# actionml/universal-recommender

Hardware: AMD Instinct MI355X
Metric: cooccurrence pairs/sec (A'A+A'B) + LLR top-k items/sec (higher is better)
Workload: dtype int32 counts / f64 LLR; 1 GPU; config4: synthetic 10M users x 2M items, Zipf-1.0, 5 event types (purchase/view/add-to-cart/search/category-pref); generator=torch Philox on the GPU (universal_recommender_amd.synth.generate_device), maxEventsPerEventType=500, maxCorrelatorsPerEventType=50, seed=20260925, entry_point=urcco_context_build_device (C ABI, include/urcco.h), launch=one process per GPU, parallelism=items range-partitioned over 1 GPU(s), one HIP stream per event type

## Files before the change

### include/urcco.h

```cpp
#ifndef URCCO_H
#define URCCO_H

#include <stdint.h>

#ifdef __cplusplus
extern "C" {
#endif

#define URCCO_VERSION 305

typedef enum urcco_status {
  URCCO_OK = 0,
  URCCO_BAD_ARG = 1,
  URCCO_OOM_HOST = 2,
  URCCO_OOM_DEVICE = 3,
  URCCO_HIP_ERROR = 4,
  URCCO_INTERNAL = 5,
  URCCO_NO_DEVICE = 6,
  URCCO_RCCL_ERROR = 7,
  URCCO_BUSY = 8
} urcco_status;

#define URCCO_ROW_RATE_MAHOUT_INT_DIV 0
#define URCCO_ROW_RATE_FRACTIONAL 1
// ... 117 lines not shown
  int32_t reserved;
  const urcco_dev_shard* shards;
} urcco_dev_dataset;
typedef struct urcco_dev_result {
  int32_t item_lo, item_hi;
  const int64_t* row_ptr;
  const int32_t* col_idx;
  const double* llr;
  const int64_t* stats;
  const int64_t* sampled_row_ptr;
  const int32_t* sampled_col_idx;
  int64_t sampled_rows;
  int64_t sampled_nnz_total;
  int32_t sampled_col_mask;
} urcco_dev_result;
int urcco_context_build_device(urcco_context* ctx, const urcco_dev_dataset* datasets, int32_t n_datasets, int64_t n_users_total,
                               int32_t random_seed, void* input_stream, urcco_dev_result* out);
int urcco_context_wait_stream(urcco_context* ctx, void* stream);
int urcco_context_synchronize(urcco_context* ctx);
int urcco_context_set_timing(urcco_context* ctx, int32_t enable);
int urcco_context_get_timings(urcco_context* ctx, double* ms, int64_t* launches);
int urcco_context_get_timings_gpu(urcco_context* ctx, int32_t local_gpu, double* ms, int64_t* launches);
int urcco_context_set_debug(urcco_context* ctx, int32_t flags);
int urcco_context_set_flags(urcco_context* ctx, int32_t flags);


typedef struct urcco_session urcco_session;

int urcco_session_create(int32_t device, void* stream, urcco_session** out);
void urcco_session_destroy(urcco_session* s);
int urcco_session_synchronize(urcco_session* s);
#define URCCO_N_STAGES 17
enum {
  URCCO_STAGE_COLUMN_COUNTS = 0,
  URCCO_STAGE_DOWNSAMPLE_FLAGS = 1,
  URCCO_STAGE_DOWNSAMPLE_SCAN = 2,
  URCCO_STAGE_DOWNSAMPLE_COMPACT = 3,
  URCCO_STAGE_TRANSPOSE = 4,
  URCCO_STAGE_ROW_WORK = 5,
  URCCO_STAGE_BINNING = 6,
  URCCO_STAGE_ENTROPY = 7,
  URCCO_STAGE_CCO_BIN0 = 8,
  URCCO_STAGE_CCO_BIN1 = 9,
  URCCO_STAGE_CCO_BIN2 = 10,
  URCCO_STAGE_CCO_BIN3 = 11,
  URCCO_STAGE_CCO_BIN4 = 12,
  URCCO_STAGE_CCO_BIN5 = 13,
  URCCO_STAGE_CCO_BIN6 = 14,
  URCCO_STAGE_COMPACT_INDICATORS = 15,
  URCCO_STAGE_EXCHANGE = 16
};
int urcco_session_set_timing(urcco_session* s, int32_t enable);
int urcco_session_set_debug(urcco_session* s, int32_t flags);
int urcco_session_get_timings(urcco_session* s, double* ms , int64_t* launches );
int64_t urcco_session_scratch_bytes(const urcco_session* s);
void urcco_debug_dump_marks(void);

int urcco_dev_column_counts(urcco_session* s, int64_t nnz, const int32_t* col_idx, int32_t n_cols, int32_t* counts);

int urcco_dev_downsample(urcco_session* s, int64_t n_rows, const int64_t* row_ptr, const int32_t* col_idx,
                         int64_t nnz, int32_t n_cols, const int32_t* raw_counts, int32_t seed,
                         int32_t max_elements_per_row, int32_t row_rate_mode, int64_t row_base,
                         int64_t* out_row_ptr, int32_t* out_col_idx, int32_t* post_counts);

int urcco_dev_transpose(urcco_session* s, int64_t n_rows, const int64_t* row_ptr, const int32_t* col_idx,
                        int64_t nnz, int32_t n_cols, const int32_t* counts, int32_t col_lo, int32_t col_hi,
                        int64_t* out_col_ptr, int32_t* out_row_idx);

int urcco_dev_row_work(urcco_session* s, int32_t item_lo, int32_t item_hi, int32_t n_items_a, const int64_t* a_col_ptr,
                       const int32_t* a_row_idx, int64_t nnz_a_bound, const int64_t* b_row_ptr, int64_t* work);

int urcco_dev_row_work_csr(urcco_session* s, int64_t n_rows, const int64_t* a_row_ptr, const int32_t* a_col_idx,
                           int64_t nnz_a, const int64_t* b_row_ptr, int32_t n_items_a, int64_t* work);

int urcco_dev_partition(urcco_session* s, int32_t n_items, const int64_t* work, int32_t n_parts,
                        int32_t* bounds_host);

int urcco_dev_merge_fragments(urcco_session* s, int32_t world, int32_t item_lo, int32_t item_hi, int32_t n_items,
                              const void* lens, int32_t wire16, const int32_t* entries, int64_t n_entries,
                              const int64_t* sizes, const int32_t* counts, int64_t* out_col_ptr, int32_t* out_row_idx);

#define URCCO_STATS_LEN 32
#define URCCO_EXCH_SIZES 4
int urcco_dev_cco_rows(urcco_session* s, int32_t item_lo, int32_t item_hi, int32_t n_items_a,
                       const int64_t* a_col_ptr, const int32_t* a_row_idx, int64_t nnz_a_bound,
                       const int64_t* b_row_ptr, const int32_t* b_col_idx, int32_t n_cols_b, const int32_t* counts_a,
                       const int32_t* counts_b, int64_t n_users, int32_t exclude_self, int32_t k,
                       int32_t has_min_llr, double min_llr, int32_t* out_count, int32_t* out_idx,
                       double* out_llr, int64_t* stats_dev);

int urcco_dev_pack_counts(urcco_session* s, int64_t n_rows_b, const int64_t* b_row_ptr, const int32_t* b_col_idx, int64_t nnz_b_bound, const int32_t* counts_b,
                          int32_t n_cols_b, int32_t* out_packed, int32_t* out_bad);
int urcco_dev_cco_rows_packed(urcco_session* s, int32_t item_lo, int32_t item_hi, int32_t n_items_a,
                              const int64_t* a_col_ptr, const int32_t* a_row_idx, int64_t nnz_a_bound,
                              const int64_t* b_row_ptr, const int32_t* b_col_idx, int32_t n_cols_b, const int32_t* counts_a,
                              const int32_t* counts_b, int64_t n_users, int32_t exclude_self, int32_t k,
                              int32_t has_min_llr, double min_llr, int32_t* out_count, int32_t* out_idx,
                              double* out_llr, int64_t* stats_dev, const int32_t* b_packed, const int32_t* pack_bad);

int urcco_dev_compact_indicators(urcco_session* s, int32_t n_rows, int32_t k, const int32_t* count,
                                 const int32_t* idx, const double* llr, int64_t* out_row_ptr,
                                 int32_t* out_col_idx, double* out_llr);

int urcco_dev_pop_counts(urcco_session* s, int64_t n_events, const int32_t* item_ids, const int64_t* times_ms, int32_t n_items,
                         int32_t n_intervals, const int64_t* bounds_host, int32_t* counts);

// ... 65 lines not shown
```

### universal-recommender_amd/_lib.py

```python
from __future__ import annotations

import ctypes as C
import os
from typing import Optional

_HERE = os.path.dirname(os.path.abspath(__file__))
DEFAULT_PATH = os.path.join(_HERE, "lib", "liburcco.so")

OK, BAD_ARG, OOM_HOST, OOM_DEVICE, HIP_ERROR, INTERNAL, NO_DEVICE, RCCL_ERROR, BUSY = range(9)
FLAG_SINGLE_STREAM = 1
FLAG_FORCE_EXCHANGE = 2
FLAG_UNORDERED_ROWS = 4
FLAG_EMULATE_RANKS = 8
UNIQUE_ID_BYTES = 128
ROW_RATE_MAHOUT_INT_DIV = 0
ROW_RATE_FRACTIONAL = 1
RNG_SPLITMIX53 = 0
RNG_MIX32 = 0x100
N_STAGES = 17
N_BINS = 7
STATS_LEN = 32
REC_MAX_CLAUSES = 16
REC_MAX_NUM = 256
REC_NO_BACKFILL = 1
# ... 68 lines not shown

class DatasetStats(C.Structure):
    _fields_ = [("nnz_raw", C.c_int64), ("nnz_sampled", C.c_int64), ("pairs", C.c_int64), ("nnz_out", C.c_int64),
                ("rows_by_bin", C.c_int64 * 7), ("ms_total", C.c_double)]


class RecClause(C.Structure):
    _fields_ = [("n_cols", C.c_int32), ("reserved", C.c_int32), ("boost", C.c_double), ("ind_col_ptr", C.c_void_p), ("ind_row_idx", C.c_void_p),
                ("q_row_ptr", C.c_void_p), ("q_col_idx", C.c_void_p)]


class RecRule(C.Structure):
    _fields_ = [("kind", C.c_int32), ("n_cols", C.c_int32), ("m_row_ptr", C.c_void_p), ("m_col_idx", C.c_void_p), ("q_row_ptr", C.c_void_p),
                ("q_col_idx", C.c_void_p), ("item_value", C.c_void_p), ("q_lo", C.c_void_p), ("q_hi", C.c_void_p)]


_p = C.c_void_p
SYMBOLS = {
    "urcco_version": (C.c_int, []),
    "urcco_device_count": (C.c_int, []),
    "urcco_last_error": (C.c_char_p, []),
    "urcco_status_string": (C.c_char_p, [C.c_int]),
    "urcco_cooccurrences_idss": (C.c_int, [C.POINTER(Csr), C.c_int32, C.c_int32, C.c_int32, C.c_int32, C.POINTER(Options),
                                           C.POINTER(Indicators), C.POINTER(DatasetStats)]),
    "urcco_cross_occurrence_downsampled": (C.c_int, [C.POINTER(Dataset), C.c_int32, C.c_int32, C.POINTER(Options),
                                                     C.POINTER(Indicators), C.POINTER(DatasetStats)]),
    "urcco_free_indicators": (None, [C.POINTER(Indicators), C.c_int32]),
    "urcco_cross_occurrence_stage": (C.c_int, [C.POINTER(Dataset), C.c_int32, C.c_int32, C.POINTER(Options)]),
    "urcco_cross_occurrence_finish": (C.c_int, [C.POINTER(Indicators), C.c_int32, C.POINTER(DatasetStats)]),
    "urcco_cross_occurrence_cancel": (C.c_int, []),
    "urcco_cross_occurrence_cancel_any": (C.c_int, []),
    "urcco_context_stage": (C.c_int, [_p, C.POINTER(Dataset), C.c_int32, C.c_int32]),
    "urcco_context_finish": (C.c_int, [_p, C.POINTER(Indicators), C.POINTER(DatasetStats)]),
    "urcco_shutdown": (C.c_int, []),
    "urcco_comm_unique_id": (C.c_int, [_p]),
    "urcco_context_create": (C.c_int, [C.POINTER(Options), C.POINTER(CommConfig), C.POINTER(_p)]),
    "urcco_context_destroy": (None, [_p]),
    "urcco_context_local_gpus": (C.c_int32, [_p]),
    "urcco_context_cross_occurrence": (C.c_int, [_p, C.POINTER(Dataset), C.c_int32, C.c_int32, C.POINTER(Indicators), C.POINTER(DatasetStats)]),
    "urcco_context_build_device": (C.c_int, [_p, C.POINTER(DevDataset), C.c_int32, C.c_int64, C.c_int32, _p, C.POINTER(DevResult)]),
    "urcco_context_wait_stream": (C.c_int, [_p, _p]),
    "urcco_context_synchronize": (C.c_int, [_p]),
    "urcco_context_set_timing": (C.c_int, [_p, C.c_int32]),
    "urcco_context_get_timings": (C.c_int, [_p, C.POINTER(C.c_double), C.POINTER(C.c_int64)]),
    "urcco_context_get_timings_gpu": (C.c_int, [_p, C.c_int32, C.POINTER(C.c_double), C.POINTER(C.c_int64)]),
    "urcco_context_set_debug": (C.c_int, [_p, C.c_int32]),
    "urcco_context_set_flags": (C.c_int, [_p, C.c_int32]),
    "urcco_session_create": (C.c_int, [C.c_int32, _p, C.POINTER(_p)]),
    "urcco_session_destroy": (None, [_p]),
    "urcco_session_synchronize": (C.c_int, [_p]),
    "urcco_session_scratch_bytes": (C.c_int64, [_p]),
    "urcco_session_set_timing": (C.c_int, [_p, C.c_int32]),
    "urcco_session_set_debug": (C.c_int, [_p, C.c_int32]),
    "urcco_debug_dump_marks": (None, []),
    "urcco_session_get_timings": (C.c_int, [_p, C.POINTER(C.c_double), C.POINTER(C.c_int64)]),
    "urcco_dev_column_counts": (C.c_int, [_p, C.c_int64, _p, C.c_int32, _p]),
    "urcco_dev_downsample": (C.c_int, [_p, C.c_int64, _p, _p, C.c_int64, C.c_int32, _p, C.c_int32, C.c_int32, C.c_int32, C.c_int64,
                                       _p, _p, _p]),
    "urcco_dev_transpose": (C.c_int, [_p, C.c_int64, _p, _p, C.c_int64, C.c_int32, _p, C.c_int32, C.c_int32, _p, _p]),
    "urcco_dev_row_work_csr": (C.c_int, [_p, C.c_int64, _p, _p, C.c_int64, _p, C.c_int32, _p]),
    "urcco_dev_row_work": (C.c_int, [_p, C.c_int32, C.c_int32, C.c_int32, _p, _p, C.c_int64, _p, _p]),
    "urcco_dev_partition": (C.c_int, [_p, C.c_int32, _p, C.c_int32, C.POINTER(C.c_int32)]),
    "urcco_dev_merge_fragments": (C.c_int, [_p, C.c_int32, C.c_int32, C.c_int32, C.c_int32, _p, C.c_int32, _p, C.c_int64, _p, _p, _p, _p]),
    "urcco_dev_cco_rows": (C.c_int, [_p, C.c_int32, C.c_int32, C.c_int32, _p, _p, C.c_int64, _p, _p, C.c_int32, _p, _p, C.c_int64, C.c_int32,
                                     C.c_int32, C.c_int32, C.c_double, _p, _p, _p, _p]),
    "urcco_dev_pack_counts": (C.c_int, [_p, C.c_int64, _p, _p, C.c_int64, _p, C.c_int32, _p, _p]),
    "urcco_dev_cco_rows_packed": (C.c_int, [_p, C.c_int32, C.c_int32, C.c_int32, _p, _p, C.c_int64, _p, _p, C.c_int32, _p, _p, C.c_int64, C.c_int32,
                                            C.c_int32, C.c_int32, C.c_double, _p, _p, _p, _p, _p, _p]),
    "urcco_dev_compact_indicators": (C.c_int, [_p, C.c_int32, C.c_int32, _p, _p, _p, _p, _p, _p]),
    "urcco_dev_pop_counts": (C.c_int, [_p, C.c_int64, _p, _p, C.c_int32, C.c_int32, C.POINTER(C.c_int64), _p]),
    "urcco_dev_recommend": (C.c_int, [_p, C.c_int64, C.c_int32, C.POINTER(RecClause), C.c_int32, _p, _p, _p, _p, C.c_int32, C.c_int32, _p, _p, _p, _p]),
    "urcco_dev_recommend_rules": (C.c_int, [_p, C.c_int64, C.c_int32, C.POINTER(RecClause), C.c_int32, _p, _p, _p, _p, C.c_int32, C.c_int32, _p, _p, _p, _p,
                                            C.POINTER(RecRule), C.c_int32]),
    "urcco_dev_llr": (C.c_int, [_p, C.c_int64, _p, _p, _p, _p, _p]),
    "urcco_dev_u01": (C.c_int, [_p, C.c_int64, C.c_int32, _p, _p, _p]),
    "urcco_dev_u01_rng": (C.c_int, [_p, C.c_int64, C.c_int32, _p, _p, C.c_int32, _p]),
    "urcco_dev_dictionary_build": (C.c_int, [_p, C.c_int64, _p, _p, C.c_int32, _p, C.POINTER(_p), C.POINTER(C.c_int64)]),
    "urcco_dev_dictionary_lookup": (C.c_int, [_p, _p, C.c_int64, _p, _p, _p]),
    "urcco_dev_dictionary_verify": (C.c_int, [_p, _p, C.c_int64, _p, _p, _p, _p, C.POINTER(C.c_int64)]),
    "urcco_dev_dictionary_verify_against": (C.c_int, [_p, _p, C.c_int64, _p, _p, _p, _p, _p, C.POINTER(C.c_int64)]),
    "urcco_hash_strings": (C.c_int, [_p, _p, C.c_int64, C.c_uint64, _p]),
    "urcco_key_table_destroy": (None, [_p]),
    "urcco_dev_csr_from_pairs": (C.c_int, [_p, C.c_int64, _p, _p, C.c_int64, _p, _p, C.POINTER(C.c_int64)]),
}

_cache = {}
_lib_path: Optional[str] = None


def _bind(path: str) -> C.CDLL:
    try:
        import torch
    except ImportError:
        pass
    lib = C.CDLL(path)
    for name, (res, args) in SYMBOLS.items():
        fn = getattr(lib, name)
        fn.restype = res
        fn.argtypes = args
    return lib


def use_library(path: Optional[str]) -> None:
    global _lib_path
    _lib_path = path

# ... 26 lines not shown
```

### universal-recommender_amd/csrc/cco_common.h

```cpp
#pragma once
#include "cco_kernels.h"

namespace urcco {


constexpr int WAVE = 64;

__device__ __forceinline__ unsigned long long shfl_xor_u64(unsigned long long v, int m) {
  unsigned lo = (unsigned)v, hi = (unsigned)(v >> 32);
  lo = __shfl_xor(lo, m);
  hi = __shfl_xor(hi, m);
  return ((unsigned long long)hi << 32) | lo;
}
__device__ __forceinline__ long long shfl_i64(long long v, int src) {
  unsigned lo = (unsigned)v, hi = (unsigned)((unsigned long long)v >> 32);
  lo = __shfl(lo, src);
  hi = __shfl(hi, src);
  return (long long)(((unsigned long long)hi << 32) | lo);
}
__device__ __forceinline__ long long shfl_up_i64(long long v, unsigned d) {
  unsigned lo = (unsigned)v, hi = (unsigned)((unsigned long long)v >> 32);
  lo = __shfl_up(lo, d);
  hi = __shfl_up(hi, d);
  return (long long)(((unsigned long long)hi << 32) | lo);
// ... 35 lines not shown
        x[2 * q + 1] = (long long)(((unsigned long long)(unsigned)a.w << 32) | (unsigned)a.z);
      }
    } else {
#pragma unroll
      for (int q = 0; q < 8; ++q) x[q] = p[i + q];
    }
  }
};
template <int NT = SCAN_THREADS>
__device__ __forceinline__ long long block_exclusive_scan(long long v, long long* s_wave , long long* total) {
  const int lane = threadIdx.x & (WAVE - 1), wave = threadIdx.x / WAVE;
  long long inc = v;
#pragma unroll
  for (int d = 1; d < WAVE; d <<= 1) {
    const long long o = shfl_up_i64(inc, d);
    if (lane >= d) inc += o;
  }
  if (lane == WAVE - 1) s_wave[wave] = inc;
  __syncthreads();
  long long base = 0, tot = 0;
#pragma unroll
  for (int w = 0; w < NT / WAVE; ++w) {
    const long long sw = s_wave[w];
    if (w < wave) base += sw;
    tot += sw;
  }
  __syncthreads();
  *total = tot;
  return base + inc - v;
}

template <typename Load>
__global__ __launch_bounds__(SCAN_THREADS) void scan_reduce_kernel(Load ld, int64_t n, int64_t* __restrict__ tile_sums,
                                                                   const int64_t* __restrict__ n_live) {
  __shared__ long long s_wave[SCAN_THREADS / WAVE];
  const int64_t base = (int64_t)blockIdx.x * SCAN_TILE;
  if (n_live && base >= *n_live) {
    if (threadIdx.x == 0) tile_sums[blockIdx.x] = 0;
    return;
  }
  long long v = 0;
#pragma unroll
  for (int q = 0; q < SCAN_ITEMS; ++q) {
    const int64_t i = base + (int64_t)q * SCAN_THREADS + threadIdx.x;
    if (i < n) v += ld(i);
  }
  long long tot;
  block_exclusive_scan(v, s_wave, &tot);
  if (threadIdx.x == 0) tile_sums[blockIdx.x] = tot;
}

constexpr int ST_THREADS = 1024;
constexpr int ST_ITEMS = 8;
static __global__ __launch_bounds__(ST_THREADS) void scan_tiles_kernel(int64_t* __restrict__ tile_sums, int64_t n_tiles, const int64_t* __restrict__ n_live) {
  __shared__ long long s_wave[ST_THREADS / WAVE];
  const int lane = threadIdx.x & (WAVE - 1), wave = threadIdx.x / WAVE;
  int64_t live_tiles = n_tiles;
  if (n_live) {
    const int64_t lt = *n_live / SCAN_TILE + 1;
    if (lt < live_tiles) live_tiles = lt;
  }
  long long carry = 0;
  for (int64_t base = 0; base < live_tiles; base += ST_THREADS * ST_ITEMS) {
    const int64_t first = base + (int64_t)threadIdx.x * ST_ITEMS;
    long long x[ST_ITEMS];
    long long sum = 0;
#pragma unroll
    for (int q = 0; q < ST_ITEMS; ++q) {
      x[q] = first + q < live_tiles ? tile_sums[first + q] : 0;
      sum += x[q];
    }
    long long inc = sum;
#pragma unroll
    for (int d = 1; d < WAVE; d <<= 1) {
      const long long o = shfl_up_i64(inc, d);
      if (lane >= d) inc += o;
    }
    if (lane == WAVE - 1) s_wave[wave] = inc;
    __syncthreads();
    long long before = 0, tot = 0;
#pragma unroll
    for (int w = 0; w < ST_THREADS / WAVE; ++w) {
      const long long sw = s_wave[w];
      if (w < wave) before += sw;
      tot += sw;
    }
    __syncthreads();
    long long run = carry + before + inc - sum;
#pragma unroll
    for (int q = 0; q < ST_ITEMS; ++q) {
      if (first + q < live_tiles) tile_sums[first + q] = run;
      run += x[q];
    }
    carry += tot;
  }
  for (int64_t t = live_tiles + threadIdx.x; t < n_tiles; t += ST_THREADS) tile_sums[t] = carry;
  if (threadIdx.x == 0) tile_sums[n_tiles] = carry;
}

template <typename Load>
__global__ __launch_bounds__(SCAN_THREADS) void scan_downsweep_kernel(Load ld, int64_t n, const int64_t* __restrict__ tile_sums,
                                                                      int64_t n_tiles, int64_t* __restrict__ out,
                                                                      const int64_t* __restrict__ n_live) {
  __shared__ long long s_wave[SCAN_THREADS / WAVE];
  if (n_live && (int64_t)blockIdx.x * SCAN_TILE > *n_live) return;
  const int64_t first = (int64_t)blockIdx.x * SCAN_TILE + (int64_t)threadIdx.x * SCAN_ITEMS;
  static_assert(SCAN_ITEMS == 8, "load8");
  long long x[SCAN_ITEMS];
  long long v = 0;
  const bool interior = first + SCAN_ITEMS <= n;
  if (interior) {
    ld.load8(first, x);
  } else {
#pragma unroll
    for (int q = 0; q < SCAN_ITEMS; ++q) x[q] = first + q < n ? ld(first + q) : 0;
  }
#pragma unroll
  for (int q = 0; q < SCAN_ITEMS; ++q) v += x[q];
  long long tot;
  long long run = block_exclusive_scan(v, s_wave, &tot) + tile_sums[blockIdx.x];
  if (interior && (reinterpret_cast<uintptr_t>(out) & 15) == 0) {
#pragma unroll
    for (int q = 0; q < SCAN_ITEMS; q += 2) {
      const long long e0 = run, e1 = run + x[q];
      run = e1 + x[q + 1];
      int4 w;
      w.x = (int)(unsigned)e0; w.y = (int)(unsigned)((unsigned long long)e0 >> 32);
      w.z = (int)(unsigned)e1; w.w = (int)(unsigned)((unsigned long long)e1 >> 32);
      *reinterpret_cast<int4*>(out + first + q) = w;
    }
  } else {
#pragma unroll
    for (int q = 0; q < SCAN_ITEMS; ++q) {
      const int64_t i = first + q;
      if (i < n) out[i] = run;
      run += x[q];
    }
  }
  if (blockIdx.x == 0 && threadIdx.x == 0) out[n] = tile_sums[n_tiles];
}

constexpr int SB_THREADS = 1024;
constexpr int SB_ITEMS = 8;
constexpr int64_t SB_MAX = 32768;
template <typename Load>
__global__ __launch_bounds__(SB_THREADS) void scan_block_kernel(Load ld, int64_t n, int64_t* __restrict__ out) {
  __shared__ long long s_wave[SB_THREADS / WAVE];
  const int lane = threadIdx.x & (WAVE - 1), wave = threadIdx.x / WAVE;
  long long carry = 0;
  for (int64_t base = 0; base < n; base += SB_THREADS * SB_ITEMS) {
    const int64_t first = base + (int64_t)threadIdx.x * SB_ITEMS;
    long long x[SB_ITEMS];
    long long sum = 0;
    if (first + SB_ITEMS <= n) {
      ld.load8(first, x);
    } else {
#pragma unroll
      for (int q = 0; q < SB_ITEMS; ++q) x[q] = first + q < n ? ld(first + q) : 0;
    }
#pragma unroll
    for (int q = 0; q < SB_ITEMS; ++q) sum += x[q];
    long long inc = sum;
#pragma unroll
    for (int d = 1; d < WAVE; d <<= 1) {
      const long long o = shfl_up_i64(inc, d);
      if (lane >= d) inc += o;
    }
    if (lane == WAVE - 1) s_wave[wave] = inc;
    __syncthreads();
    long long before = 0, tot = 0;
#pragma unroll
    for (int w = 0; w < SB_THREADS / WAVE; ++w) {
      const long long sw = s_wave[w];
      if (w < wave) before += sw;
      tot += sw;
    }
    __syncthreads();
    long long run = carry + before + inc - sum;
#pragma unroll
    for (int q = 0; q < SB_ITEMS; ++q) {
      if (first + q < n) out[first + q] = run;
      run += x[q];
    }
    carry += tot;
  }
  if (threadIdx.x == 0) out[n] = carry;
}

template <typename Load>
static hipError_t launch_scan(hipStream_t st, Load ld, int64_t n, int64_t* out, int64_t* tile_sums, const int64_t* n_live = nullptr, bool tile_sums_ready = false) {
  if (n <= 0) return hipMemsetAsync(out, 0, sizeof(int64_t), st);
  if (n <= SB_MAX) {
    hipLaunchKernelGGL((scan_block_kernel<Load>), dim3(1), dim3(SB_THREADS), 0, st, ld, n, out);
    return hipGetLastError();
  }
  const int64_t n_tiles = (n + SCAN_TILE - 1) / SCAN_TILE;
  if (!tile_sums_ready) hipLaunchKernelGGL((scan_reduce_kernel<Load>), dim3((unsigned)n_tiles), dim3(SCAN_THREADS), 0, st, ld, n, tile_sums, n_live);
  hipLaunchKernelGGL(scan_tiles_kernel, dim3(1), dim3(ST_THREADS), 0, st, tile_sums, n_tiles, n_live);
  hipLaunchKernelGGL((scan_downsweep_kernel<Load>), dim3((unsigned)n_tiles), dim3(SCAN_THREADS), 0, st, ld, n, tile_sums, n_tiles, out, n_live);
  return hipGetLastError();
}
}
```

### universal-recommender_amd/csrc/cco_expand.hip

```cpp
#include "cco_kernels.h"

#include <atomic>
#include <cstdio>
#include <cstdlib>

#include "cco_common.h"
#include "cco_device.h"


namespace urcco {

__global__ __launch_bounds__(256) void item_entropy_kernel(const int32_t* __restrict__ counts, int32_t n, long long n_users,
                                                           double* __restrict__ ent, double* __restrict__ xlx_n) {
  const int64_t i = (int64_t)blockIdx.x * 256 + threadIdx.x;
  if (i < n) {
    const long long c = counts[i];
    ent[i] = entropy2(c, n_users - c);
  }
  if (i == 0 && xlx_n) *xlx_n = x_log_x(n_users);
}

hipError_t launch_item_entropy(hipStream_t st, const int32_t* counts, int32_t n, long long n_users, double* ent, double* xlx_n) {
  const int blocks = n > 0 ? (n + 255) / 256 : 1;
  hipLaunchKernelGGL(item_entropy_kernel, dim3(blocks), dim3(256), 0, st, counts, n, n_users, ent, xlx_n);
// ... 58 lines not shown
    const unsigned d0 = two ? (unsigned)cnt[z.x] : 0u, d1 = two ? (unsigned)cnt[z.y] : 0u, d2 = two ? (unsigned)cnt[z.z] : 0u, d3 = two ? (unsigned)cnt[z.w] : 0u;
    n_bad += (c0 >= limit) + (c1 >= limit) + (c2 >= limit) + (c3 >= limit) + (d0 >= limit) + (d1 >= limit) + (d2 >= limit) + (d3 >= limit);
    int4 y;
    y.x = (int)((unsigned)x.x | (c0 << shift)); y.y = (int)((unsigned)x.y | (c1 << shift));
    y.z = (int)((unsigned)x.z | (c2 << shift)); y.w = (int)((unsigned)x.w | (c3 << shift));
    nt_store4(out + 4 * v, y);
    if (two) {
      y.x = (int)((unsigned)z.x | (d0 << shift)); y.y = (int)((unsigned)z.y | (d1 << shift));
      y.z = (int)((unsigned)z.z | (d2 << shift)); y.w = (int)((unsigned)z.w | (d3 << shift));
      nt_store4(out + 4 * (v + stride), y);
    }
  }
  for (int64_t e = (nvec << 2) + (int64_t)blockIdx.x * 256 + threadIdx.x; e < nnz; e += stride) {
    const unsigned j = (unsigned)ci[e], c = (unsigned)cnt[j];
    n_bad += c >= limit;
    out[e] = (int)(j | (c << shift));
  }
  if (n_bad) atomicAdd(bad, n_bad);
}
hipError_t launch_pack_counts(hipStream_t st, int n_cu, const int32_t* col_idx, const int64_t* nnz_dev, int64_t nnz_bound, const unsigned short* counts16,
                              const int32_t* bad16, int32_t count_bits, int32_t* out, int32_t* bad) {
  hipError_t e = hipMemsetAsync(bad, 0, sizeof(int32_t), st);
  if (e != hipSuccess || nnz_bound <= 0) return e;
  const int shift = 32 - count_bits;
  int64_t blocks = (nnz_bound / 4 + 255) / 256;
  const int64_t cap = (int64_t)n_cu * 16;
  if (blocks > cap) blocks = cap;
  if (blocks < 1) blocks = 1;
  const int vec_ok = ((reinterpret_cast<uintptr_t>(col_idx) | reinterpret_cast<uintptr_t>(out)) & 15) == 0;
  hipLaunchKernelGGL(pack_counts_kernel, dim3((unsigned)blocks), dim3(256), 0, st, col_idx, nnz_dev, nnz_bound, counts16, bad16, shift, out, bad, vec_ok);
  return hipGetLastError();
}

__global__ __launch_bounds__(256) void xlx_table_kernel(double* __restrict__ tab) {
  const int x = blockIdx.x * 256 + threadIdx.x;
  if (x < XLX_TABLE) tab[x] = x_log_x((long long)x);
}
hipError_t launch_xlx_table(hipStream_t st, double* tab) {
  hipLaunchKernelGGL(xlx_table_kernel, dim3(XLX_TABLE / 256), dim3(256), 0, st, tab);
  return hipGetLastError();
}
__global__ __launch_bounds__(256) void xlx_hi_table_kernel(double* __restrict__ tab, const double* __restrict__ xlx_tab, long long n_users) {
  const int d = blockIdx.x * 256 + threadIdx.x;
  if (d >= XLX_TABLE) return;
  tab[d] = n_users - d >= 0 ? x_log_x(n_users - (long long)d) : 0.0;
  const double hi = n_users - d >= 0 ? x_log_x(n_users - (long long)d) : 0.0;
  tab[XLX_TABLE + d] = d <= n_users ? (x_log_x(n_users) - x_log_x_tab((long long)d, xlx_tab)) - hi : 0.0;
}
hipError_t launch_xlx_hi_table(hipStream_t st, double* tab, const double* xlx_tab, long long n_users) {
  hipLaunchKernelGGL(xlx_hi_table_kernel, dim3(XLX_TABLE / 256), dim3(256), 0, st, tab, xlx_tab, n_users);
  return hipGetLastError();
}

__global__ __launch_bounds__(256) void narrow_row_ptr_kernel(const int64_t* __restrict__ rp, int64_t n, unsigned* __restrict__ out) {
  for (int64_t i = (int64_t)blockIdx.x * 256 + threadIdx.x; i < n; i += (int64_t)gridDim.x * 256) out[i] = (unsigned)rp[i];
}

__global__ __launch_bounds__(256) void expand_prepare_kernel(const int64_t* __restrict__ a_cp, int32_t n_items_a, const int32_t* __restrict__ a_ri,
                                                             const int64_t* __restrict__ b_rp, const unsigned* __restrict__ b_rp32, int64_t n_rows_b,
                                                             int64_t cap, int64_t* __restrict__ pstart, int32_t* __restrict__ plen) {
  const int64_t nnz = a_cp[n_items_a];
  int64_t lim = (nnz / SCAN_TILE + 1) * SCAN_TILE;
  if (lim > cap) lim = cap;
  const bool narrow = b_rp32 != nullptr && b_rp[n_rows_b] < ((int64_t)1 << 32);
  const int64_t stride = (int64_t)gridDim.x * 256;
  for (int64_t p0 = (int64_t)blockIdx.x * 256 + threadIdx.x; p0 < lim; p0 += stride * 4) {
    int u[4];
#pragma unroll
    for (int q = 0; q < 4; ++q) {
      const int64_t p = p0 + q * stride;
      u[q] = p < nnz ? a_ri[p] : -1;
    }
    int64_t s[4], e[4];
    if (narrow) {
#pragma unroll
      for (int q = 0; q < 4; ++q) {
        s[q] = u[q] >= 0 ? (int64_t)b_rp32[u[q]] : 0;
        e[q] = u[q] >= 0 ? (int64_t)b_rp32[u[q] + 1] : 0;
      }
    } else {
#pragma unroll
      for (int q = 0; q < 4; ++q) {
        s[q] = u[q] >= 0 ? b_rp[u[q]] : 0;
        e[q] = u[q] >= 0 ? b_rp[u[q] + 1] : 0;
      }
    }
#pragma unroll
    for (int q = 0; q < 4; ++q) {
      const int64_t p = p0 + q * stride;
      if (p < lim) {
        pstart[p] = s[q];
        plen[p] = (int32_t)(e[q] - s[q]);
      }
    }
  }
}

hipError_t launch_expand_prepare(hipStream_t st, int n_cu, const int64_t* a_col_ptr, int32_t n_items_a, const int32_t* a_row_idx,
                                 const int64_t* b_row_ptr, unsigned* b_rp32_scratch, int64_t n_rows_b, int64_t cap, int64_t* pstart, int32_t* plen,
                                 int64_t* wp, int64_t* tile_sums) {
  if (cap > 0) {
    if (b_rp32_scratch) {
      int64_t nb = (n_rows_b + 1 + 255) / 256;
      if (nb > (int64_t)n_cu * 8) nb = (int64_t)n_cu * 8;
      hipLaunchKernelGGL(narrow_row_ptr_kernel, dim3((unsigned)nb), dim3(256), 0, st, b_row_ptr, n_rows_b + 1, b_rp32_scratch);
    }
    int64_t blocks = (cap + 1023) / 1024;
    const int64_t lim = (int64_t)n_cu * 16;
    if (blocks > lim) blocks = lim;
    hipLaunchKernelGGL(expand_prepare_kernel, dim3((unsigned)blocks), dim3(256), 0, st, a_col_ptr, n_items_a, a_row_idx, b_row_ptr,
                       (const unsigned*)b_rp32_scratch, n_rows_b, cap, pstart, plen);
  }
  return launch_scan(st, LoadI32{plen}, cap, wp, tile_sums, a_col_ptr + n_items_a);
}

struct __attribute__((packed, aligned(4))) Words4 { unsigned a, b, c, d; };
struct __attribute__((packed, aligned(4))) Words2 { unsigned a, b; };
struct ExpandMultiArgs {
  const int64_t* b_rp[EXPAND_MULTI_MAX];
  int64_t* pstart[EXPAND_MULTI_MAX];
  int32_t* plen[EXPAND_MULTI_MAX];
  int64_t* tsum[EXPAND_MULTI_MAX];
  int n;
};
__global__ __launch_bounds__(256) void expand_pack_kernel(ExpandMultiArgs a, int64_t n_rows_b, unsigned* __restrict__ T) {
  for (int64_t u = (int64_t)blockIdx.x * 256 + threadIdx.x; u <= n_rows_b; u += (int64_t)gridDim.x * 256)
    for (int d = 0; d < a.n; ++d) T[u * a.n + d] = (unsigned)a.b_rp[d][u];
}
template <int N>
__global__ __launch_bounds__(256) void expand_prepare_multi_kernel(const int64_t* __restrict__ a_cp, int32_t n_items_a, const int32_t* __restrict__ a_ri,
                                                                   const unsigned* __restrict__ T, int64_t cap, ExpandMultiArgs a) {
  __shared__ long long s_part[256 / WAVE][N];
  const int64_t nnz = a_cp[n_items_a];
  int64_t lim = (nnz / SCAN_TILE + 1) * SCAN_TILE;
  if (lim > cap) lim = cap;
  const int64_t n_tiles = (lim + SCAN_TILE - 1) / SCAN_TILE;
  for (int64_t tile = blockIdx.x; tile < n_tiles; tile += gridDim.x) {
    const int64_t base = tile * SCAN_TILE;
    long long sum[N];
#pragma unroll
    for (int d = 0; d < N; ++d) sum[d] = 0;
    for (int r = 0; r < SCAN_ITEMS; r += 2) {
      int u[2];
      unsigned v[2][2 * N];
#pragma unroll
      for (int q = 0; q < 2; ++q) {
        const int64_t p = base + (int64_t)(r + q) * 256 + threadIdx.x;
        u[q] = p < nnz ? a_ri[p] : -1;
      }
#pragma unroll
      for (int q = 0; q < 2; ++q) {
        if (u[q] >= 0) {
          const unsigned* t = T + (int64_t)u[q] * N;
          if (N == 4) {
            const uint4 x = *reinterpret_cast<const uint4*>(t), y = *reinterpret_cast<const uint4*>(t + 4);
            v[q][0] = x.x; v[q][1] = x.y; v[q][2] = x.z; v[q][3] = x.w;
            v[q][4 % (2 * N)] = y.x; v[q][5 % (2 * N)] = y.y; v[q][6 % (2 * N)] = y.z; v[q][7 % (2 * N)] = y.w;
          } else {
            constexpr int W = 2 * N;
#pragma unroll
            for (int d = 0; d + 4 <= W; d += 4) {
              const Words4 x = *reinterpret_cast<const Words4*>(t + d);
              v[q][d] = x.a; v[q][(d + 1) % W] = x.b; v[q][(d + 2) % W] = x.c; v[q][(d + 3) % W] = x.d;
            }
            if (W % 4 >= 2) {
              const Words2 x = *reinterpret_cast<const Words2*>(t + (W / 4) * 4);
              v[q][(W / 4) * 4 % W] = x.a; v[q][((W / 4) * 4 + 1) % W] = x.b;
            }
            if (W % 2 == 1) v[q][W - 1] = t[W - 1];
          }
        } else {
#pragma unroll
          for (int d = 0; d < 2 * N; ++d) v[q][d] = 0u;
        }
      }
#pragma unroll
      for (int q = 0; q < 2; ++q) {
        const int64_t p = base + (int64_t)(r + q) * 256 + threadIdx.x;
        if (p < lim) {
#pragma unroll
          for (int d = 0; d < N; ++d) {
            const int32_t len = (int32_t)(v[q][N + d] - v[q][d]);
            a.pstart[d][p] = (int64_t)v[q][d];
            a.plen[d][p] = len;
            sum[d] += (long long)len;
          }
        }
      }
    }
#pragma unroll
    for (int d = 0; d < N; ++d) {
      unsigned long long x = (unsigned long long)sum[d];
#pragma unroll
      for (int m = 1; m < WAVE; m <<= 1) x += shfl_xor_u64(x, m);
      if ((threadIdx.x & (WAVE - 1)) == 0) s_part[threadIdx.x / WAVE][d] = (long long)x;
    }
    __syncthreads();
    if (threadIdx.x < N && a.tsum[threadIdx.x]) {
      long long tot = 0;
#pragma unroll
      for (int w = 0; w < 256 / WAVE; ++w) tot += s_part[w][threadIdx.x];
      a.tsum[threadIdx.x][tile] = tot;
    }
    __syncthreads();
  }
}
hipError_t launch_expand_prepare_multi(hipStream_t st, int n_cu, const int64_t* a_col_ptr, int32_t n_items_a, const int32_t* a_row_idx, int n,
                                       const int64_t* const* b_row_ptr, int64_t n_rows_b, int64_t cap, int64_t* const* pstart, int32_t* const* plen, void* T,
                                       int64_t* const* tsum) {
  if (n < 1 || n > EXPAND_MULTI_MAX) return hipErrorInvalidValue;
  if (cap <= 0) return hipSuccess;
  ExpandMultiArgs a;
  a.n = n;
  for (int d = 0; d < EXPAND_MULTI_MAX; ++d) {
    a.b_rp[d] = d < n ? b_row_ptr[d] : nullptr;
    a.pstart[d] = d < n ? pstart[d] : nullptr;
    a.plen[d] = d < n ? plen[d] : nullptr;
    a.tsum[d] = (d < n && tsum) ? tsum[d] : nullptr;
  }
  int64_t nb = (n_rows_b + 255) / 256;
  if (nb > (int64_t)n_cu * 8) nb = (int64_t)n_cu * 8;
  if (nb < 1) nb = 1;
  hipLaunchKernelGGL(expand_pack_kernel, dim3((unsigned)nb), dim3(256), 0, st, a, n_rows_b, static_cast<unsigned*>(T));
  int64_t blocks = (cap + SCAN_TILE - 1) / SCAN_TILE;
  const int64_t lim = (int64_t)n_cu * 16;
  if (blocks > lim) blocks = lim;
  const unsigned* Tc = static_cast<const unsigned*>(T);
  switch (n) {
    case 1: hipLaunchKernelGGL(expand_prepare_multi_kernel<1>, dim3((unsigned)blocks), dim3(256), 0, st, a_col_ptr, n_items_a, a_row_idx, Tc, cap, a); break;
    case 2: hipLaunchKernelGGL(expand_prepare_multi_kernel<2>, dim3((unsigned)blocks), dim3(256), 0, st, a_col_ptr, n_items_a, a_row_idx, Tc, cap, a); break;
    case 3: hipLaunchKernelGGL(expand_prepare_multi_kernel<3>, dim3((unsigned)blocks), dim3(256), 0, st, a_col_ptr, n_items_a, a_row_idx, Tc, cap, a); break;
    case 4: hipLaunchKernelGGL(expand_prepare_multi_kernel<4>, dim3((unsigned)blocks), dim3(256), 0, st, a_col_ptr, n_items_a, a_row_idx, Tc, cap, a); break;
    case 5: hipLaunchKernelGGL(expand_prepare_multi_kernel<5>, dim3((unsigned)blocks), dim3(256), 0, st, a_col_ptr, n_items_a, a_row_idx, Tc, cap, a); break;
    case 6: hipLaunchKernelGGL(expand_prepare_multi_kernel<6>, dim3((unsigned)blocks), dim3(256), 0, st, a_col_ptr, n_items_a, a_row_idx, Tc, cap, a); break;
    case 7: hipLaunchKernelGGL(expand_prepare_multi_kernel<7>, dim3((unsigned)blocks), dim3(256), 0, st, a_col_ptr, n_items_a, a_row_idx, Tc, cap, a); break;
    default: hipLaunchKernelGGL(expand_prepare_multi_kernel<8>, dim3((unsigned)blocks), dim3(256), 0, st, a_col_ptr, n_items_a, a_row_idx, Tc, cap, a); break;
  }
  return hipGetLastError();
}
hipError_t launch_expand_scan(hipStream_t st, const int64_t* a_col_ptr, int32_t n_items_a, const int32_t* plen, int64_t cap, int64_t* wp, int64_t* tile_sums,
                              bool tile_sums_ready) {
  return launch_scan(st, LoadI32{plen}, cap, wp, tile_sums, a_col_ptr + n_items_a, tile_sums_ready);
}

__global__ __launch_bounds__(256) void row_work_kernel(int32_t item_lo, int32_t item_hi, const int64_t* __restrict__ a_cp,
                                                       const int64_t* __restrict__ wp, int64_t* __restrict__ work) {
  const int64_t n = (int64_t)item_hi - item_lo;
  for (int64_t t = (int64_t)blockIdx.x * 256 + threadIdx.x; t < n; t += (int64_t)gridDim.x * 256) {
    const int64_t i = item_lo + t;
    work[t] = wp[a_cp[i + 1]] - wp[a_cp[i]];
  }
}

hipError_t launch_row_work(hipStream_t st, int n_cu, int32_t item_lo, int32_t item_hi, const int64_t* a_col_ptr, const int64_t* wp, int64_t* work) {
  const int64_t n = (int64_t)item_hi - item_lo;
  if (n <= 0) return hipSuccess;
  int64_t blocks = (n + 255) / 256;
  const int64_t cap = (int64_t)n_cu * 8;
  if (blocks > cap) blocks = cap;
  hipLaunchKernelGGL(row_work_kernel, dim3((unsigned)blocks), dim3(256), 0, st, item_lo, item_hi, a_col_ptr, wp, work);
  return hipGetLastError();
}


}
```

### universal-recommender_amd/csrc/cco_kernels.h

```cpp
#pragma once
#include <hip/hip_runtime.h>
#include <stdint.h>

namespace urcco {

constexpr int NBINS = 7;
constexpr int MP_KMAX_HOST = 256;

constexpr int SCAN_TILE = 2048;
constexpr int DS_TILE = 4096;
constexpr int GLOBAL_BIN_BLOCKS = 128;
constexpr int BIN_TILE = 1024;
constexpr int XLX_TABLE_HOST = 4096;
constexpr int BIN_COLS_HOST = 3 * NBINS + 3;
constexpr int BIN_OFF_LEN = NBINS + 3;
constexpr int CAND_SLOTS = 64;
constexpr int STATS_LEN = 32;

constexpr int32_t DBG_GATHER_ONLY = 1;
constexpr int32_t DBG_NO_LLR = 2;
constexpr int32_t DBG_NO_TOPK = 4;
constexpr int32_t DBG_NO_SELECT = 8;
constexpr int32_t DBG_NO_RANK = 16;
constexpr int32_t DBG_NO_COUNT_GATHER = 512;
constexpr int32_t DBG_UNFUSED_EXPAND = 4096;
constexpr int32_t DBG_GATHERED_PRIMARY = 8192;
constexpr int32_t DBG_UNFILTERED_EXCHANGE = 16384;
constexpr int32_t DBG_SELECT_DELAY = 131072;
constexpr int32_t DBG_UNPACKED_COUNTS = 1048576;
constexpr int32_t DBG_ROW_KERNELS = DBG_GATHER_ONLY | DBG_NO_LLR | DBG_NO_TOPK | DBG_NO_SELECT | DBG_NO_RANK | DBG_NO_COUNT_GATHER | DBG_SELECT_DELAY;

struct CcoArgs {
  const int32_t* bin_rows;
  const int32_t* bin_off;
  const int64_t* a_col_ptr;
  const int64_t* pstart;
  const int64_t* wp;
  const int32_t* b_col_idx;
  const int32_t* b_packed;
  const int32_t* pack_bad;
  int32_t pk_known;
  uint32_t b_col_mask;
  const int32_t* cnt_a;
  const int32_t* cnt_b;
  const double* ent_a;
  const unsigned short* cnt_b16;
  const int32_t* cnt16_bad;
  const double* xlx_n;
  const double* xlx_tab;
  const double* xlx_hi;
  const double* col_ent;
  int32_t debug;
  long long n_users;
  int32_t n_cols_b;
  int32_t item_lo;
  int32_t exclude_self;
  int32_t k;
  int32_t has_min_llr;
  double min_llr;
  int32_t count_bits;
  int32_t col_bytes;
  int32_t g_log2;
  int32_t unordered;
  int32_t* out_count;
  int32_t* out_idx;
  double* out_llr;
  unsigned long long* err;
  unsigned long long* cand;
  int32_t* g_counts;
  unsigned long long* g_cand_key;
  int32_t* g_cand_col;
  int32_t g_blocks;
};

hipError_t launch_column_counts(hipStream_t st, int n_cu, const int32_t* col_idx, int64_t nnz, int32_t n_cols, int32_t* counts);
constexpr int64_t PH_MIN_NNZ = 1 << 20;
int64_t column_counts_scratch_bytes(int64_t nnz, int32_t n_cols);
hipError_t launch_column_counts_partitioned(hipStream_t st, const int32_t* col_idx, int64_t nnz, const int64_t* nnz_dev, int32_t n_cols,
                                            int32_t* counts, char* scratch);

hipError_t launch_scan_i32(hipStream_t st, const int32_t* in, int64_t n, int64_t* out, int64_t* tile_sums);
hipError_t launch_slice_weights(hipStream_t st, const unsigned short* loc_t, int n_buckets, int64_t n_parts, long long* weight);

hipError_t launch_downsample_flags(hipStream_t st, int n_cu, int64_t n_rows, const int64_t* row_ptr, const int32_t* col_idx, int64_t nnz,
                                   int32_t n_cols, const int32_t* raw_counts, unsigned long long* thresholds, uint32_t seed, int32_t max_n,
                                   int row_rate_mode, int64_t row_base, int64_t* tile_rows, unsigned long long* flags, int64_t* tile_count,
                                   int32_t* post_counts);
hipError_t launch_downsample_scan(hipStream_t st, int64_t nnz, int64_t* tile_count);
hipError_t launch_downsample_compact(hipStream_t st, int64_t n_rows, const int64_t* row_ptr, const int32_t* col_idx, int64_t nnz,
                                     const int64_t* tile_rows, const unsigned long long* flags, const int64_t* tile_off, int64_t* out_row_ptr,
                                     int32_t* out_col_idx);

hipError_t launch_scan_i32_range(hipStream_t st, const int32_t* in, int64_t n, int32_t lo, int32_t hi, int64_t* out, int64_t* tile_sums);
hipError_t launch_transpose(hipStream_t st, int n_cu, int64_t n_rows, const int64_t* row_ptr, const int32_t* col_idx, int g_log2,
                            const int64_t* col_ptr, int32_t* cursor, int32_t* out_row_idx, int32_t col_lo, int32_t col_hi);
int64_t transpose_scratch_bytes(int64_t n_rows, int64_t nnz, int32_t n_cols);
hipError_t launch_transpose_partitioned(hipStream_t st, int64_t n_rows, const int64_t* row_ptr, const int32_t* col_idx, int64_t nnz, int32_t n_cols,
                                        const int64_t* col_ptr, int32_t* cursor , int32_t* out_row_idx, int32_t col_lo, int32_t col_hi, char* scratch);
hipError_t launch_row_work_csr(hipStream_t st, int n_cu, int64_t n_rows, const int64_t* a_row_ptr, const int32_t* a_col_idx,
                               const int64_t* b_row_ptr, int g_log2, int32_t n_items_a, int64_t* work);

struct KeyTable {
  unsigned long long* keys;
  unsigned* minpos;
  unsigned* count;
  int32_t* id;
  unsigned long long mask;
};
hipError_t launch_dictionary_build(hipStream_t st, int n_cu, KeyTable t, int64_t n, const unsigned long long* keys, const int32_t* select,
                                   int32_t min_count, int32_t* flag, int64_t* prefix, int64_t* tile_sums, int64_t* first_pos);
hipError_t launch_dictionary_lookup(hipStream_t st, int n_cu, KeyTable t, int64_t n, const unsigned long long* keys, const int32_t* select,
                                    int32_t* ids);
hipError_t launch_dictionary_verify(hipStream_t st, int n_cu, KeyTable t, int64_t n, const unsigned long long* keys, const int32_t* select,
                                    const unsigned long long* check, const unsigned long long* ref_check, const int64_t* first_pos, unsigned long long* err);
hipError_t launch_csr_from_pairs(hipStream_t st, int n_cu, int64_t n, const int32_t* rows, const int32_t* cols, int64_t n_rows, int32_t* cnt,
                                 int64_t* raw_ptr, int32_t* tmp, int64_t* tile_sums, int64_t* out_row_ptr, int32_t* out_col_idx);

constexpr int EXCH_SIZES = 4;
hipError_t launch_row_lengths(hipStream_t st, int n_cu, int64_t n_rows, const int64_t* row_ptr, int32_t* len, unsigned short* len16, int64_t* sizes);
hipError_t launch_counts_over_limit(hipStream_t st, int n_cu, const int32_t* counts, int64_t n, int32_t count_bits, int64_t* out);
hipError_t launch_need_mask(hipStream_t st, int n_cu, int64_t n_rows, const int64_t* a_row_ptr, const int32_t* a_col_idx, const int32_t* bounds, int world,
                            unsigned long long* mask);
hipError_t launch_masked_lengths(hipStream_t st, int n_cu, int64_t n_rows, const int64_t* row_ptr, const unsigned long long* mask, int world, int32_t* mlen, int64_t* off,
                                 int64_t* tile_sums, int64_t* to_nnz);
hipError_t launch_pack_rows(hipStream_t st, int n_cu, int64_t n_rows, const int64_t* row_ptr, const int32_t* col_idx, const unsigned long long* mask, int world,
                            const int64_t* off, int32_t* pack);
hipError_t launch_scan_u16(hipStream_t st, const unsigned short* in, int64_t n, int64_t* out, int64_t* tile_sums);
hipError_t launch_frag_record(hipStream_t st, int32_t world, const int32_t* bounds, const int64_t* l_cp, const int32_t* bad, int64_t* rec);
hipError_t launch_frag_place(hipStream_t st, int n_cu, int32_t world, int32_t lo, int32_t n_range, const void* lens, int wire16, const int64_t* src_off,
                             const int32_t* ents, const int64_t* a_cp, const int64_t* sizes, int32_t* a_ri);

hipError_t launch_validate_csr(hipStream_t st, int n_cu, int64_t n_rows, const int64_t* row_ptr, const int32_t* col_idx, int64_t nnz, int32_t n_cols,
                               int g_log2, int64_t rp0, unsigned long long* err);
hipError_t launch_rebase_i64(hipStream_t st, int n_cu, int64_t* p, int64_t n, int64_t delta);
hipError_t launch_publish_word(hipStream_t st, const unsigned long long* src, unsigned long long* dst_mapped);

hipError_t launch_pop_counts(hipStream_t st, int n_cu, int64_t n, const int32_t* item, const int64_t* t_ms, int32_t n_items, int n_buckets,
                             const int64_t* bounds, int32_t* counts);

hipError_t launch_pack_counts(hipStream_t st, int n_cu, const int32_t* col_idx, const int64_t* nnz_dev, int64_t nnz_bound, const unsigned short* counts16,
                              const int32_t* bad16, int32_t count_bits, int32_t* out, int32_t* bad);
hipError_t launch_xlx_table(hipStream_t st, double* tab);
hipError_t launch_xlx_hi_table(hipStream_t st, double* tab , const double* xlx_tab, long long n_users);
hipError_t launch_item_entropy(hipStream_t st, const int32_t* counts, int32_t n, long long n_users, double* ent, double* xlx_n);
hipError_t launch_narrow_counts(hipStream_t st, int n_cu, const int32_t* counts, int64_t n, unsigned short* out16, int32_t* bad);

hipError_t launch_expand_prepare(hipStream_t st, int n_cu, const int64_t* a_col_ptr, int32_t n_items_a, const int32_t* a_row_idx,
                                 const int64_t* b_row_ptr, unsigned* b_rp32_scratch , int64_t n_rows_b, int64_t cap,
                                 int64_t* pstart, int32_t* plen, int64_t* wp, int64_t* tile_sums);
constexpr int EXPAND_MULTI_MAX = 8;
hipError_t launch_expand_prepare_multi(hipStream_t st, int n_cu, const int64_t* a_col_ptr, int32_t n_items_a, const int32_t* a_row_idx, int n,
                                       const int64_t* const* b_row_ptr, int64_t n_rows_b, int64_t cap, int64_t* const* pstart, int32_t* const* plen, void* T,
                                       int64_t* const* tsum );
hipError_t launch_expand_scan(hipStream_t st, const int64_t* a_col_ptr, int32_t n_items_a, const int32_t* plen, int64_t cap, int64_t* wp, int64_t* tile_sums,
                              bool tile_sums_ready = false);
hipError_t launch_row_work(hipStream_t st, int n_cu, int32_t item_lo, int32_t item_hi, const int64_t* a_col_ptr, const int64_t* wp, int64_t* work);

hipError_t launch_binning(hipStream_t st, int32_t item_lo, int32_t n, const int64_t* work, const int32_t* cnt_a, int32_t n_cols_b,
                          int32_t count_bits, int32_t k, int64_t* tile_counts, int32_t* bin_off, int32_t* bin_rows, int64_t* stats);

hipError_t launch_cco_rows_bin(hipStream_t st, int n_cu, const CcoArgs& args, int bin, int32_t n_rows );
hipError_t launch_bin_out_stats(hipStream_t st, const int32_t* bin_rows, const int32_t* bin_off, int32_t item_lo, const int32_t* out_count,
                                const unsigned long long* cand, int64_t* stats);

hipError_t launch_compact_indicators(hipStream_t st, int32_t n_rows, int32_t k, const int32_t* count, const int32_t* idx,
                                     const double* llr, const int64_t* row_ptr, int32_t* out_idx, double* out_llr);

hipError_t launch_partition(hipStream_t st, int32_t n_items, const int64_t* work_prefix, int32_t n_parts, int32_t* bounds);
hipError_t launch_scan_i64(hipStream_t st, const int64_t* in, int64_t n, int64_t* out, int64_t* tile_sums);

constexpr int REC_MAX_CLAUSES = 16;
constexpr int REC_MAX_NUM = 256;
constexpr int REC_NO_BACKFILL = 1;
constexpr int REC_STATS_LEN = 8;
constexpr int REC_LDS_LIMIT = 3072;
struct RecClause {
  const int64_t* ind_col_ptr;
  const int32_t* ind_row_idx;
  const int64_t* q_row_ptr;
  const int32_t* q_col_idx;
  double boost;
  int32_t n_cols;
  int32_t reserved;
};
constexpr int REC_MAX_RULES = 16;
constexpr int REC_RULE_ANY = 0;
constexpr int REC_RULE_NONE = 1;
constexpr int REC_RULE_RANGE = 2;
struct RecRule {
  const int64_t* m_row_ptr;
  const int32_t* m_col_idx;
  const int64_t* q_row_ptr;
  const int32_t* q_col_idx;
  const int64_t* item_value;
  const int64_t* q_lo;
  const int64_t* q_hi;
  int32_t kind, n_cols;
};
struct RecArgs;
int32_t recommend_global_blocks(int64_t n_queries, int32_t n_items, int n_cu);
hipError_t launch_recommend(hipStream_t st, int n_cu, int64_t n_queries, int32_t n_items, const RecClause* clauses, int32_t n_clauses, const int64_t* excl_row_ptr,
                            const int32_t* excl_col_idx, const uint8_t* item_mask, const int32_t* fill_order, int32_t num, int32_t flags, int32_t* out_count,
                            int32_t* out_idx, double* out_score, int64_t* stats_dev, unsigned long long* ctr, int32_t* list, int32_t* pos, int32_t g_blocks,
                            unsigned* g_state, unsigned* g_m, int32_t* g_list, double* g_score, int32_t lds_limit = REC_LDS_LIMIT, const RecRule* rules = nullptr,
                            int32_t n_rules = 0);

hipError_t launch_llr_test(hipStream_t st, int64_t n, const int64_t* a, const int64_t* b, const int64_t* ab, const int64_t* nu, double* out);
hipError_t launch_u01_test(hipStream_t st, int64_t n, uint32_t seed, const int32_t* row, const int32_t* col, double* out, int rng32 = 0);

// ... 2 lines not shown
```

### universal-recommender_amd/csrc/cco_rows.hip

```cpp
#include "cco_kernels.h"

#include <atomic>
#include <cstdlib>

#include "cco_common.h"
#include "cco_device.h"


namespace urcco {

constexpr int E0 = 1024, E1S = 4096, E1 = 8192, E2S = 16384, E2 = 32768;
constexpr int MP_KMAX = 256;

__host__ __device__ constexpr int table_slots(int E, int T) { return (2 * E / 3) / (2 * T) * (2 * T); }
constexpr int URCCO_WB1 = 512;
constexpr int URCCO_WB2 = 8192;
__device__ __forceinline__ int choose_bin(long long w, long long ca, int32_t n_cols_b, int32_t count_bits, int32_t k) {
  if (ca <= 0 || w <= 0) return -1;
  if (count_bits < 31 && ca > ((1ll << count_bits) - 1)) return NBINS - 1;
  if (w <= 64 && ca <= 64) return 0;
  int cap_bin = NBINS - 1;
  const long long dmax = (w < (long long)n_cols_b ? w : (long long)n_cols_b) * 3 + (long long)k * 3 + 2;
  if (dmax <= E0) cap_bin = 1;
  else if (dmax <= E1S) cap_bin = 2;
// ... 389 lines not shown
}

template <int T>
__device__ __forceinline__ unsigned claim_positions(bool want, unsigned* counter, unsigned& wave_count) {
  const unsigned long long m = __ballot(want);
  const unsigned c = (unsigned)__popcll(m);
  unsigned base;
  if (T == WAVE) {
    base = wave_count;
    wave_count += c;
  } else {
    unsigned b = 0u;
    if ((threadIdx.x & (WAVE - 1)) == 0 && c != 0u) b = atomicAdd(counter, c);
    base = wave_read_lane(b, 0);
  }
  return base + lanes_below(m);
}
template <int T>
__device__ __forceinline__ unsigned team_exclusive_scan(unsigned v, unsigned* s_wsum , unsigned* total) {
  const int lane = threadIdx.x & (WAVE - 1);
  const unsigned inc = wave_inclusive_sum(v);
  if (T == WAVE) {
    *total = wave_read_lane(inc, WAVE - 1);
    return inc - v;
  }
  const int wave = (threadIdx.x % T) / WAVE;
  if (lane == WAVE - 1) s_wsum[wave] = inc;
  __syncthreads();
  unsigned base = 0, tot = 0;
#pragma unroll
  for (int w = 0; w < T / WAVE; ++w) {
    const unsigned sw = s_wsum[w];
    if (w < wave) base += sw;
    tot += sw;
  }
  __syncthreads();
  *total = tot;
  return base + inc - v;
}

constexpr int URCCO_U_WAVE = 2;
constexpr int URCCO_U_BS = 2;
constexpr int URCCO_U_B = 2;
constexpr int URCCO_U_H = 1;
constexpr int URCCO_U_C = 1;
constexpr int URCCO_OCC_WAVE = 8;
constexpr int URCCO_OCC_BS = 7;
constexpr int URCCO_G_WAVE = 2;
constexpr int URCCO_SEL_AMB_WAVE = 64;
constexpr int URCCO_SEL_AMB_BLOCK = 128;
constexpr int URCCO_G_BLOCK = 2;
constexpr int URCCO_SEL_M_BLOCK = 128;
constexpr int URCCO_G_CU = 2;
template <int T, int E, int U, bool MP = false, bool DBG = false, bool PK = false>
__global__ __launch_bounds__((T < 256 ? 256 : T), (T == 64 ? URCCO_OCC_WAVE : (T == 256 && E == 4096 ? URCCO_OCC_BS : (T == 512 ? 4 : 1)))) void cco_rows_kernel(CcoArgs a, int bin) {
  if ((a.b_packed != nullptr && (a.pk_known != 0 || *a.pack_bad == 0)) != PK) return;
  const int dbg = DBG ? a.debug : 0;
  constexpr bool packed = PK;
  URCCO_OWN_GLOBAL_PTR(const int32_t, b_col_idx, PK ? a.b_packed : a.b_col_idx);
  const int cshift = 32 - a.count_bits;
  const unsigned colmask = PK ? (1u << cshift) - 1u : a.b_col_mask;
  URCCO_OWN_GLOBAL_PTR(const unsigned short, cnt_b16, a.cnt_b16);
  URCCO_OWN_GLOBAL_PTR(const int32_t, cnt_b, a.cnt_b);
  URCCO_OWN_GLOBAL_PTR(const double, xlx_tab, a.xlx_tab);
  URCCO_OWN_GLOBAL_PTR(const double, xlx_hi, a.xlx_hi);
  URCCO_OWN_GLOBAL_PTR(const double, col_ent, a.col_ent);
  URCCO_OWN_GLOBAL_PTR(int32_t, out_idx, a.out_idx);
  URCCO_OWN_GLOBAL_PTR(double, out_llr, a.out_llr);
  long long n_users = a.n_users;
  URCCO_OWN_SGPRS(n_users);
  constexpr int BLOCK = T < 256 ? 256 : T;
  constexpr int TEAMS = BLOCK / T;
  constexpr int SH = table_slots(E, T);
  constexpr int SPT = SH / T;
  static_assert(SH % (2 * T) == 0 && SH + SH / 2 <= E && SH <= 65536, "slots and the candidate list share the table; a slot index takes 16 bits of a list word");
  constexpr unsigned CAND_CAP = (unsigned)(E - SH);
  constexpr int CPT = ((E - 5) / 3 + T - 1) / T;
  constexpr int NW = T / WAVE;
  constexpr int G = T == WAVE ? URCCO_G_WAVE : (T == 256 ? URCCO_G_BLOCK : URCCO_G_CU);
  constexpr int LOG2E = E == 1024 ? 10 : (E == 4096 ? 12 : (E == 8192 ? 13 : (E == 16384 ? 14 : 15)));
  static_assert((1 << LOG2E) == E, "table size");
  constexpr int LOG2T = T == 64 ? 6 : (T == 256 ? 8 : (T == 512 ? 9 : 10));
  static_assert((1 << LOG2T) == T, "team size");
  __shared__ __attribute__((aligned(16))) unsigned s_tab[TEAMS * E];
  constexpr int NH = T == WAVE ? 1 : 3;
  constexpr int SEL_CAP = T == WAVE ? 0 : (T == 256 ? 512 : 2048);
  constexpr int SEL_M = T == WAVE ? 64 : URCCO_SEL_M_BLOCK;
  constexpr int SEL_AMB = T == WAVE ? URCCO_SEL_AMB_WAVE : URCCO_SEL_AMB_BLOCK;
  static_assert(SEL_AMB <= SEL_M, "ambiguous set capacity");
  constexpr bool SHARE = T == WAVE || (T == 256 && E == 4096);
  constexpr int SH_INS = T * 8 + (T + 1) * 4;
  constexpr int SH_LST = ((NH * 128 * 4 > SEL_M * 12 ? NH * 128 * 4 : SEL_M * 12) + 7) / 8 * 8;
  constexpr int SH_SEL = SH_LST + SEL_CAP * 2;
  constexpr int SHARE_WORDS = ((SH_INS > SH_SEL ? SH_INS : SH_SEL) + 7) / 8;
  __shared__ unsigned long long s_share[SHARE ? TEAMS * SHARE_WORDS : 1];
  __shared__ long long s_ustart[SHARE ? 1 : TEAMS * T];
  __shared__ unsigned s_uoff[SHARE ? 1 : TEAMS * (T + 1)];
  __shared__ unsigned s_wsum[NW];
  __shared__ unsigned s_hist[SHARE ? 1 : TEAMS * NH * 128];
  __shared__ unsigned s_selres[TEAMS * 4];
  __shared__ unsigned short s_lst[SHARE ? 1 : TEAMS * (SEL_CAP > 0 ? SEL_CAP : 1)];
  __shared__ unsigned long long s_ambkey[SHARE ? 1 : TEAMS * SEL_M];
  __shared__ unsigned s_ambcol[SHARE ? 1 : TEAMS * SEL_M];
  __shared__ unsigned long long s_selthr[TEAMS * 2];
  constexpr bool SKIP_SHARED = T >= 256;
  __shared__ unsigned long long s_kbits[2 * NW];
  __shared__ unsigned s_mpflag;
  __shared__ unsigned s_ncand;
  __shared__ unsigned long long s_runk[MP ? 2 * MP_KMAX : 1];
  __shared__ unsigned s_runc[MP ? 2 * MP_KMAX : 1];

  const int team = TEAMS == 1 ? 0 : uni((int)threadIdx.x / T);
  const int tl = threadIdx.x % T;
  const int lane = threadIdx.x & (WAVE - 1);
  unsigned* tab = s_tab + team * E;
  unsigned* cand = tab + SH;
  unsigned long long* share = s_share + (SHARE ? team * SHARE_WORDS : 0);
  long long* ustart = SHARE ? reinterpret_cast<long long*>(share) : s_ustart + team * T;
  unsigned* uoff = SHARE ? reinterpret_cast<unsigned*>(share + T) : s_uoff + team * (T + 1);
  unsigned* hist = SHARE ? reinterpret_cast<unsigned*>(share) : s_hist + team * NH * 128;
  unsigned* sel_res = s_selres + team * 4;
  unsigned* nsel = sel_res + 3;
  unsigned short* lst = SHARE ? reinterpret_cast<unsigned short*>(share) + SH_LST / 2 : s_lst + team * (SEL_CAP > 0 ? SEL_CAP : 1);
  unsigned long long* amb_key = SHARE ? share : s_ambkey + team * SEL_M;
  unsigned* amb_col = SHARE ? reinterpret_cast<unsigned*>(share + SEL_M) : s_ambcol + team * SEL_M;
  unsigned long long* sel_thr = s_selthr + team * 2;
  const int list_start = a.bin_off[bin];
  const int list_n = a.bin_off[bin + 1] - list_start;
  const int total_teams = gridDim.x * TEAMS;
  bool ident = (long long)a.n_cols_b * 3 + (long long)a.k * 3 + 2 <= E && a.n_cols_b <= SH;
  int cb = a.count_bits;
  unsigned cmask = (1u << cb) - 1u;
  unsigned long long cand_acc = 0ull;
  const double xlx_n = *a.xlx_n;
  const bool use16 = *a.cnt16_bad == 0;

  int li = blockIdx.x * TEAMS + team;
  if (li >= list_n) return;
  const int S = total_teams;
  auto pos_of = [&](int l) { return list_start + (l < list_n ? l : list_n - 1); };
  const unsigned* wp32 = reinterpret_cast<const unsigned*>(a.wp);
  const int lane3 = lane < 3 ? lane : 2;
  int idv = a.bin_rows[pos_of(li + lane3 * S)];
  int64_t cs_c, ce_c;
  int64_t bnd_b;
  {
    const int id0 = (int)wave_read_lane((unsigned)idv, 0);
    const int id1 = (int)wave_read_lane((unsigned)idv, 1);
    cs_c = uni(a.a_col_ptr[id0]);
    ce_c = uni(a.a_col_ptr[id0 + 1]);
    bnd_b = a.a_col_ptr[id1 + (lane & 1)];
  }
  unsigned pf_w0, pf_w1, pf_wp;
  int64_t pf_start;
  {
    const int64_t c1 = cs_c + T < ce_c ? cs_c + T : ce_c;
    const int64_t pl = cs_c + tl < c1 ? cs_c + tl : c1 - 1;
    pf_w0 = wp32[2 * cs_c];
    pf_w1 = wp32[2 * c1];
    pf_wp = wp32[2 * pl];
    pf_start = a.pstart[pl];
  }
  URCCO_SETTLE(idv); URCCO_SETTLE(bnd_b); URCCO_SETTLE(pf_w0); URCCO_SETTLE(pf_w1); URCCO_SETTLE(pf_wp); URCCO_SETTLE(pf_start);
  int64_t cs_n = 0, ce_n = 0, bnd_c = 0;
  for (; li < list_n; li += S, cs_c = cs_n, ce_c = ce_n, bnd_b = bnd_c) {
    const int i = (int)wave_read_lane((unsigned)idv, 0);
    const int id2 = (int)wave_read_lane((unsigned)idv, 2);
    const int64_t cs = cs_c, ce = ce_c;
    cs_n = wave_read_lane64(bnd_b, 0);
    ce_n = wave_read_lane64(bnd_b, 1);
    const unsigned row_w0 = uni(pf_w0), row_w1 = uni(pf_w1);
    const unsigned my_wp = pf_wp;
    const int64_t my_start = pf_start;
    int lz = lane;
    URCCO_OPAQUE(lz);
    idv = a.bin_rows[pos_of(li + (1 + (lz < 3 ? lz : 2)) * S)];
    bnd_c = a.a_col_ptr[id2 + (lz & 1)];
    if (!MP) {
      const int64_t c1 = cs_n + T < ce_n ? cs_n + T : ce_n;
      const int64_t pl = cs_n + tl < c1 ? cs_n + tl : c1 - 1;
      pf_w0 = wp32[2 * cs_n];
      pf_w1 = wp32[2 * c1];
      pf_wp = wp32[2 * pl];
      pf_start = a.pstart[pl];
    }
    int mp_s = 0;
    unsigned mp_q = 0u, n_run = 0u, run_cur = 0u;
    if (MP) {
      const long long w_row = (long long)(uni(a.wp[ce]) - uni(a.wp[cs]));
      const long long ca_row = a.cnt_a[i];
      const long long dd = w_row < (long long)a.n_cols_b ? w_row : (long long)a.n_cols_b;
      const long long cap = ((long long)E - 3ll * a.k - 2ll) / 3ll;
      for (;; ++mp_s) {
        const long long cols_pp = ((long long)a.n_cols_b + (1ll << mp_s) - 1) >> mp_s;
        int kb = 1;
        while ((1ll << kb) <= cols_pp) ++kb;
        const bool count_ok = kb <= 1 || ca_row <= (1ll << (32 - kb)) - 1;
        const long long exp_d = ((dd >> mp_s) + (dd >> (mp_s + 2)) + 1) < cols_pp ? ((dd >> mp_s) + (dd >> (mp_s + 2)) + 1) : cols_pp;
        if (count_ok && exp_d <= cap) break;
      }
    }
  mp_again:
    if (MP) {
      const long long cols_pp = ((long long)a.n_cols_b + (1ll << mp_s) - 1) >> mp_s;
      int kb = 1;
      while ((1ll << kb) <= cols_pp) ++kb;
      cb = 32 - kb;
      cmask = cb >= 32 ? 0xffffffffu : (1u << cb) - 1u;
      ident = cols_pp * 3 + 3ll * a.k + 2ll <= (long long)E && cols_pp <= (long long)SH;
      if (tl == 0) s_mpflag = 0u;
    }
    const unsigned mp_mask = MP ? (1u << mp_s) - 1u : 0u;
#pragma unroll
    for (int q = 0; q < SPT / 2; ++q) *reinterpret_cast<uint2*>(&tab[2 * (tl + q * T)]) = make_uint2(0u, 0u);
    unsigned n_cand = 0u;
    if (T != WAVE && tl == 0) s_ncand = 0u;
    team_sync<T>();
    for (int64_t c0 = cs; c0 < ce; c0 += T) {
      const int64_t c1 = c0 + T < ce ? c0 + T : ce;
      const bool pre = !MP && c0 == cs;
      const unsigned w0 = pre ? row_w0 : uni(wp32[2 * c0]);
      const unsigned total = (pre ? row_w1 : uni(wp32[2 * c1])) - w0;
      const int64_t p = c0 + tl;
      if (p < c1) {
        ustart[tl] = pre ? my_start : a.pstart[p];
        uoff[tl] = (pre ? my_wp : wp32[2 * p]) - w0;
      } else {
        uoff[tl] = total;
      }
      if (tl == 0) uoff[T] = total;
      team_sync<T>();
      if (total > 0u) {
        const unsigned per = (total + T - 1) / T;
        const unsigned first = (unsigned)tl * per;
        const bool act = first < total;
        const unsigned last = act ? (first + per < total ? first + per : total) : first;
        int o = 0;
        int64_t pos = 0;
        unsigned uend = 0u;
        if (act) {
          int lo = 1, hi = T;
#pragma unroll
          for (int step = 0; step < LOG2T; ++step) {
            const int mid = (lo + hi) >> 1;
            const bool gt = uoff[mid] > first;
            hi = gt ? mid : hi;
            lo = gt ? lo : mid + 1;
          }
          o = lo - 1;
          pos = ustart[o] + (first - uoff[o]);
          uend = uoff[o + 1];
        }
        for (unsigned x = 0; x < per; x += G) {
          unsigned jj[G];
          bool on[G];
#pragma unroll
          for (int q = 0; q < G; ++q) {
            const unsigned t = first + x + (unsigned)q;
            on[q] = t < last;
            jj[q] = 0u;
            if (on[q]) {
              if (t >= uend) {
                do { ++o; } while (uoff[o + 1] <= t);
                pos = ustart[o];
                uend = uoff[o + 1];
              }
              jj[q] = (unsigned)b_col_idx[pos++];
            }
          }
          unsigned at[G];
#pragma unroll
          for (int q = 0; q < G; ++q) {
            at[q] = ~0u;
            if (on[q]) {
              const unsigned col = jj[q] & colmask;
              if (dbg & DBG_GATHER_ONLY) {
                if (jj[q] == 0xffffffffu) tab[0] = 1u;
              } else if (MP) {
                if ((col & mp_mask) == mp_q && !tab_insert<SH>(tab, (col >> mp_s) + 1u, cb, ident, at[q])) s_mpflag = 1u;
              } else if (!tab_insert<SH>(tab, col + 1u, cb, ident, at[q])) {
                atomicAdd(a.err, 1ull);
              }
            }
          }
          unsigned long long cm[G];
          unsigned n_new = 0u;
#pragma unroll
          for (int q = 0; q < G; ++q) {
            cm[q] = __ballot(at[q] != ~0u);
            n_new += (unsigned)__popcll(cm[q]);
          }
          if (n_new != 0u) {
            unsigned base;
            if (T == WAVE) {
              base = n_cand;
              n_cand += n_new;
            } else {
              unsigned b = 0u;
              if (lane == 0) b = atomicAdd(&s_ncand, n_new);
              base = wave_read_lane(b, 0);
            }
#pragma unroll
            for (int q = 0; q < G; ++q) {
              const unsigned idx = base + lanes_below(cm[q]);
              if (at[q] != ~0u) {
                if (idx < CAND_CAP) cand[idx] = at[q] | ((packed ? jj[q] >> cshift : 0u) << 16);
                else if (MP) s_mpflag = 1u;
                else atomicAdd(a.err, 1ull);
              }
              base += (unsigned)__popcll(cm[q]);
            }
          }
        }
      }
      team_sync<T>();
    }
    unsigned D = T == WAVE ? n_cand : uni(s_ncand);
// ... 402 lines not shown
      const unsigned* rc = s_runc + run_cur * MP_KMAX;
      for (unsigned t = (unsigned)tl; t < n_run; t += T) {
        out_idx[obase + t] = (int)rc[t];
        out_llr[obase + t] = __longlong_as_double((long long)rk[t]);
      }
      if (tl == 0) a.out_count[i - a.item_lo] = (int)n_run;
    }
    team_sync<T>();
  }
  if (a.cand && tl == 0 && cand_acc != 0ull) atomicAdd(&a.cand[(blockIdx.x * TEAMS + team) & (CAND_SLOTS - 1)], cand_acc);
}

constexpr int URCCO_OCC_MICRO = 8;
template <int L> struct MicroGeom {
  static constexpr int S = WAVE / L;
  static constexpr int TW = 256 / S;
  static constexpr int LOG2TW = S == 1 ? 8 : (S == 2 ? 7 : 6);
  static constexpr int LIST = L + 4;
  static constexpr int MARKS = L + 2;
  static constexpr int ROW_WORDS = LIST + 2 * LIST + MARKS;
  static constexpr int WORDS = (256 + S * ROW_WORDS + 3) / 4 * 4;
};
template <int L>
__device__ __forceinline__ unsigned seg_inclusive_max(unsigned v) {
  if (L == WAVE) return wave_inclusive_max(v);
  int x = (int)v;
  int y;
  y = __builtin_amdgcn_update_dpp(0, x, 0x111, 0xf, 0xf, true);
  x = (unsigned)y > (unsigned)x ? y : x;
  y = __builtin_amdgcn_update_dpp(0, x, 0x112, 0xf, 0xf, true);
  x = (unsigned)y > (unsigned)x ? y : x;
  y = __builtin_amdgcn_update_dpp(0, x, 0x114, 0xf, 0xf, true);
  x = (unsigned)y > (unsigned)x ? y : x;
  y = __builtin_amdgcn_update_dpp(0, x, 0x118, 0xf, 0xf, true);
  x = (unsigned)y > (unsigned)x ? y : x;
  if (L == 32) {
    y = __builtin_amdgcn_update_dpp(0, x, 0x142, 0xa, 0xf, false);
    x = (unsigned)y > (unsigned)x ? y : x;
  }
  return (unsigned)x;
}
template <int L>
__device__ __forceinline__ unsigned seg_max_popc(unsigned long long m) {
  if (L == WAVE) return (unsigned)__popcll(m);
  unsigned best = 0;
#pragma unroll
  for (int q = 0; q < WAVE / L; ++q) {
    const unsigned c = (unsigned)__popcll((m >> (q * L)) & ((1ull << L) - 1ull));
    best = c > best ? c : best;
  }
  return best;
}

template <int L, bool DBG, bool PK = false>
__global__ __launch_bounds__(256, (L == WAVE ? URCCO_OCC_MICRO : URCCO_OCC_MICRO - 2)) void cco_rows_micro_kernel(CcoArgs a) {
  if ((a.b_packed != nullptr && (a.pk_known != 0 || *a.pack_bad == 0)) != PK) return;
  using G = MicroGeom<L>;
  constexpr int S = G::S;
  const int dbg = DBG ? a.debug : 0;
  const int32_t* bin_rows = a.bin_rows;
  const int64_t* a_col_ptr = a.a_col_ptr;
  const int64_t* pstart = a.pstart;
  constexpr bool packed = PK;
  const int32_t* b_col_idx = PK ? a.b_packed : a.b_col_idx;
  const int cshift = 32 - a.count_bits;
  const unsigned colmask = PK ? (1u << cshift) - 1u : a.b_col_mask;
  const int32_t* cnt_a = a.cnt_a;
  const double* ent_a = a.ent_a;
  const double* xlx_tab = a.xlx_tab;
  const double* xlx_hi = a.xlx_hi;
  const double* col_ent = a.col_ent;
  int32_t* out_idx = a.out_idx;
  double* out_llr = a.out_llr;
  int32_t* out_count = a.out_count;
  long long n_users = a.n_users;
  constexpr int TEAMS = 256 / WAVE;
  __shared__ __attribute__((aligned(16))) unsigned s_tab[TEAMS * G::WORDS];
  const int team = threadIdx.x / WAVE;
  const int lane = threadIdx.x & (WAVE - 1);
  const int seg = lane / L, sl = lane % L;
  const unsigned long long seg_mask = L == WAVE ? ~0ull : (((1ull << (L % WAVE)) - 1ull) << (seg * L));
  unsigned* tab_w = s_tab + team * G::WORDS;
  unsigned* tab = tab_w + seg * G::TW;
  unsigned* cand = tab_w + 256 + seg * G::ROW_WORDS;
  unsigned long long* kkm = reinterpret_cast<unsigned long long*>(cand + G::LIST);
  unsigned* marks = cand + 3 * G::LIST;
  const int list_start = L == 16 ? a.bin_off[0] : a.bin_off[NBINS + (L == 32 ? 1 : 2)];
  const int list_n = (L == 16 ? a.bin_off[NBINS + 1] : (L == 32 ? a.bin_off[NBINS + 2] : a.bin_off[1])) - list_start;
  const int n_groups = (list_n + S - 1) / S;
  const int total_teams = gridDim.x * TEAMS;
  const bool ident = a.n_cols_b <= G::TW;
  const int cb = a.count_bits;
  const unsigned cmask = (1u << cb) - 1u;
  const double xlx_n = *a.xlx_n;
  const bool use16 = *a.cnt16_bad == 0;
  unsigned long long cand_acc = 0ull;

  int li = blockIdx.x * TEAMS + team;
  if (li >= n_groups) return;
  const int stride = total_teams;
  auto row_at = [&](int g) { const int l = g * S + seg; return bin_rows[list_start + (l < list_n ? l : list_n - 1)]; };
  const unsigned* wp32 = reinterpret_cast<const unsigned*>(a.wp);
  const unsigned* cnt_words = use16 ? reinterpret_cast<const unsigned*>(a.cnt_b16) : reinterpret_cast<const unsigned*>(a.cnt_b);
  int i_cur = row_at(li);
  int i_n1 = row_at(li + stride);
  int i_n2 = row_at(li + 2 * stride);
  int64_t cs1 = a_col_ptr[i_n1], ce1 = a_col_ptr[i_n1 + 1];
  unsigned pf_w1, pf_wp;
  int64_t pf_start;
  int pf_ca;
  double pf_ent;
  int n_cur;
  {
    const int64_t cs0 = a_col_ptr[i_cur], ce0 = a_col_ptr[i_cur + 1];
    n_cur = (int)(ce0 - cs0);
    const int64_t pl = sl < n_cur ? cs0 + sl : ce0 - 1;
    pf_w1 = wp32[2 * ce0];
    pf_wp = wp32[2 * pl];
    pf_start = pstart[pl];
    pf_ca = cnt_a[i_cur];
    pf_ent = ent_a[i_cur];
  }
  URCCO_SETTLE(pf_w1); URCCO_SETTLE(pf_wp); URCCO_SETTLE(pf_start); URCCO_SETTLE(pf_ca); URCCO_SETTLE(pf_ent);
  URCCO_SETTLE(cs1); URCCO_SETTLE(ce1); URCCO_SETTLE(i_n2);
#pragma unroll
  for (int q = 0; q < 4; ++q) tab_w[lane + q * WAVE] = 0u;
  for (; li < n_groups; li += stride) {
    const int i = i_cur;
    const bool live = S == 1 || li * S + seg < list_n;
    const unsigned w0 = S == 1 ? wave_read_lane(pf_wp, 0) : wave_gather(pf_wp, (unsigned)(lane & ~(L - 1)));
    const unsigned total = live ? pf_w1 - w0 : 0u;
    const bool owns_user = live && sl < n_cur;
    const long long ca = (long long)pf_ca;
    const double row_entropy = pf_ent;
    const int64_t my_start = owns_user ? pf_start : 0;
    const unsigned my_off = owns_user ? pf_wp - w0 : total;
    int i_n3 = row_at(li + 3 * stride);
    int64_t cs2 = a_col_ptr[i_n2], ce2 = a_col_ptr[i_n2 + 1];
    n_cur = (int)(ce1 - cs1);
    {
      const int64_t pl = sl < n_cur ? cs1 + sl : ce1 - 1;
      pf_w1 = wp32[2 * ce1];
      pf_wp = wp32[2 * pl];
      pf_start = pstart[pl];
      pf_ca = cnt_a[i_n1];
      pf_ent = ent_a[i_n1];
    }
    marks[sl] = 0u;
    wave_sync();
    if (owns_user) atomicMax(&marks[my_off], (unsigned)sl);
    wave_sync();
    const unsigned o = seg_inclusive_max<L>(marks[sl]);
    const int64_t base_o = wave_gather64(my_start - (int64_t)my_off, (unsigned)(seg * L) + o);
    unsigned slot = 0xffffffffu;
    unsigned jj = 0u;
    if ((unsigned)sl < total) {
      jj = (unsigned)b_col_idx[base_o + sl];
      if (!(dbg & DBG_GATHER_ONLY)) {
        bool ok;
        slot = tab_insert_claim(tab, (jj & colmask) + 1u, cb, (unsigned)(G::TW - 1), 32 - G::LOG2TW, ident, &ok);
        if (!ok) atomicAdd(a.err, 1ull);
      }
    }
    wave_sync();
    const bool is_cand = slot != 0xffffffffu;
    const unsigned long long cand_mask = __ballot(is_cand);
    const unsigned D = (unsigned)__popcll(cand_mask & seg_mask);
    const unsigned D_max = seg_max_popc<L>(cand_mask);
    cand_acc += (unsigned)__popcll(cand_mask);
    unsigned long long mk = 0ull;
    unsigned vv = 0u, cb_raw = 0u;
    if (is_cand) {
      vv = tab[slot];
      tab[slot] = 0u;
      const int j = (int)(vv >> cb) - 1;
      if (!packed) cb_raw = cnt_words[use16 ? j >> 1 : j];
    }
    if (D + (unsigned)sl < (unsigned)G::LIST) {
      kkm[D + (unsigned)sl] = 0ull;
      cand[D + (unsigned)sl] = 0xffffffffu;
    }
    bool in_tables = true;
    if (is_cand) {
      const int j = (int)(vv >> cb) - 1;
      const long long k11 = (long long)(vv & cmask);
      const unsigned cbj = packed ? jj >> cshift : ((dbg & DBG_NO_COUNT_GATHER) ? (unsigned)k11 + 100u : (use16 ? ((j & 1) ? cb_raw >> 16 : cb_raw & 0xffffu) : cb_raw));
      in_tables = llr_operands_in_tables((unsigned)k11, ca, cbj, n_users, col_ent);
    }
    const bool all_in_tables = !(dbg & DBG_NO_LLR) && __ballot(is_cand && !in_tables) == 0ull;
    if (is_cand) {
      const int j = (int)(vv >> cb) - 1;
      const long long k11 = (long long)(vv & cmask);
      if (!(a.exclude_self && j == i)) {
        const unsigned cbj = packed ? jj >> cshift : ((dbg & DBG_NO_COUNT_GATHER) ? (unsigned)k11 + 100u : (use16 ? ((j & 1) ? cb_raw >> 16 : cb_raw & 0xffffu) : cb_raw));
        const double llr = all_in_tables ? llr_from_tables(row_entropy, xlx_n, (unsigned)k11, (unsigned)ca, cbj, xlx_tab, xlx_hi, col_ent)
                                         : ((dbg & DBG_NO_LLR) ? (double)k11
                                                      : llr_of(row_entropy, xlx_n, k11, ca, (long long)cbj, n_users, xlx_tab, xlx_hi, col_ent));
        if (llr > 0.0 && (!a.has_min_llr || llr >= a.min_llr)) mk = (unsigned long long)__double_as_longlong(llr);
      }
      const unsigned pos = lanes_below(cand_mask & seg_mask);
      kkm[pos] = mk;
      cand[pos] = (unsigned)j;
    }
    wave_sync();
    const unsigned long long valid_mask = __ballot(mk != 0ull);
    const int n_valid = __popcll(valid_mask & seg_mask);
    const bool all_fit_k = (int)seg_max_popc<L>(valid_mask) <= a.k;
    auto settle_prefetch = [&]() {
      URCCO_SETTLE(pf_w1); URCCO_SETTLE(pf_wp); URCCO_SETTLE(pf_start); URCCO_SETTLE(pf_ca); URCCO_SETTLE(pf_ent);
      URCCO_SETTLE(cs2); URCCO_SETTLE(ce2); URCCO_SETTLE(i_n3);
// ... 11 lines not shown
      const int64_t obase = ((int64_t)(i - a.item_lo)) * a.k;
      unsigned rank;
      unsigned long long rk;
      unsigned rc;
      unsigned ln = (unsigned)sl;
      URCCO_OPAQUE(ln);
      if (D_max <= (unsigned)(L / 4)) {
        const unsigned c = ln & (unsigned)(L / 4 - 1);
        rk = kkm[c];
        rc = cand[c];
        rank = rank_by_counting_strided<4>(kkm, cand, ln / (unsigned)(L / 4), (D_max + 3u) & ~3u, rk, rc);
        rank += (unsigned)__shfl_xor((int)rank, L / 4);
        rank += (unsigned)__shfl_xor((int)rank, L / 2);
      } else if (D_max <= (unsigned)(L / 2)) {
        const unsigned c = ln & (unsigned)(L / 2 - 1);
        rk = kkm[c];
        rc = cand[c];
        rank = rank_by_counting_strided<2>(kkm, cand, ln / (unsigned)(L / 2), (D_max + 1u) & ~1u, rk, rc);
        rank += (unsigned)__shfl_xor((int)rank, L / 2);
      } else {
        rk = kkm[ln];
        rc = cand[ln];
        rank = rank_by_counting_strided<1>(kkm, cand, 0u, D_max, rk, rc);
      }
      wave_sync();
      const unsigned n_out = (unsigned)(n_valid < a.k ? n_valid : a.k);
      if ((unsigned)sl < D && rk != 0ull && rank < n_out) {
        cand[rank] = rc;
        kkm[rank] = rk;
      }
      wave_sync();
      settle_prefetch();
      if ((unsigned)sl < n_out) {
        out_idx[obase + sl] = (int)cand[sl];
        out_llr[obase + sl] = __longlong_as_double((long long)kkm[sl]);
      }
      if (sl == 0 && live) out_count[i - a.item_lo] = (int)n_out;
    } else {
      settle_prefetch();
    }
    i_cur = i_n1;
    i_n1 = i_n2;
    i_n2 = i_n3;
    cs1 = cs2;
    ce1 = ce2;
    wave_sync();
  }
  if (a.cand && lane == 0 && cand_acc != 0ull) atomicAdd(&a.cand[(blockIdx.x * TEAMS + team) & (CAND_SLOTS - 1)], cand_acc);
}

constexpr int GB_THREADS = 1024;
constexpr int GSEL_K = 1024;

__global__ __launch_bounds__(GB_THREADS) void cco_rows_global_kernel(CcoArgs a) {
  constexpr int NW = GB_THREADS / WAVE;
  __shared__ unsigned long long s_pkey[2][NW];
  __shared__ int s_pcol[2][NW];
  __shared__ int s_ncand;
  __shared__ unsigned s_hist[256];
  __shared__ unsigned s_sel[4];
  __shared__ int s_nsel;
  __shared__ unsigned long long s_selk[GSEL_K];
  __shared__ unsigned s_selc[GSEL_K];
  const int bin = NBINS - 1;
  const int list_start = a.bin_off[bin];
  const int list_n = a.bin_off[bin + 1] - list_start;
  int32_t* cnt = a.g_counts + (int64_t)blockIdx.x * a.n_cols_b;
  unsigned long long* ckey = a.g_cand_key + (int64_t)blockIdx.x * a.n_cols_b;
  int32_t* ccol = a.g_cand_col + (int64_t)blockIdx.x * a.n_cols_b;
  const int lane = threadIdx.x & (WAVE - 1), wv = threadIdx.x / WAVE;
  const int G = 1 << a.g_log2;
  const int grp = threadIdx.x >> a.g_log2, gl = threadIdx.x & (G - 1), ngrp = GB_THREADS >> a.g_log2;
  const double xlx_n = *a.xlx_n;
  for (int li = blockIdx.x; li < list_n; li += gridDim.x) {
    const int i = a.bin_rows[list_start + li];
    const int64_t cs = a.a_col_ptr[i], ce = a.a_col_ptr[i + 1];
    if (threadIdx.x == 0) s_ncand = 0;
    for (int64_t p = cs + grp; p < ce; p += ngrp) {
      const int64_t s = a.pstart[p], e = s + (a.wp[p + 1] - a.wp[p]);
      for (int64_t q = s + gl; q < e; q += G) atomicAdd(&cnt[(unsigned)a.b_col_idx[q] & a.b_col_mask], 1);
    }
    __syncthreads();
    const long long ca = a.cnt_a[i];
    const double row_entropy = a.ent_a[i];
    for (int64_t p = cs + grp; p < ce; p += ngrp) {
      const int64_t s = a.pstart[p], e = s + (a.wp[p + 1] - a.wp[p]);
      for (int64_t q = s + gl; q < e; q += G) {
        const int j = (int)((unsigned)a.b_col_idx[q] & a.b_col_mask);
        const long long k11 = atomicExch(&cnt[j], 0);
        if (k11 > 0 && !(a.exclude_self && j == i)) {
          const long long cbj = a.cnt_b[j];
          const double llr = llr_from_entropies_tab(row_entropy, column_entropy_of(cbj, xlx_n, a.n_users, a.xlx_tab, a.xlx_hi, a.col_ent), xlx_n, k11, ca - k11, cbj - k11,
                                                    a.n_users - ca - cbj + k11, a.xlx_tab, a.n_users, a.xlx_hi);
          if (llr > 0.0 && (!a.has_min_llr || llr >= a.min_llr)) {
            const int pos = atomicAdd(&s_ncand, 1);
            ckey[pos] = (unsigned long long)__double_as_longlong(llr);
            ccol[pos] = j;
          }
        }
      }
    }
    __syncthreads();
    const int ncand = s_ncand;
    const int64_t obase = ((int64_t)(i - a.item_lo)) * a.k;
    if (a.k <= GSEL_K) {
      unsigned long long thr_key = 0ull;
      unsigned thr_ncol = 0u;
      if (ncand > a.k) {
        unsigned need = (unsigned)a.k;
        if (a.col_bytes < 4) thr_ncol = 0xffffffffu << (8 * a.col_bytes);
        const int first_col_pass = 8 + (3 - (a.col_bytes - 1));
        for (int p = 0; p < 12; ++p) {
          if (p >= 8 && p < first_col_pass) continue;
          if (threadIdx.x < 256) s_hist[threadIdx.x] = 0u;
          __syncthreads();
          const int shk = p < 8 ? 56 - 8 * p : 0, shc = p < 8 ? 0 : 24 - 8 * (p - 8);
          for (int t = threadIdx.x; t < ncand; t += GB_THREADS) {
            const unsigned long long key = ckey[t];
            bool match;
            unsigned dig;
            if (p < 8) {
              match = p == 0 || (key >> (shk + 8)) == (thr_key >> (shk + 8));
              dig = (unsigned)(key >> shk) & 255u;
            } else {
              const unsigned ncol = ~(unsigned)ccol[t];
              match = key == thr_key && (p == first_col_pass || (ncol >> (shc + 8)) == (thr_ncol >> (shc + 8)));
              dig = (ncol >> shc) & 255u;
            }
            if (match) atomicAdd(&s_hist[dig], 1u);
          }
          __syncthreads();
          if (threadIdx.x == 0) {
            unsigned above = 0u, d = 255u;
            for (;; --d) {
              if (above + s_hist[d] >= need || d == 0u) break;
              above += s_hist[d];
            }
            s_sel[0] = d;
            s_sel[1] = s_hist[d];
// ... 188 lines not shown
```

### universal-recommender_amd/csrc/urcco_api.hip

```cpp
#include <memory>

#include "urcco_internal.h"

using namespace urcco_detail;

#include <signal.h>
#include <unistd.h>

#include <mutex>

namespace urcco_detail {
char* err_buf() {
  static thread_local char buf[512] = "";
  return buf;
}

const DebugCfg& debug_cfg() {
  static const DebugCfg cfg = [] {
    DebugCfg c;
    const char* m = getenv("URCCO_DEBUG_MARKS");
    const char* p = getenv("URCCO_DEBUG_POISON");
    c.marks = m && *m && *m != '0';
    c.poison = p && *p && *p != '0';
    return c;
// ... 100 lines not shown

const char* urcco_last_error(void) { return err_buf(); }

const char* urcco_status_string(int status) {
  switch (status) {
    case URCCO_OK: return "OK";
    case URCCO_BAD_ARG: return "BAD_ARG";
    case URCCO_OOM_HOST: return "OOM_HOST";
    case URCCO_OOM_DEVICE: return "OOM_DEVICE";
    case URCCO_HIP_ERROR: return "HIP_ERROR";
    case URCCO_INTERNAL: return "INTERNAL";
    case URCCO_NO_DEVICE: return "NO_DEVICE";
    case URCCO_RCCL_ERROR: return "RCCL_ERROR";
    default: return "UNKNOWN";
  }
}

void urcco_debug_dump_marks(void) {
  if (debug_cfg().marks) dump_marks("dump");
}

int urcco_session_create(int32_t device, void* stream, urcco_session** out) {
  if (!out) return fail(URCCO_BAD_ARG, "urcco_session_create: out is NULL");
  *out = nullptr;
  const int n = urcco_device_count();
  if (n <= 0) return fail(URCCO_NO_DEVICE, "no HIP device visible (liburcco has no CPU fallback)");
  if (device < 0 || device >= n) return fail(URCCO_BAD_ARG, "device %d out of range [0,%d)", device, n);
  HIPC(hipSetDevice(device));
  urcco_session* s = new (std::nothrow) urcco_session();
  if (!s) return fail(URCCO_OOM_HOST, "session alloc");
  s->device = device;
  if (stream) {
    s->stream = (hipStream_t)stream;
  } else {
    hipError_t e = hipStreamCreate(&s->stream);
    if (e != hipSuccess) { delete s; return hip_fail(e, "hipStreamCreate"); }
    s->own_stream = true;
  }
  hipDeviceProp_t prop;
  if (hipGetDeviceProperties(&prop, device) == hipSuccess && prop.multiProcessorCount > 0) s->n_cu = prop.multiProcessorCount;
  debug_register(s);
  *out = s;
  return URCCO_OK;
}

void urcco_session_destroy(urcco_session* s) {
  if (!s) return;
  (void)hipSetDevice(s->device);
  (void)hipStreamSynchronize(s->stream);
  debug_unregister(s);
  if (s->arena) (void)hipFree(s->arena);
  if (s->xlx_tab) (void)hipFree(s->xlx_tab);
  if (s->xlx_hi) (void)hipFree(s->xlx_hi);
  if (s->g_counts) { (void)hipFree(s->g_counts); (void)hipFree(s->g_cand_key); (void)hipFree(s->g_cand_col); }
  s->collect();
  for (hipEvent_t e : s->free_events) (void)hipEventDestroy(e);
  if (s->own_stream) (void)hipStreamDestroy(s->stream);
  delete s;
}

int urcco_session_synchronize(urcco_session* s) {
  if (!s) return fail(URCCO_BAD_ARG, "session is NULL");
  HIPC(hipStreamSynchronize(s->stream));
  return URCCO_OK;
}

int urcco_session_set_debug(urcco_session* s, int32_t flags) {
  if (!s) return fail(URCCO_BAD_ARG, "session is NULL");
  s->debug = flags;
  return URCCO_OK;
}

int urcco_session_set_timing(urcco_session* s, int32_t enable) {
  if (!s) return fail(URCCO_BAD_ARG, "session is NULL");
  s->collect();
  s->timing = enable != 0;
  for (int i = 0; i < URCCO_N_STAGES; ++i) { s->acc_ms[i] = 0; s->acc_n[i] = 0; }
  return URCCO_OK;
}

int urcco_session_get_timings(urcco_session* s, double* ms, int64_t* launches) {
  if (!s || !ms || !launches) return fail(URCCO_BAD_ARG, "urcco_session_get_timings: bad argument");
  s->collect();
  for (int i = 0; i < URCCO_N_STAGES; ++i) { ms[i] = s->acc_ms[i]; launches[i] = s->acc_n[i]; }
  return URCCO_OK;
}

int64_t urcco_session_scratch_bytes(const urcco_session* s) {
  if (!s) return 0;
  return (int64_t)s->arena_cap + (int64_t)s->g_cap * 16;
}

int urcco_dev_column_counts(urcco_session* s, int64_t nnz, const int32_t* col_idx, int32_t n_cols, int32_t* counts) {
  if (!s || nnz < 0 || n_cols < 0 || (nnz > 0 && !col_idx) || (n_cols > 0 && !counts)) return fail(URCCO_BAD_ARG, "urcco_dev_column_counts: bad argument");
  if (n_cols == 0) return URCCO_OK;
  const int64_t ph_bytes = urcco::column_counts_scratch_bytes(nnz, n_cols);
  if (ph_bytes > 0) URC(s->reserve((size_t)ph_bytes));
  s->begin(URCCO_STAGE_COLUMN_COUNTS);
  if (ph_bytes > 0)
    HIPC(urcco::launch_column_counts_partitioned(s->stream, col_idx, nnz, nullptr, n_cols, counts, s->take<char>((size_t)ph_bytes)));
  else
    HIPC(urcco::launch_column_counts(s->stream, s->n_cu, col_idx, nnz, n_cols, counts));
  s->end();
  return URCCO_OK;
}

int urcco_dev_downsample(urcco_session* s, int64_t n_rows, const int64_t* row_ptr, const int32_t* col_idx, int64_t nnz, int32_t n_cols,
                         const int32_t* raw_counts, int32_t seed, int32_t max_elements_per_row, int32_t row_rate_mode, int64_t row_base,
                         int64_t* out_row_ptr, int32_t* out_col_idx, int32_t* post_counts) {
  if (!s || n_rows < 0 || nnz < 0 || n_cols < 0 || !row_ptr || !out_row_ptr || (nnz > 0 && (!col_idx || !raw_counts || !out_col_idx)))
    return fail(URCCO_BAD_ARG, "urcco_dev_downsample: bad argument");
  if (max_elements_per_row <= 0) return fail(URCCO_BAD_ARG, "maxElementsPerRow must be positive, got %d", max_elements_per_row);
  if ((row_rate_mode & ~URCCO_RNG_MIX32) != URCCO_ROW_RATE_MAHOUT_INT_DIV && (row_rate_mode & ~URCCO_RNG_MIX32) != URCCO_ROW_RATE_FRACTIONAL)
    return fail(URCCO_BAD_ARG, "unknown row_rate_mode %d", row_rate_mode);
  if (post_counts && n_cols > 0) HIPC(hipMemsetAsync(post_counts, 0, sizeof(int32_t) * (size_t)n_cols, s->stream));
  if (nnz == 0) {
    HIPC(hipMemsetAsync(out_row_ptr, 0, sizeof(int64_t) * (size_t)(n_rows + 1), s->stream));
    return URCCO_OK;
  }
  const int64_t ph_bytes = post_counts ? urcco::column_counts_scratch_bytes(nnz, n_cols) : 0;
  const int64_t ds_tiles = (nnz + urcco::DS_TILE - 1) / urcco::DS_TILE;
  const size_t n_words = (size_t)ds_tiles * (urcco::DS_TILE / 64);
// ... 20 lines not shown
    HIPC(urcco::launch_column_counts_partitioned(s->stream, out_col_idx, nnz, out_row_ptr + n_rows, n_cols, post_counts, s->take<char>((size_t)ph_bytes)));
    s->end();
  }
  return URCCO_OK;
}

int urcco_dev_transpose(urcco_session* s, int64_t n_rows, const int64_t* row_ptr, const int32_t* col_idx, int64_t nnz, int32_t n_cols,
                        const int32_t* counts, int32_t col_lo, int32_t col_hi, int64_t* out_col_ptr, int32_t* out_row_idx) {
  if (!s || n_rows < 0 || nnz < 0 || n_cols < 0 || !row_ptr || !out_col_ptr || (n_cols > 0 && !counts) || (nnz > 0 && (!col_idx || !out_row_idx)) ||
      col_lo < 0 || col_hi < col_lo || col_hi > n_cols)
    return fail(URCCO_BAD_ARG, "urcco_dev_transpose: bad argument");
  const int64_t n_tiles = ((int64_t)n_cols + urcco::SCAN_TILE - 1) / urcco::SCAN_TILE;
  const int64_t tr_bytes = urcco::transpose_scratch_bytes(n_rows, nnz, n_cols);
  URC(s->reserve(urcco_session::need((size_t)n_cols, 4) + urcco_session::need((size_t)n_tiles + 2, 8) + (size_t)tr_bytes + 256));
  int32_t* cursor = s->take<int32_t>((size_t)n_cols);
  int64_t* tile_sums = s->take<int64_t>((size_t)n_tiles + 2);
  s->begin(URCCO_STAGE_TRANSPOSE);
  HIPC(urcco::launch_scan_i32_range(s->stream, counts, n_cols, col_lo, col_hi, out_col_ptr, tile_sums));
  if (nnz > 0 && n_rows > 0) {
    int g = ceil_log2_i64((nnz + n_rows - 1) / n_rows);
    if (g < 1) g = 1;
    if (g > 6) g = 6;
    HIPC(hipMemsetAsync(cursor, 0, sizeof(int32_t) * (size_t)n_cols, s->stream));
    if (tr_bytes > 0) {
      HIPC(urcco::launch_transpose_partitioned(s->stream, n_rows, row_ptr, col_idx, nnz, n_cols, out_col_ptr, cursor, out_row_idx, col_lo, col_hi,
                                               s->take<char>((size_t)tr_bytes)));
    } else {
      HIPC(urcco::launch_transpose(s->stream, s->n_cu, n_rows, row_ptr, col_idx, g, out_col_ptr, cursor, out_row_idx, col_lo, col_hi));
    }
  }
  s->end();
  return URCCO_OK;
}

int urcco_dev_row_work_csr(urcco_session* s, int64_t n_rows, const int64_t* a_row_ptr, const int32_t* a_col_idx, int64_t nnz_a, const int64_t* b_row_ptr,
                           int32_t n_items_a, int64_t* work) {
  if (!s || n_rows < 0 || nnz_a < 0 || n_items_a < 0 || !a_row_ptr || !b_row_ptr || (nnz_a > 0 && !a_col_idx) || (n_items_a > 0 && !work))
    return fail(URCCO_BAD_ARG, "urcco_dev_row_work_csr: bad argument");
  int g = n_rows > 0 ? ceil_log2_i64((nnz_a + n_rows - 1) / n_rows) : 1;
  if (g < 1) g = 1;
  if (g > 6) g = 6;
  s->begin(URCCO_STAGE_ROW_WORK);
  HIPC(urcco::launch_row_work_csr(s->stream, s->n_cu, n_rows, a_row_ptr, a_col_idx, b_row_ptr, g, n_items_a, work));
  s->end();
  return URCCO_OK;
}

int urcco_dev_row_work(urcco_session* s, int32_t item_lo, int32_t item_hi, int32_t n_items_a, const int64_t* a_col_ptr, const int32_t* a_row_idx,
                       int64_t nnz_a_bound, const int64_t* b_row_ptr, int64_t* work) {
  if (!s || item_lo < 0 || item_hi < item_lo || item_hi > n_items_a || nnz_a_bound < 0 || !a_col_ptr || !b_row_ptr || (item_hi > item_lo && !work))
    return fail(URCCO_BAD_ARG, "urcco_dev_row_work: bad argument");
  const int64_t cap = nnz_a_bound;
  const int64_t n_tiles = (cap + urcco::SCAN_TILE - 1) / urcco::SCAN_TILE;
  URC(s->reserve(urcco_session::need((size_t)cap, 8) + urcco_session::need((size_t)cap, 4) + urcco_session::need((size_t)cap + 1, 8) +
                 urcco_session::need((size_t)n_tiles + 2, 8)));
  int64_t* pstart = s->take<int64_t>((size_t)cap);
  int32_t* plen = s->take<int32_t>((size_t)cap);
  int64_t* wp = s->take<int64_t>((size_t)cap + 1);
  int64_t* tile_sums = s->take<int64_t>((size_t)n_tiles + 2);
  s->begin(URCCO_STAGE_ROW_WORK);
  HIPC(urcco::launch_expand_prepare(s->stream, s->n_cu, a_col_ptr, n_items_a, a_row_idx, b_row_ptr, nullptr, 0, cap, pstart, plen, wp, tile_sums));
  HIPC(urcco::launch_row_work(s->stream, s->n_cu, item_lo, item_hi, a_col_ptr, wp, work));
  s->end();
  return URCCO_OK;
}

int urcco_dev_partition(urcco_session* s, int32_t n_items, const int64_t* work, int32_t n_parts, int32_t* bounds_host) {
  if (!s || n_items < 0 || n_parts <= 0 || n_parts > 4096 || !bounds_host || (n_items > 0 && !work)) return fail(URCCO_BAD_ARG, "urcco_dev_partition: bad argument");
  int32_t* bounds = nullptr;
  URC(urcco_detail::partition_dev(s, n_items, work, n_parts, nullptr, &bounds));
  HIPC(hipMemcpyAsync(bounds_host, bounds, sizeof(int32_t) * (size_t)(n_parts + 1), hipMemcpyDeviceToHost, s->stream));
  HIPC(hipStreamSynchronize(s->stream));
  return URCCO_OK;
}

int urcco_dev_merge_fragments(urcco_session* s, int32_t world, int32_t item_lo, int32_t item_hi, int32_t n_items, const void* lens, int32_t wire16,
                              const int32_t* entries, int64_t n_entries, const int64_t* sizes, const int32_t* counts, int64_t* out_col_ptr,
                              int32_t* out_row_idx) {
  if (!s || world <= 0 || item_lo < 0 || item_hi < item_lo || item_hi > n_items || n_entries < 0 || !sizes || !out_col_ptr || (n_items > 0 && !counts) ||
      (item_hi > item_lo && !lens) || (n_entries > 0 && (!entries || !out_row_idx)))
    return fail(URCCO_BAD_ARG, "urcco_dev_merge_fragments: bad argument");
  const int32_t n_range = item_hi - item_lo;
  const int64_t n_runs = (int64_t)world * n_range;
  const int64_t t_items = ((int64_t)n_items + urcco::SCAN_TILE - 1) / urcco::SCAN_TILE, t_runs = (n_runs + urcco::SCAN_TILE - 1) / urcco::SCAN_TILE;
  URC(s->reserve(urcco_session::need((size_t)n_runs + 1, 8) + urcco_session::need((size_t)(t_items > t_runs ? t_items : t_runs) + 2, 8)));
  int64_t* src_off = s->take<int64_t>((size_t)n_runs + 1);
  int64_t* tile_sums = s->take<int64_t>((size_t)(t_items > t_runs ? t_items : t_runs) + 2);
  s->begin(URCCO_STAGE_TRANSPOSE);
  HIPC(urcco::launch_scan_i32_range(s->stream, counts, n_items, item_lo, item_hi, out_col_ptr, tile_sums));
  if (wire16) {
    HIPC(urcco::launch_scan_u16(s->stream, static_cast<const unsigned short*>(lens), n_runs, src_off, tile_sums));
  } else {
    HIPC(urcco::launch_scan_i32(s->stream, static_cast<const int32_t*>(lens), n_runs, src_off, tile_sums));
  }
  HIPC(urcco::launch_frag_place(s->stream, s->n_cu, world, item_lo, n_range, lens, wire16, src_off, entries, out_col_ptr, sizes, out_row_idx));
  s->end();
  return URCCO_OK;
}

int urcco_dev_cco_rows(urcco_session* s, int32_t item_lo, int32_t item_hi, int32_t n_items_a, const int64_t* a_col_ptr,
                       const int32_t* a_row_idx, int64_t nnz_a_bound, const int64_t* b_row_ptr, const int32_t* b_col_idx, int32_t n_cols_b,
                       const int32_t* counts_a, const int32_t* counts_b, int64_t n_users, int32_t exclude_self, int32_t k,
                       int32_t has_min_llr, double min_llr, int32_t* out_count, int32_t* out_idx, double* out_llr, int64_t* stats_dev) {
  return urcco_detail::cco_rows_impl(s, item_lo, item_hi, n_items_a, a_col_ptr, a_row_idx, nnz_a_bound, b_row_ptr, b_col_idx, n_cols_b, counts_a, counts_b, n_users,
                                     exclude_self, k, has_min_llr, min_llr, out_count, out_idx, out_llr, stats_dev, nullptr, nullptr);
}

int urcco_dev_pack_counts(urcco_session* s, int64_t n_rows_b, const int64_t* b_row_ptr, const int32_t* b_col_idx, int64_t nnz_b_bound, const int32_t* counts_b,
                          int32_t n_cols_b, int32_t* out_packed, int32_t* out_bad) {
  return urcco_detail::pack_counts(s, b_row_ptr, n_rows_b, b_col_idx, nnz_b_bound, counts_b, n_cols_b, out_packed, out_bad);
}

int urcco_dev_cco_rows_packed(urcco_session* s, int32_t item_lo, int32_t item_hi, int32_t n_items_a, const int64_t* a_col_ptr,
                              const int32_t* a_row_idx, int64_t nnz_a_bound, const int64_t* b_row_ptr, const int32_t* b_col_idx, int32_t n_cols_b,
                              const int32_t* counts_a, const int32_t* counts_b, int64_t n_users, int32_t exclude_self, int32_t k,
                              int32_t has_min_llr, double min_llr, int32_t* out_count, int32_t* out_idx, double* out_llr, int64_t* stats_dev,
                              const int32_t* b_packed, const int32_t* pack_bad) {
  if ((b_packed == nullptr) != (pack_bad == nullptr)) return fail(URCCO_BAD_ARG, "urcco_dev_cco_rows_packed: b_packed and pack_bad come together");
  return urcco_detail::cco_rows_impl(s, item_lo, item_hi, n_items_a, a_col_ptr, a_row_idx, nnz_a_bound, b_row_ptr, b_col_idx, n_cols_b, counts_a, counts_b, n_users,
                                     exclude_self, k, has_min_llr, min_llr, out_count, out_idx, out_llr, stats_dev, nullptr, nullptr, nullptr, b_packed, pack_bad);
}

}

namespace urcco_detail {

int partition_dev(urcco_session* s, int32_t n_items, const int64_t* work, int32_t n_parts, int32_t* bounds_dev, int32_t** bounds_out) {
  const int64_t n_tiles = ((int64_t)n_items + urcco::SCAN_TILE - 1) / urcco::SCAN_TILE;
  URC(s->reserve(urcco_session::need((size_t)n_items + 1, 8) + urcco_session::need((size_t)n_tiles + 2, 8) + urcco_session::need((size_t)n_parts + 1, 4)));
  int64_t* prefix = s->take<int64_t>((size_t)n_items + 1);
  int64_t* tile_sums = s->take<int64_t>((size_t)n_tiles + 2);
  int32_t* bounds = bounds_dev ? bounds_dev : s->take<int32_t>((size_t)n_parts + 1);
  HIPC(urcco::launch_scan_i64(s->stream, work, n_items, prefix, tile_sums));
  HIPC(urcco::launch_partition(s->stream, n_items, prefix, n_parts, bounds));
  if (bounds_out) *bounds_out = bounds;
  return URCCO_OK;
}

int cco_rows_impl(urcco_session* s, int32_t item_lo, int32_t item_hi, int32_t n_items_a, const int64_t* a_col_ptr, const int32_t* a_row_idx, int64_t nnz_a_bound,
                  const int64_t* b_row_ptr, const int32_t* b_col_idx, int32_t n_cols_b, const int32_t* counts_a, const int32_t* counts_b, int64_t n_users,
                  int32_t exclude_self, int32_t k, int32_t has_min_llr, double min_llr, int32_t* out_count, int32_t* out_idx, double* out_llr, int64_t* stats_dev,
                  const int64_t* pre_pstart, const int32_t* pre_plen, int64_t* pre_tile_sums, const int32_t* b_packed, const int32_t* pack_bad, bool pk_known) {
  if (!s || item_lo < 0 || item_hi < item_lo || item_hi > n_items_a || n_cols_b < 0 || n_users < 0 || nnz_a_bound < 0 || !a_col_ptr || !b_row_ptr)
    return fail(URCCO_BAD_ARG, "urcco_dev_cco_rows: bad argument");
  if (k <= 0) return fail(URCCO_BAD_ARG, "maxInterestingElements must be positive, got %d", k);
  const int32_t n = item_hi - item_lo;
  if (n == 0) {
    if (stats_dev) HIPC(hipMemsetAsync(stats_dev, 0, sizeof(int64_t) * URCCO_STATS_LEN, s->stream));
    return URCCO_OK;
  }
  if (!out_count || !out_idx || !out_llr || !counts_a || (n_cols_b > 0 && !counts_b)) return fail(URCCO_BAD_ARG, "urcco_dev_cco_rows: NULL buffer");
  HIPC(hipMemsetAsync(out_count, 0, sizeof(int32_t) * (size_t)n, s->stream));
  if (n_cols_b == 0 || n_users == 0) {
    if (stats_dev) HIPC(hipMemsetAsync(stats_dev, 0, sizeof(int64_t) * URCCO_STATS_LEN, s->stream));
    return URCCO_OK;
  }
  int key_bits = 1;
  while (((int64_t)1 << key_bits) <= (int64_t)n_cols_b) ++key_bits;
  const int count_bits = 32 - key_bits;
  if (count_bits < 1) return fail(URCCO_BAD_ARG, "n_cols_b %d too large for the packed accumulator", n_cols_b);
  const bool dense_bin6 = k > urcco::MP_KMAX_HOST || 3ll * k + 5 > 32768ll;
  if (dense_bin6) URC(s->ensure_global_bin(n_cols_b));
  if (!s->xlx_tab) {
    HIPC(hipMalloc((void**)&s->xlx_tab, sizeof(double) * urcco::XLX_TABLE_HOST));
    HIPC(urcco::launch_xlx_table(s->stream, s->xlx_tab));
  }
  if (!s->xlx_hi) HIPC(hipMalloc((void**)&s->xlx_hi, sizeof(double) * 2 * urcco::XLX_TABLE_HOST));
  if (s->xlx_hi_n != n_users) {
    HIPC(urcco::launch_xlx_hi_table(s->stream, s->xlx_hi, s->xlx_tab, n_users));
    s->xlx_hi_n = n_users;
  }
  const int64_t n_tiles = ((int64_t)n + urcco::BIN_TILE - 1) / urcco::BIN_TILE;
  const int64_t cap = nnz_a_bound;
  const int64_t p_tiles = (cap + urcco::SCAN_TILE - 1) / urcco::SCAN_TILE;
  URC(s->reserve(urcco_session::need((size_t)cap, 8) + urcco_session::need((size_t)cap, 4) + urcco_session::need((size_t)cap + 1, 8) +
                 urcco_session::need((size_t)p_tiles + 2, 8) +
                 urcco_session::need((size_t)n, 8) + urcco_session::need((size_t)(n_tiles + 1) * urcco::BIN_COLS_HOST, 8) +
                 urcco_session::need(urcco::BIN_OFF_LEN, 4) + urcco_session::need((size_t)n, 4) + urcco_session::need((size_t)n_items_a, 8) +
                 urcco_session::need((size_t)n_cols_b, 2) + urcco_session::need(1, 4) + urcco_session::need(urcco::CAND_SLOTS, 8) + urcco_session::need(1, 8) + urcco_session::need(URCCO_STATS_LEN, 8) +
                 urcco_session::need((size_t)n_users + 1, 4)));
  int64_t* own_pstart = s->take<int64_t>((size_t)cap);
  int32_t* own_plen = s->take<int32_t>((size_t)cap);
  const int64_t* pstart = pre_pstart ? pre_pstart : own_pstart;
  int64_t* wp = s->take<int64_t>((size_t)cap + 1);
  int64_t* p_tile_sums = s->take<int64_t>((size_t)p_tiles + 2);
  int64_t* work = s->take<int64_t>((size_t)n);
  int64_t* tile_counts = s->take<int64_t>((size_t)(n_tiles + 1) * urcco::BIN_COLS_HOST);
  int32_t* bin_off = s->take<int32_t>(urcco::BIN_OFF_LEN);
  int32_t* bin_rows = s->take<int32_t>((size_t)n);
  double* ent_a = s->take<double>((size_t)n_items_a);
  unsigned short* cnt_b16 = s->take<unsigned short>((size_t)n_cols_b);
  int32_t* cnt16_bad = s->take<int32_t>(1);
  unsigned long long* cand = s->take<unsigned long long>(urcco::CAND_SLOTS);
  double* xlx_n = s->take<double>(1);
  int64_t* stats = stats_dev ? stats_dev : s->take<int64_t>(URCCO_STATS_LEN);
  unsigned* b_rp32 = s->take<unsigned>((size_t)n_users + 1);

  s->begin(URCCO_STAGE_ROW_WORK);
  if (pre_pstart && pre_plen)
    HIPC(urcco::launch_expand_scan(s->stream, a_col_ptr, n_items_a, pre_plen, cap, wp, pre_tile_sums ? pre_tile_sums : p_tile_sums, pre_tile_sums != nullptr));
  else
    HIPC(urcco::launch_expand_prepare(s->stream, s->n_cu, a_col_ptr, n_items_a, a_row_idx, b_row_ptr, b_rp32, n_users, cap, own_pstart, own_plen, wp, p_tile_sums));
  HIPC(urcco::launch_row_work(s->stream, s->n_cu, item_lo, item_hi, a_col_ptr, wp, work));
  s->end();
  s->begin(URCCO_STAGE_BINNING);
  HIPC(hipMemsetAsync(stats, 0, sizeof(int64_t) * URCCO_STATS_LEN, s->stream));
  HIPC(urcco::launch_binning(s->stream, item_lo, n, work, counts_a, n_cols_b, count_bits, k, tile_counts, bin_off, bin_rows, stats));
  s->end();
  s->begin(URCCO_STAGE_ENTROPY);
  HIPC(urcco::launch_item_entropy(s->stream, counts_a, n_items_a, n_users, ent_a, xlx_n));
  HIPC(urcco::launch_narrow_counts(s->stream, s->n_cu, counts_b, n_cols_b, cnt_b16, cnt16_bad));
  s->end();

  urcco::CcoArgs a;
  a.bin_rows = bin_rows; a.bin_off = bin_off;
  a.a_col_ptr = a_col_ptr; a.pstart = pstart; a.wp = wp; a.b_col_idx = b_col_idx;
  a.b_packed = pk_known ? b_col_idx : ((b_packed && pack_bad && !(s->debug & urcco::DBG_UNPACKED_COUNTS)) ? b_packed : nullptr);
  a.pack_bad = pack_bad;
  a.pk_known = pk_known ? 1 : 0;
  a.b_col_mask = pk_known ? (key_bits >= 32 ? 0xffffffffu : (1u << key_bits) - 1u) : 0xffffffffu;
  a.cnt_a = counts_a; a.cnt_b = counts_b; a.ent_a = ent_a; a.cnt_b16 = cnt_b16; a.cnt16_bad = cnt16_bad; a.xlx_n = xlx_n; a.xlx_tab = s->xlx_tab; a.xlx_hi = s->xlx_hi; a.col_ent = s->xlx_hi + urcco::XLX_TABLE_HOST; a.debug = s->debug;
  a.n_users = n_users; a.n_cols_b = n_cols_b; a.item_lo = item_lo; a.exclude_self = exclude_self ? 1 : 0; a.k = k;
  a.has_min_llr = has_min_llr ? 1 : 0; a.min_llr = min_llr; a.count_bits = count_bits;
  a.col_bytes = n_cols_b <= (1 << 8) ? 1 : (n_cols_b <= (1 << 16) ? 2 : (n_cols_b <= (1 << 24) ? 3 : 4));
  a.unordered = s->unordered_rows ? 1 : 0;
  a.g_log2 = 4;
  a.out_count = out_count; a.out_idx = out_idx; a.out_llr = out_llr;
  a.err = reinterpret_cast<unsigned long long*>(stats + 1 + 4 * urcco::NBINS);
  a.cand = s->timing ? cand : nullptr;
  if (s->timing) HIPC(hipMemsetAsync(cand, 0, sizeof(unsigned long long) * urcco::CAND_SLOTS, s->stream));
  a.g_counts = s->g_counts; a.g_cand_key = s->g_cand_key; a.g_cand_col = s->g_cand_col; a.g_blocks = dense_bin6 ? s->g_blocks : 0;
  for (int step = 0; step < urcco::NBINS; ++step) {
    const int bin = urcco::NBINS - 1 - step;
    s->begin(URCCO_STAGE_CCO_BIN0 + bin);
    HIPC(urcco::launch_cco_rows_bin(s->stream, s->n_cu, a, bin, n));
    s->end();
  }
  if (s->timing) HIPC(urcco::launch_bin_out_stats(s->stream, bin_rows, bin_off, item_lo, out_count, cand, stats));
  return URCCO_OK;
}

int pack_counts(urcco_session* s, const int64_t* b_row_ptr, int64_t n_rows_b, const int32_t* b_col_idx, int64_t nnz_bound, const int32_t* counts_b, int32_t n_cols_b,
                int32_t* out, int32_t* bad) {
  if (!s || !b_row_ptr || n_rows_b < 0 || nnz_bound < 0 || !out || !bad || (nnz_bound > 0 && (!b_col_idx || !counts_b))) return fail(URCCO_BAD_ARG, "pack_counts: bad argument");
  int key_bits = 1;
  while (((int64_t)1 << key_bits) <= (int64_t)n_cols_b) ++key_bits;
  const int count_bits = 32 - key_bits;
  if (count_bits < 1) return fail(URCCO_BAD_ARG, "n_cols_b %d too large for the packed accumulator", n_cols_b);
  URC(s->reserve(urcco_session::need((size_t)n_cols_b + 8, 2) + urcco_session::need(1, 4) + 256));
  unsigned short* c16 = s->take<unsigned short>((size_t)n_cols_b + 8);
  int32_t* bad16 = s->take<int32_t>(1);
  s->begin(URCCO_STAGE_ENTROPY);
  HIPC(urcco::launch_narrow_counts(s->stream, s->n_cu, counts_b, n_cols_b, c16, bad16));
  HIPC(urcco::launch_pack_counts(s->stream, s->n_cu, b_col_idx, b_row_ptr + n_rows_b, nnz_bound, c16, bad16, count_bits, out, bad));
  s->end();
  return URCCO_OK;
}

int expand_multi(urcco_session* s, int n, const int64_t* a_col_ptr, int32_t n_items_a, const int32_t* a_row_idx, int64_t cap, const int64_t* const* b_row_ptr,
                 int64_t n_users, int64_t* const* pstart, int32_t* const* plen, int64_t* const* tile_sums) {
  if (!s || n < 1 || n > urcco::EXPAND_MULTI_MAX || !a_col_ptr || cap < 0) return fail(URCCO_BAD_ARG, "expand_multi: bad argument");
  URC(s->reserve(urcco_session::need(((size_t)n_users + 2) * (size_t)n, 4) + 256));
  void* T = s->take<unsigned>(((size_t)n_users + 2) * (size_t)n);
  s->begin(URCCO_STAGE_ROW_WORK);
  HIPC(urcco::launch_expand_prepare_multi(s->stream, s->n_cu, a_col_ptr, n_items_a, a_row_idx, n, b_row_ptr, n_users, cap, pstart, plen, T, tile_sums));
  s->end();
  return URCCO_OK;
}

}

extern "C" {

int urcco_dev_compact_indicators(urcco_session* s, int32_t n_rows, int32_t k, const int32_t* count, const int32_t* idx, const double* llr,
                                 int64_t* out_row_ptr, int32_t* out_col_idx, double* out_llr) {
  if (!s || n_rows < 0 || k <= 0 || !out_row_ptr || (n_rows > 0 && (!count || !idx || !llr || !out_col_idx || !out_llr)))
    return fail(URCCO_BAD_ARG, "urcco_dev_compact_indicators: bad argument");
  const int64_t n_tiles = ((int64_t)n_rows + urcco::SCAN_TILE - 1) / urcco::SCAN_TILE;
  URC(s->reserve(urcco_session::need((size_t)n_tiles + 2, 8)));
  int64_t* tile_sums = s->take<int64_t>((size_t)n_tiles + 2);
  s->begin(URCCO_STAGE_COMPACT_INDICATORS);
  HIPC(urcco::launch_scan_i32(s->stream, count, n_rows, out_row_ptr, tile_sums));
  HIPC(urcco::launch_compact_indicators(s->stream, n_rows, k, count, idx, llr, out_row_ptr, out_col_idx, out_llr));
  s->end();
  return URCCO_OK;
}

struct urcco_key_table {
  urcco::KeyTable t{};
  int64_t capacity = 0;
  int device = 0;
};

void urcco_key_table_destroy(urcco_key_table* table) {
  if (!table) return;
  (void)hipSetDevice(table->device);
  if (table->t.keys) (void)hipFree(table->t.keys);
  if (table->t.minpos) (void)hipFree(table->t.minpos);
  if (table->t.count) (void)hipFree(table->t.count);
  if (table->t.id) (void)hipFree(table->t.id);
  delete table;
}

int urcco_dev_dictionary_build(urcco_session* s, int64_t n, const uint64_t* keys, const int32_t* select, int32_t min_count,
                               int64_t* first_pos, urcco_key_table** table, int64_t* n_ids) {
  if (!s || n < 0 || (n > 0 && (!keys || !first_pos)) || !table || !n_ids) return fail(URCCO_BAD_ARG, "urcco_dev_dictionary_build: bad argument");
  if (n >= ((int64_t)1 << 32) - 1) return fail(URCCO_BAD_ARG, "urcco_dev_dictionary_build: at most 2^32 - 2 events per stream, got %lld", (long long)n);
  *table = nullptr;
  std::unique_ptr<urcco_key_table, void (*)(urcco_key_table*)> tab(new (std::nothrow) urcco_key_table(), urcco_key_table_destroy);
  if (!tab) return fail(URCCO_OOM_HOST, "key table alloc");
  tab->device = s->device;
  int64_t cap = 1024;
  while (cap < 2 * n) cap <<= 1;
// ... 178 lines not shown
```

### universal-recommender_amd/csrc/urcco_context.hip

```cpp
#include <dlfcn.h>

#include <algorithm>
#include <atomic>
#include <chrono>
#include <condition_variable>
#include <functional>
#include <memory>
#include <future>
#include <mutex>
#include <string>
#include <thread>
#include <unordered_map>

#include "urcco_internal.h"

using namespace urcco_detail;

namespace {

struct Rccl {
  typedef struct { char internal[URCCO_UNIQUE_ID_BYTES]; } UniqueId;
  typedef void* Comm;
  void* handle = nullptr;
  int (*GetUniqueId)(UniqueId*) = nullptr;
// ... 98 lines not shown
      }
    return false;
  }
  void trim() {
    std::lock_guard<std::mutex> g(mu);
    std::vector<Block> keep;
    for (Block& b : blocks) {
      if (b.used) keep.push_back(b);
      else (void)hipHostFree(b.p);
    }
    blocks.swap(keep);
  }
};
PinnedPool& pinned_pool() {
  static PinnedPool* pool = new PinnedPool();
  return *pool;
}

constexpr int A_SETS = 2;

struct EvState {
  urcco_session* s = nullptr;
  DBuf<int64_t> in_rp;
  DBuf<int32_t> in_ci;
  DBuf<int32_t> raw, post;
  DBuf<int64_t> s_rp;
  DBuf<int32_t> s_ci;
  DBuf<int32_t> deg, f_deg;
  DBuf<unsigned short> deg16, f_deg16;
  DBuf<int64_t> f_rp;
  DBuf<int32_t> f_ci;
  DBuf<int64_t> sizes;
  DBuf<int64_t> scan_tmp;
  DBuf<int32_t> o_count, o_idx;
  DBuf<double> o_llr;
  DBuf<int64_t> c_rp;
  DBuf<int32_t> c_idx;
  DBuf<double> c_llr;
  DBuf<int64_t> stats;
  DBuf<unsigned long long> verr;
  DBuf<int32_t> b_pk;
  DBuf<int32_t> pk_bad;
  DBuf<int32_t> s_pk;
  bool b_pk_known = false;
  uint32_t b_col_mask = 0xffffffffu;
  unsigned long long* h_verr = nullptr;
  unsigned long long* h_verr_dev = nullptr;
  int ensure_h_verr() {
    if (h_verr) return URCCO_OK;
    HIPC(hipHostMalloc((void**)&h_verr, sizeof(unsigned long long), hipHostMallocMapped | hipHostMallocCoherent));
    HIPC(hipHostGetDevicePointer((void**)&h_verr_dev, h_verr, 0));
    return URCCO_OK;
  }
  DBuf<int64_t> pre_pstart;
  DBuf<int32_t> pre_plen;
  DBuf<int64_t> pre_tsum;
  DBuf<int32_t> mlen, pack;
  DBuf<unsigned short> mlen16;
  DBuf<int32_t> mlen_bad;
  DBuf<int64_t> moff, mtmp, to_nnz;
  hipEvent_t ev_sampled = nullptr, ev_done = nullptr, ev_rp = nullptr;
  hipEvent_t ev_cons[A_SETS] = {};
  bool cons_valid[A_SETS] = {};
  const int64_t* b_rp = nullptr;
  const int32_t* b_ci = nullptr;
  int64_t b_rows = 0, b_nnz_bound = 0;
  void release() {
    in_rp.release(); in_ci.release(); raw.release(); post.release(); s_rp.release(); s_ci.release(); deg.release(); f_deg.release();
    deg16.release(); f_deg16.release();
    f_rp.release(); f_ci.release(); sizes.release(); scan_tmp.release(); o_count.release(); o_idx.release(); o_llr.release(); c_rp.release();
    c_idx.release(); c_llr.release(); stats.release(); verr.release(); b_pk.release(); pk_bad.release(); s_pk.release(); pre_pstart.release(); pre_plen.release(); pre_tsum.release();
    mlen.release(); pack.release(); mlen16.release(); mlen_bad.release(); moff.release(); mtmp.release(); to_nnz.release();
    if (h_verr) (void)hipHostFree(h_verr);
    h_verr = nullptr;
    h_verr_dev = nullptr;
    if (ev_sampled) (void)hipEventDestroy(ev_sampled);
    if (ev_done) (void)hipEventDestroy(ev_done);
    if (ev_rp) (void)hipEventDestroy(ev_rp);
    for (int q = 0; q < A_SETS; ++q) {
      if (ev_cons[q]) (void)hipEventDestroy(ev_cons[q]);
      ev_cons[q] = nullptr;
      cons_valid[q] = false;
    }
    ev_sampled = ev_done = ev_rp = nullptr;
  }
};

struct DevState {
  int device = 0;
  int rank = 0;
  int n_cu = 256;
  std::vector<urcco_session*> sessions;
  std::vector<EvState> ev;
  DBuf<int64_t> a_cp[A_SETS];
  DBuf<int32_t> a_ri[A_SETS];
  DBuf<int32_t> a_post[A_SETS];
  int par = 0;
  DBuf<int64_t> work;
  DBuf<int32_t> bounds;
  DBuf<int32_t> l_cnt, l_ri, len_bad, f_ent;
  DBuf<int64_t> l_cp, rec;
  DBuf<unsigned short> len16;
  DBuf<char> f_len;
  DBuf<unsigned long long> need;
  hipEvent_t need_ready = nullptr;
  hipEvent_t a_ready = nullptr, in_ready = nullptr, b_expanded = nullptr;
  Rccl::Comm comm = nullptr;
// ... 232 lines not shown
    D.sessions.push_back(s);
  }
  if ((int)D.ev.size() < n_ds) D.ev.resize((size_t)n_ds);
  for (int d = 0; d < n_ds; ++d) {
    EvState& E = D.ev[(size_t)d];
    E.s = sess_of(c, D, d);
    E.s->unordered_rows = (c->flags & URCCO_FLAG_UNORDERED_ROWS) ? 1 : 0;
    if (!E.ev_sampled) HIPC(hipEventCreateWithFlags(&E.ev_sampled, hipEventDisableTiming));
    if (!E.ev_done) HIPC(hipEventCreateWithFlags(&E.ev_done, hipEventDisableTiming));
    for (int q = 0; q < A_SETS; ++q)
      if (!E.ev_cons[q]) HIPC(hipEventCreateWithFlags(&E.ev_cons[q], hipEventDisableTiming));
    if (!E.ev_rp) HIPC(hipEventCreateWithFlags(&E.ev_rp, hipEventDisableTiming));
  }
  if (!D.a_ready) HIPC(hipEventCreateWithFlags(&D.a_ready, hipEventDisableTiming));
  if (!D.in_ready) HIPC(hipEventCreateWithFlags(&D.in_ready, hipEventDisableTiming));
  if (!D.b_expanded) HIPC(hipEventCreateWithFlags(&D.b_expanded, hipEventDisableTiming));
  if (!D.need_ready) HIPC(hipEventCreateWithFlags(&D.need_ready, hipEventDisableTiming));
  return URCCO_OK;
}

int stage_raw_counts(DevState& D, EvState& E, const Shard& sh, const DsParams& p) {
  URC(E.raw.ensure((size_t)p.n_cols + 1));
  return urcco_dev_column_counts(E.s, sh.nnz, sh.ci, (int32_t)p.n_cols, E.raw.p);
}
DBuf<int32_t>& post_of(DevState& D, int d) { return d == 0 ? D.a_post[D.par] : D.ev[(size_t)d].post; }

int stage_downsample(urcco_context* c, DevState& D, int d, const Shard& sh, const DsParams& p, int32_t seed) {
  EvState& E = D.ev[(size_t)d];
  URC(E.s_rp.ensure((size_t)sh.n_rows + 1));
  URC(E.s_ci.ensure((size_t)sh.nnz + 4));
  URC(post_of(D, d).ensure((size_t)p.n_cols + 1));
  return urcco_dev_downsample(E.s, sh.n_rows, sh.rp, sh.ci, sh.nnz, (int32_t)p.n_cols, E.raw.p, seed, p.max_rows, c->row_rate_mode, sh.row_base, E.s_rp.p,
                              E.s_ci.p, post_of(D, d).p);
}

int stage_rows(DevState& D, EvState& E, EvState& A, int d, const DsParams& pa, const DsParams& p, int64_t n_users, int64_t a_nnz_bound, bool pre_expanded = false) {
  const int32_t n = D.item_hi - D.item_lo;
  const size_t strided = (size_t)(n > 0 ? n : 1) * (size_t)p.k;
  URC(E.o_count.ensure((size_t)n + 1));
  URC(E.o_idx.ensure(strided));
  URC(E.o_llr.ensure(strided));
  URC(E.c_rp.ensure((size_t)n + 2));
  URC(E.c_idx.ensure(strided));
  URC(E.c_llr.ensure(strided));
  URC(E.stats.ensure(URCCO_STATS_LEN));
  if (!E.b_pk_known) {
    URC(E.b_pk.ensure((size_t)E.b_nnz_bound + 4));
    URC(E.pk_bad.ensure(1));
    URC(pack_counts(E.s, E.b_rp, E.b_rows, E.b_ci, E.b_nnz_bound, post_of(D, d).p, (int32_t)p.n_cols, E.b_pk.p, E.pk_bad.p));
  }
  URC(cco_rows_impl(E.s, D.item_lo, D.item_hi, (int32_t)pa.n_cols, D.a_cp[D.par].p, D.a_ri[D.par].p, a_nnz_bound, E.b_rp, E.b_ci, (int32_t)p.n_cols,
                    post_of(D, 0).p, post_of(D, d).p, n_users, d == 0 ? 1 : 0, p.k, p.has_min_llr, p.min_llr, E.o_count.p, E.o_idx.p, E.o_llr.p, E.stats.p,
                    pre_expanded ? E.pre_pstart.p : nullptr, pre_expanded ? E.pre_plen.p : nullptr, pre_expanded ? E.pre_tsum.p : nullptr,
                    E.b_pk_known ? nullptr : E.b_pk.p, E.b_pk_known ? nullptr : E.pk_bad.p, E.b_pk_known));
  URC(urcco_dev_compact_indicators(E.s, n, p.k, E.o_count.p, E.o_idx.p, E.o_llr.p, E.c_rp.p, E.c_idx.p, E.c_llr.p));
  HIPC(hipEventRecord(E.ev_done, E.s->stream));
  HIPC(hipEventRecord(E.ev_cons[D.par], E.s->stream));
  E.cons_valid[D.par] = true;
  return URCCO_OK;
}

struct InputGate {
  const HostTrace* trace = nullptr;
  std::function<int(int)> after_chain;
  std::vector<int> order;
  std::vector<std::promise<int>> staged;
  std::vector<std::shared_future<int>> fut;
  std::vector<char> released;
  explicit InputGate(int n) : staged((size_t)n), fut((size_t)n), released((size_t)n, 0) {
    for (int d = 0; d < n; ++d) fut[(size_t)d] = staged[(size_t)d].get_future().share();
  }
  void release(int d, int status) {
    released[(size_t)d] = 1;
    staged[(size_t)d].set_value(status);
  }
  int wait(DevState& D, int d) {
    const int st = fut[(size_t)d].get();
    if (st != URCCO_OK) return fail(st, "dataset %d: staging failed", d);
    EvState& E = D.ev[(size_t)d];
    HIPC(hipStreamSynchronize(E.s->stream));
    const unsigned long long bad = E.h_verr ? *(volatile unsigned long long*)E.h_verr : 0ull;
    if (bad)
      return fail(URCCO_BAD_ARG, "dataset %d: %llu invalid entries (row_ptr not monotone, or col_idx out of [0, n_cols) / not strictly increasing inside a row)", d, bad);
    if (trace) trace->mark("matrices landed and checked", d);
    return URCCO_OK;
  }
};

int build_single(urcco_context* c, DevState& D, const std::vector<Shard>& sh, const std::vector<DsParams>& ps_, int64_t n_users, int32_t seed,
                 InputGate* gate) {
  const int n_ds = (int)sh.size();
  URC(set_dev(D));
  EvState& A = D.ev[0];
  D.item_lo = 0;
  D.item_hi = (int32_t)ps_[0].n_cols;
  URC(D.a_cp[D.par].ensure((size_t)ps_[0].n_cols + 2));
  URC(D.a_ri[D.par].ensure((size_t)sh[0].nnz + 4));
  std::atomic<bool> a_ok{false};
  const bool threaded = n_ds > 1 && !c->single_stream();
  std::promise<void> a_recorded;
  std::shared_future<void> a_recorded_f = a_recorded.get_future().share();
  bool fuse = n_ds >= 3 && n_ds - 1 <= urcco::EXPAND_MULTI_MAX && !(c->debug & urcco::DBG_UNFUSED_EXPAND) && gate == nullptr;
  for (int d = 1; d < n_ds; ++d) fuse = fuse && sh[(size_t)d].nnz < ((int64_t)1 << 32);
  const bool fold = fuse && n_ds <= urcco::EXPAND_MULTI_MAX && sh[0].nnz < ((int64_t)1 << 32);
  const int f0 = fold ? 0 : 1;
  std::vector<std::promise<int>> sampled((size_t)n_ds);
  std::vector<std::shared_future<int>> sampled_f((size_t)n_ds);
  for (int d = 0; d < n_ds; ++d) sampled_f[(size_t)d] = sampled[(size_t)d].get_future().share();
  std::promise<int> expanded;
  std::shared_future<int> expanded_f = expanded.get_future().share();
  const int64_t a_cap = sh[0].nnz;
  auto fused_expand = [&]() -> int {
    EvState& L = D.ev[1];
    if (L.s != A.s) HIPC(hipStreamWaitEvent(L.s->stream, D.a_ready, 0));
    std::vector<const int64_t*> rp((size_t)(n_ds - f0));
    std::vector<int64_t*> ps((size_t)(n_ds - f0));
    std::vector<int32_t*> pl((size_t)(n_ds - f0));
    std::vector<int64_t*> ts((size_t)(n_ds - f0));
    for (int d = f0; d < n_ds; ++d) {
      EvState& E = D.ev[(size_t)d];
      if (d > 0 && E.s != L.s) HIPC(hipStreamWaitEvent(L.s->stream, E.ev_sampled, 0));
      URC(E.pre_pstart.ensure((size_t)a_cap + 1));
      URC(E.pre_plen.ensure((size_t)a_cap + 1));
      URC(E.pre_tsum.ensure(expand_tile_words(a_cap)));
      ts[(size_t)(d - f0)] = E.pre_tsum.p;
      rp[(size_t)(d - f0)] = E.s_rp.p;
      ps[(size_t)(d - f0)] = E.pre_pstart.p;
      pl[(size_t)(d - f0)] = E.pre_plen.p;
    }
    URC(expand_multi(L.s, n_ds - f0, D.a_cp[D.par].p, (int32_t)ps_[0].n_cols, D.a_ri[D.par].p, a_cap, rp.data(), n_users, ps.data(), pl.data(), ts.data()));
    HIPC(hipEventRecord(D.b_expanded, L.s->stream));
    return URCCO_OK;
  };
  auto sample_secondary = [&](int d) -> int {
    URC(set_dev(D));
    EvState& E = D.ev[(size_t)d];
    if (gate) URC(gate->wait(D, d));
    URC(stage_raw_counts(D, E, sh[(size_t)d], ps_[(size_t)d]));
    URC(stage_downsample(c, D, d, sh[(size_t)d], ps_[(size_t)d], seed));
    HIPC(hipEventRecord(E.ev_sampled, E.s->stream));
    return URCCO_OK;
  };
  auto rows_secondary = [&](int d) -> int {
    EvState& E = D.ev[(size_t)d];
    if (E.s != A.s) HIPC(hipStreamWaitEvent(E.s->stream, D.a_ready, 0));
    if (fuse && E.s != D.ev[1].s) HIPC(hipStreamWaitEvent(E.s->stream, D.b_expanded, 0));
    E.b_rp = E.s_rp.p;
    E.b_ci = E.s_ci.p;
    E.b_pk_known = false;
    E.b_col_mask = 0xffffffffu;
    E.b_rows = sh[(size_t)d].n_rows;
    E.b_nnz_bound = sh[(size_t)d].nnz;
    URC(stage_rows(D, E, A, d, ps_[0], ps_[(size_t)d], n_users, sh[0].nnz, fuse));
    if (gate && gate->trace) gate->trace->mark("chain enqueued", d);
    if (threaded && gate && gate->after_chain) URC(gate->after_chain(d));
    return URCCO_OK;
  };
  struct Fulfil {
    std::promise<int>* p;
    bool done = false;
    void set(int v) { if (p && !done) { done = true; p->set_value(v); } }
    ~Fulfil() { set(URCCO_INTERNAL); }
  };
  auto secondary_thread = [&](int d) -> int {
    Fulfil my_sample{fuse ? &sampled[(size_t)d] : nullptr};
    Fulfil my_expand{fuse && d == 1 ? &expanded : nullptr};
    int st = sample_secondary(d);
    my_sample.set(st);
    if (st == URCCO_OK) a_recorded_f.wait();
// ... 439 lines not shown
    URC(exchange_phase(c, 0, sh, ps, n_users, sizes, &fp));
  } else {
    c->h_bounds.assign((size_t)W + 1, 0);
    for (DevState& D : c->devs) {
      URC(set_dev(D));
      std::vector<int32_t> b((size_t)W + 1);
      URC(urcco_dev_partition(D.ev[0].s, n_items_a, D.work.p, W, b.data()));
      c->h_bounds = b;
      D.item_lo = b[(size_t)D.rank];
      D.item_hi = b[(size_t)D.rank + 1];
    }
    URC(exchange_phase(c, 0, sh, ps, n_users, sizes));
  }
  c->h_sizes.assign((size_t)n_ds, 0);
  int64_t a_nnz = 0;
  for (int r = 0; r < W; ++r) a_nnz += sizes[(size_t)XS * r + 1];
  c->h_sizes[0] = a_nnz;
  URC(c->workers->run([&](size_t g) -> int {
    DevState& D = c->devs[g];
    URC(set_dev(D));
    EvState& A = D.ev[0];
    URC(D.a_cp[D.par].ensure((size_t)n_items_a + 2));
    if (fp.on) {
      int64_t ents = 0;
      for (int p = 0; p < W; ++p) ents += fp.cpb[(size_t)p * (size_t)(W + 1) + (size_t)D.rank + 1] - fp.cpb[(size_t)p * (size_t)(W + 1) + (size_t)D.rank];
      D.a_ents = ents;
      URC(D.a_ri[D.par].ensure((size_t)ents + 4));
      URC(urcco_dev_merge_fragments(A.s, W, D.item_lo, D.item_hi, n_items_a, D.f_len.p, fp.wire16 ? 1 : 0, D.f_ent.p, ents, A.sizes.p, post_of(D, 0).p,
                                    D.a_cp[D.par].p, D.a_ri[D.par].p));
    } else {
      D.a_ents = a_nnz;
      URC(D.a_ri[D.par].ensure((size_t)a_nnz + 4));
      URC(urcco_dev_transpose(A.s, n_users, A.f_rp.p, A.f_ci.p, a_nnz, n_items_a, post_of(D, 0).p, D.item_lo, D.item_hi, D.a_cp[D.par].p, D.a_ri[D.par].p));
    }
    HIPC(hipEventRecord(D.a_ready, A.s->stream));
    return stage_rows(D, A, A, 0, ps[0], ps[0], n_users, D.a_ents);
  }));
  for (int d = 1; d < n_ds; ++d) URC(input_phase(c, d, sh, ps, seed));
  std::vector<int64_t> b_nnz((size_t)n_ds, 0);
  for (int d = 1; d < n_ds; ++d) {
    URC(exchange_phase(c, d, sh, ps, n_users, sizes));
    for (int r = 0; r < W; ++r) b_nnz[(size_t)d] += sizes[(size_t)XS * r + 1];
    c->h_sizes[(size_t)d] = b_nnz[(size_t)d];
  }
  bool fuse = n_ds >= 3 && n_ds - 1 <= urcco::EXPAND_MULTI_MAX && !(c->debug & urcco::DBG_UNFUSED_EXPAND);
  for (int d = 1; d < n_ds; ++d) fuse = fuse && b_nnz[(size_t)d] < ((int64_t)1 << 32);
  URC(c->workers->run([&](size_t g) -> int {
    DevState& D = c->devs[g];
    URC(set_dev(D));
    if (fuse && D.a_ents > 0) {
      EvState& L = D.ev[1];
      if (L.s != D.ev[0].s) HIPC(hipStreamWaitEvent(L.s->stream, D.a_ready, 0));
      std::vector<const int64_t*> rp((size_t)n_ds - 1);
      std::vector<int64_t*> pst((size_t)n_ds - 1);
      std::vector<int32_t*> pl((size_t)n_ds - 1);
      std::vector<int64_t*> ts((size_t)n_ds - 1);
      for (int d = 1; d < n_ds; ++d) {
        EvState& E = D.ev[(size_t)d];
        HIPC(hipEventRecord(E.ev_sampled, E.s->stream));
        if (E.s != L.s) HIPC(hipStreamWaitEvent(L.s->stream, E.ev_sampled, 0));
        URC(E.pre_pstart.ensure((size_t)D.a_ents + 1));
        URC(E.pre_plen.ensure((size_t)D.a_ents + 1));
        URC(E.pre_tsum.ensure(expand_tile_words(D.a_ents)));
        ts[(size_t)d - 1] = E.pre_tsum.p;
        rp[(size_t)d - 1] = E.b_rp;
        pst[(size_t)d - 1] = E.pre_pstart.p;
        pl[(size_t)d - 1] = E.pre_plen.p;
      }
      URC(expand_multi(L.s, n_ds - 1, D.a_cp[D.par].p, n_items_a, D.a_ri[D.par].p, D.a_ents, rp.data(), n_users, pst.data(), pl.data(), ts.data()));
      HIPC(hipEventRecord(D.b_expanded, L.s->stream));
    }
    for (int d = 1; d < n_ds; ++d) {
      EvState& E = D.ev[(size_t)d];
      if (E.s != D.ev[0].s) HIPC(hipStreamWaitEvent(E.s->stream, D.a_ready, 0));
      if (fuse && D.a_ents > 0 && E.s != D.ev[1].s) HIPC(hipStreamWaitEvent(E.s->stream, D.b_expanded, 0));
      URC(stage_rows(D, E, D.ev[0], d, ps[0], ps[(size_t)d], n_users, D.a_ents, fuse && D.a_ents > 0));
    }
    return URCCO_OK;
  }));
  return URCCO_OK;
}

int check_params(const DsParams& p, int d) {
  if (p.n_cols < 0 || p.n_cols > 0x7ffffff0ll) return fail(URCCO_BAD_ARG, "dataset %d: bad column count", d);
  if (p.max_rows <= 0 || p.k <= 0) return fail(URCCO_BAD_ARG, "dataset %d: maxElementsPerRow / maxInterestingElements must be positive", d);
  return URCCO_OK;
}

int run_build(urcco_context* c, const std::vector<std::vector<Shard>>& sh, const std::vector<DsParams>& ps, int64_t n_users, int32_t seed,
              hipStream_t input_stream, InputGate* gate = nullptr) {
  const int n_ds = (int)ps.size();
  for (DevState& D : c->devs) {
    if (!gate) URC(ensure_events(c, D, n_ds));
    D.par = (D.par + 1) % A_SETS;
    for (size_t d = 1; d < D.ev.size(); ++d)
      if (D.ev[d].cons_valid[D.par] && D.ev[d].s != D.ev[0].s) HIPC(hipStreamWaitEvent(D.ev[0].s->stream, D.ev[d].ev_cons[D.par], 0));
    if (input_stream && c->devs.size() == 1) {
      HIPC(hipEventRecord(D.in_ready, input_stream));
      for (int d = 0; d < n_ds; ++d) HIPC(hipStreamWaitEvent(D.ev[(size_t)d].s->stream, D.in_ready, 0));
    }
  }
  if (!c->exchange()) return build_single(c, c->devs[0], [&] {
    std::vector<Shard> one((size_t)n_ds);
    for (int d = 0; d < n_ds; ++d) one[(size_t)d] = sh[(size_t)d][0];
    return one;
  }(), ps, n_users, seed, gate);
  return build_sharded(c, sh, ps, n_users, seed);
// ... 748 lines not shown
```

### universal-recommender_amd/csrc/urcco_internal.h

```cpp
#pragma once
#include <hip/hip_runtime.h>

#include <cstdarg>
#include <cstdio>
#include <cstdlib>
#include <cstring>
#include <new>
#include <vector>

#include "../../include/urcco.h"
#include "cco_kernels.h"
static_assert(urcco::EXCH_SIZES == URCCO_EXCH_SIZES && urcco::STATS_LEN == URCCO_STATS_LEN, "include/urcco.h and cco_kernels.h agree");
static_assert(urcco::REC_MAX_CLAUSES == URCCO_REC_MAX_CLAUSES && urcco::REC_MAX_NUM == URCCO_REC_MAX_NUM && urcco::REC_NO_BACKFILL == URCCO_REC_NO_BACKFILL &&
                  urcco::REC_STATS_LEN == URCCO_REC_STATS_LEN && urcco::REC_MAX_RULES == URCCO_REC_MAX_RULES && urcco::REC_RULE_ANY == URCCO_RULE_ANY &&
                  urcco::REC_RULE_NONE == URCCO_RULE_NONE && urcco::REC_RULE_RANGE == URCCO_RULE_RANGE,
              "include/urcco.h and cco_kernels.h agree on the recommendation call");

struct urcco_session;
namespace urcco_detail {

char* err_buf();

inline int fail(int status, const char* fmt, ...) {
  va_list ap;
// ... 3 lines not shown
  return status;
}

inline int hip_fail(hipError_t e, const char* what) {
  return fail(e == hipErrorOutOfMemory ? URCCO_OOM_DEVICE : URCCO_HIP_ERROR, "%s: %s", what, hipGetErrorString(e));
}

#define HIPC(expr)                                                  \
  do {                                                              \
    hipError_t _e = (expr);                                         \
    if (_e != hipSuccess) return urcco_detail::hip_fail(_e, #expr); \
  } while (0)

#define URC(expr)                  \
  do {                             \
    int _s = (expr);               \
    if (_s != URCCO_OK) return _s; \
  } while (0)

template <typename F>
inline int guarded(F&& body) {
  try {
    return body();
  } catch (const std::bad_alloc&) {
    return fail(URCCO_OOM_HOST, "out of host memory");
  } catch (const std::exception& e) {
    return fail(URCCO_INTERNAL, "unexpected exception: %s", e.what());
  } catch (...) {
    return fail(URCCO_INTERNAL, "unexpected exception");
  }
}

inline size_t align_up(size_t v, size_t a) { return (v + a - 1) / a * a; }

struct DebugCfg { bool marks = false, poison = false; };
const DebugCfg& debug_cfg();
void debug_mark(urcco_session* s, int which , int stage);
void debug_register(urcco_session* s);
void debug_unregister(urcco_session* s);
void debug_poison(void* p, size_t bytes, hipStream_t st, bool async);

inline int ceil_log2_i64(int64_t v) {
  int l = 0;
  while (((int64_t)1 << l) < v) ++l;
  return l;
}

}

namespace urcco_detail {
int cco_rows_impl(urcco_session* s, int32_t item_lo, int32_t item_hi, int32_t n_items_a, const int64_t* a_col_ptr, const int32_t* a_row_idx, int64_t nnz_a_bound,
                  const int64_t* b_row_ptr, const int32_t* b_col_idx, int32_t n_cols_b, const int32_t* counts_a, const int32_t* counts_b, int64_t n_users,
                  int32_t exclude_self, int32_t k, int32_t has_min_llr, double min_llr, int32_t* out_count, int32_t* out_idx, double* out_llr, int64_t* stats_dev,
                  const int64_t* pre_pstart, const int32_t* pre_plen, int64_t* pre_tile_sums = nullptr ,
                  const int32_t* b_packed = nullptr , const int32_t* pack_bad = nullptr ,
                  bool pk_known = false );
int pack_counts(urcco_session* s, const int64_t* b_row_ptr, int64_t n_rows_b, const int32_t* b_col_idx, int64_t nnz_bound, const int32_t* counts_b, int32_t n_cols_b,
                int32_t* out, int32_t* bad);
int partition_dev(urcco_session* s, int32_t n_items, const int64_t* work, int32_t n_parts, int32_t* bounds_dev, int32_t** bounds_out);
int expand_multi(urcco_session* s, int n, const int64_t* a_col_ptr, int32_t n_items_a, const int32_t* a_row_idx, int64_t cap, const int64_t* const* b_row_ptr,
                 int64_t n_users, int64_t* const* pstart, int32_t* const* plen, int64_t* const* tile_sums = nullptr );
inline size_t expand_tile_words(int64_t cap) { return (size_t)((cap + urcco::SCAN_TILE - 1) / urcco::SCAN_TILE + 2); }
}

using namespace urcco_detail;

struct urcco_session {
  int device = 0;
  hipStream_t stream = nullptr;
  bool own_stream = false;
  int n_cu = 256;
  char* arena = nullptr;
  size_t arena_cap = 0;
  size_t arena_off = 0;
  int32_t* g_counts = nullptr;
  unsigned long long* g_cand_key = nullptr;
  int32_t* g_cand_col = nullptr;
  int64_t g_cols = 0;
  double* xlx_tab = nullptr;
  double* xlx_hi = nullptr;
  long long xlx_hi_n = -1;
  int debug = 0;
  unsigned* marks = nullptr;
  unsigned mark_seq = 0;
  int unordered_rows = 0;
  bool timing = false;
  struct Rec { int stage; hipEvent_t e0, e1; };
  std::vector<Rec> recs;
  std::vector<hipEvent_t> free_events;
  double acc_ms[URCCO_N_STAGES] = {0};
  int64_t acc_n[URCCO_N_STAGES] = {0};

  hipEvent_t get_event() noexcept {
    if (!free_events.empty()) { hipEvent_t e = free_events.back(); free_events.pop_back(); return e; }
    hipEvent_t e = nullptr;
    (void)hipEventCreate(&e);
    return e;
  }
  void begin(int stage) noexcept {
    cur_stage = stage;
    if (marks) debug_mark(this, 0, stage);
    if (!timing) return;
    try {
      recs.reserve(recs.size() + 1);
      free_events.reserve(free_events.size() + 2 * (recs.size() + 1));
    } catch (...) {
      open_rec = false;
      return;
    }
    Rec r{stage, get_event(), get_event()};
    if (!r.e0 || !r.e1) { open_rec = false; return; }
    (void)hipEventRecord(r.e0, stream);
    recs.push_back(r);
    open_rec = true;
  }
  bool open_rec = false;
  int cur_stage = 0;
  void end() noexcept {
    if (marks) debug_mark(this, 1, cur_stage);
    if (!timing || !open_rec || recs.empty()) return;
    (void)hipEventRecord(recs.back().e1, stream);
    open_rec = false;
  }
  void collect() {
    (void)hipStreamSynchronize(stream);
    for (const Rec& r : recs) {
      float ms = 0.f;
      if (hipEventElapsedTime(&ms, r.e0, r.e1) == hipSuccess) { acc_ms[r.stage] += ms; acc_n[r.stage] += 1; }
      free_events.push_back(r.e0);
      free_events.push_back(r.e1);
    }
    recs.clear();
  }

  int reserve(size_t bytes) {
// ... 73 lines not shown
```

### universal-recommender_amd/device.py

```python
from __future__ import annotations

import ctypes as C
from dataclasses import dataclass, field
from typing import List, Optional, Sequence

import torch

from . import _lib


@dataclass
class DatasetParams:
    max_elements_per_row: int = 500
    max_interesting_elements: int = 50
    min_llr: Optional[float] = None


@dataclass
class DevCsr:
    n_rows: int
    n_cols: int
    row_ptr: torch.Tensor
    col_idx: torch.Tensor
    nnz_bound: int
# ... 20 lines not shown

    def to_host(self):
        if self.row_ptr.numel() == 0:
            import numpy as np
            return np.zeros(1, np.int64), np.zeros(0, np.int32), np.zeros(0, np.float64)
        rp = self.row_ptr.cpu().numpy()
        nnz = int(rp[-1])
        return rp, self.col_idx[:nnz].cpu().numpy(), self.llr[:nnz].cpu().numpy()


def _ptr(t: Optional[torch.Tensor]) -> Optional[int]:
    return None if t is None else t.data_ptr()


class DeviceSession:

    def __init__(self, device: torch.device, library=None, stream: Optional["torch.cuda.Stream"] = None):
        self.device = torch.device(device)
        self.lib = library if library is not None else _lib.lib()
        self.pack_counts = True
        self.torch_stream = None
        handle = C.c_void_p()
        if self.device.type == "cuda":
            index = self.device.index if self.device.index is not None else torch.cuda.current_device()
            self.device = torch.device("cuda", index)
            self.torch_stream = stream if stream is not None else torch.cuda.current_stream(self.device)
            self._check(self.lib.urcco_session_create(index, C.c_void_p(self.torch_stream.cuda_stream), C.byref(handle)))
        else:
            self._check(self.lib.urcco_session_create(0, None, C.byref(handle)))
        self.handle = handle

    def _check(self, status: int):
        _lib.check(status, self.lib)

    def close(self):
        if self.handle:
            self.lib.urcco_session_destroy(self.handle)
            self.handle = C.c_void_p()

    def __del__(self):
        try:
            self.close()
        except Exception:
            pass

    def synchronize(self):
        self._check(self.lib.urcco_session_synchronize(self.handle))

    def set_timing(self, enable: bool):
        self._check(self.lib.urcco_session_set_timing(self.handle, int(enable)))

    def set_debug(self, flags: int):
        self._check(self.lib.urcco_session_set_debug(self.handle, int(flags)))

    def get_timings(self):
        ms = (C.c_double * _lib.N_STAGES)()
        n = (C.c_int64 * _lib.N_STAGES)()
        self._check(self.lib.urcco_session_get_timings(self.handle, ms, n))
        return {_lib.STAGE_NAMES[i]: (ms[i], n[i]) for i in range(_lib.N_STAGES) if _lib.STAGE_NAMES[i]}

    def empty(self, n, dtype):
        return torch.empty(int(n), dtype=dtype, device=self.device)

    def column_counts(self, col_idx: torch.Tensor, nnz: int, n_cols: int, out: Optional[torch.Tensor] = None) -> torch.Tensor:
        out = out if out is not None else self.empty(n_cols, torch.int32)
        self._check(self.lib.urcco_dev_column_counts(self.handle, nnz, _ptr(col_idx), n_cols, _ptr(out)))
        return out

    def downsample(self, m: DevCsr, nnz: int, raw_counts: torch.Tensor, seed: int, max_elements_per_row: int,
                   row_rate_mode: int = _lib.ROW_RATE_MAHOUT_INT_DIV, row_base: int = 0, post_out: Optional[torch.Tensor] = None):
        out_rp = self.empty(m.n_rows + 1, torch.int64)
        out_ci = self.empty(max(nnz, 1), torch.int32)
        post = post_out if post_out is not None else self.empty(max(m.n_cols, 1), torch.int32)
        self._check(self.lib.urcco_dev_downsample(self.handle, m.n_rows, _ptr(m.row_ptr), _ptr(m.col_idx), nnz, m.n_cols, _ptr(raw_counts),
                                                 _to_i32(seed), max_elements_per_row, row_rate_mode, row_base, _ptr(out_rp), _ptr(out_ci),
                                                 _ptr(post)))
        return DevCsr(m.n_rows, m.n_cols, out_rp, out_ci, nnz), post

    def transpose(self, m: DevCsr, counts: torch.Tensor, col_lo: int = 0, col_hi: Optional[int] = None):
        col_hi = m.n_cols if col_hi is None else col_hi
        col_ptr = self.empty(m.n_cols + 1, torch.int64)
        row_idx = self.empty(max(m.nnz_bound, 1), torch.int32)
        self._check(self.lib.urcco_dev_transpose(self.handle, m.n_rows, _ptr(m.row_ptr), _ptr(m.col_idx), m.nnz_bound, m.n_cols, _ptr(counts),
                                                col_lo, col_hi, _ptr(col_ptr), _ptr(row_idx)))
        return col_ptr, row_idx

    def merge_fragments(self, world: int, item_lo: int, item_hi: int, n_items: int, lens: torch.Tensor, entries: torch.Tensor, n_entries: int,
                        sizes: torch.Tensor, counts: torch.Tensor):
        assert lens.dtype in (torch.uint16, torch.int16, torch.int32)
        col_ptr = self.empty(n_items + 1, torch.int64)
        row_idx = self.empty(max(n_entries, 1), torch.int32)
        self._check(self.lib.urcco_dev_merge_fragments(self.handle, world, item_lo, item_hi, n_items, _ptr(lens), int(lens.dtype != torch.int32), _ptr(entries),
                                                      n_entries, _ptr(sizes), _ptr(counts), _ptr(col_ptr), _ptr(row_idx)))
        return col_ptr, row_idx

    def row_work_csr(self, a: DevCsr, b_row_ptr: torch.Tensor) -> torch.Tensor:
        work = self.empty(max(a.n_cols, 1), torch.int64)
        self._check(self.lib.urcco_dev_row_work_csr(self.handle, a.n_rows, _ptr(a.row_ptr), _ptr(a.col_idx), a.nnz_bound, _ptr(b_row_ptr), a.n_cols,
                                                   _ptr(work)))
        return work[: a.n_cols]

    def row_work(self, item_lo: int, item_hi: int, n_items_a: int, a_col_ptr, a_row_idx, nnz_a_bound: int, b_row_ptr) -> torch.Tensor:
        work = self.empty(max(item_hi - item_lo, 1), torch.int64)
        self._check(self.lib.urcco_dev_row_work(self.handle, item_lo, item_hi, n_items_a, _ptr(a_col_ptr), _ptr(a_row_idx), nnz_a_bound,
                                                _ptr(b_row_ptr), _ptr(work)))
        return work[: item_hi - item_lo]
# ... 279 lines not shown
```

Measured before the change: 34.43 billion pairs/s.

## Narrow expansion prefix and pair-start arrays to 32-bit with device-side form flag

Stores the per-pair start offsets as 32-bit values and, when a device-computed form word shows no overflow, writes the work prefix scan as 32-bit words, reconstructing 64-bit values from tile sums. The goal is to halve memory traffic for the pstart and work-prefix arrays in the expansion and CCO stages. A fused scan-tiles kernel sets overflow/pack/host flags into the form word so downstream kernels choose the narrow or wide path at runtime. Test hooks are added to force the limit and seed the prefix. This adds per-kernel branching and the risk of reconstruction errors at tile boundaries.

```diff
diff --git a/include/urcco.h b/include/urcco.h
--- a/include/urcco.h
+++ b/include/urcco.h
@@ -193,6 +193,8 @@
 };
 int urcco_session_set_timing(urcco_session* s, int32_t enable);
 int urcco_session_set_debug(urcco_session* s, int32_t flags);
+int urcco_session_expand_form(urcco_session* s, int32_t* form_host);
+int urcco_session_set_expand_test(urcco_session* s, int64_t limit, int64_t prefix_seed);
 int urcco_session_get_timings(urcco_session* s, double* ms , int64_t* launches );
 int64_t urcco_session_scratch_bytes(const urcco_session* s);
 void urcco_debug_dump_marks(void);
diff --git a/universal-recommender_amd/_lib.py b/universal-recommender_amd/_lib.py
--- a/universal-recommender_amd/_lib.py
+++ b/universal-recommender_amd/_lib.py
@@ -144,6 +144,8 @@
     "urcco_session_scratch_bytes": (C.c_int64, [_p]),
     "urcco_session_set_timing": (C.c_int, [_p, C.c_int32]),
     "urcco_session_set_debug": (C.c_int, [_p, C.c_int32]),
+    "urcco_session_expand_form": (C.c_int, [_p, C.POINTER(C.c_int32)]),
+    "urcco_session_set_expand_test": (C.c_int, [_p, C.c_int64, C.c_int64]),
     "urcco_debug_dump_marks": (None, []),
     "urcco_session_get_timings": (C.c_int, [_p, C.POINTER(C.c_double), C.POINTER(C.c_int64)]),
     "urcco_dev_column_counts": (C.c_int, [_p, C.c_int64, _p, C.c_int32, _p]),
diff --git a/universal-recommender_amd/csrc/cco_common.h b/universal-recommender_amd/csrc/cco_common.h
--- a/universal-recommender_amd/csrc/cco_common.h
+++ b/universal-recommender_amd/csrc/cco_common.h
@@ -111,15 +111,20 @@
 
 constexpr int ST_THREADS = 1024;
 constexpr int ST_ITEMS = 8;
-static __global__ __launch_bounds__(ST_THREADS) void scan_tiles_kernel(int64_t* __restrict__ tile_sums, int64_t n_tiles, const int64_t* __restrict__ n_live) {
+static __global__ __launch_bounds__(ST_THREADS) void scan_tiles_kernel(int64_t* __restrict__ tile_sums, int64_t n_tiles, const int64_t* __restrict__ n_live,
+                                                                       ExpandForm form) {
   __shared__ long long s_wave[ST_THREADS / WAVE];
+  __shared__ int s_over;
+  if (threadIdx.x == 0) s_over = 0;
+  __syncthreads();
+  bool over = false;
   const int lane = threadIdx.x & (WAVE - 1), wave = threadIdx.x / WAVE;
   int64_t live_tiles = n_tiles;
   if (n_live) {
     const int64_t lt = *n_live / SCAN_TILE + 1;
     if (lt < live_tiles) live_tiles = lt;
   }
-  long long carry = 0;
+  long long carry = form.seed;
   for (int64_t base = 0; base < live_tiles; base += ST_THREADS * ST_ITEMS) {
     const int64_t first = base + (int64_t)threadIdx.x * ST_ITEMS;
     long long x[ST_ITEMS];
@@ -128,6 +133,7 @@
     for (int q = 0; q < ST_ITEMS; ++q) {
       x[q] = first + q < live_tiles ? tile_sums[first + q] : 0;
       sum += x[q];
+      over = over || (unsigned long long)x[q] >= form.limit;
     }
     long long inc = sum;
 #pragma unroll
@@ -155,6 +161,18 @@
   }
   for (int64_t t = live_tiles + threadIdx.x; t < n_tiles; t += ST_THREADS) tile_sums[t] = carry;
   if (threadIdx.x == 0) tile_sums[n_tiles] = carry;
+  if (form.word) {
+    if (over) s_over = 1;
+    __syncthreads();
+    if (threadIdx.x == 0) {
+      int f = form.host_narrow ? 0 : *form.word;
+      if (form.host_narrow) s_over = 0;
+      if (s_over) f |= FORM_TILE;
+      if (form.pack_bad && *form.pack_bad != 0) f |= FORM_PACK;
+      if (form.host_wide) f |= FORM_HOST;
+      *form.word = f ? (f | FORM_WIDE) : 0;
+    }
+  }
 }
 
 template <typename Load>
@@ -255,7 +273,7 @@
   }
   const int64_t n_tiles = (n + SCAN_TILE - 1) / SCAN_TILE;
   if (!tile_sums_ready) hipLaunchKernelGGL((scan_reduce_kernel<Load>), dim3((unsigned)n_tiles), dim3(SCAN_THREADS), 0, st, ld, n, tile_sums, n_live);
-  hipLaunchKernelGGL(scan_tiles_kernel, dim3(1), dim3(ST_THREADS), 0, st, tile_sums, n_tiles, n_live);
+  hipLaunchKernelGGL(scan_tiles_kernel, dim3(1), dim3(ST_THREADS), 0, st, tile_sums, n_tiles, n_live, ExpandForm{nullptr, nullptr, 0, 0, ~0ull, 0});
   hipLaunchKernelGGL((scan_downsweep_kernel<Load>), dim3((unsigned)n_tiles), dim3(SCAN_THREADS), 0, st, ld, n, tile_sums, n_tiles, out, n_live);
   return hipGetLastError();
 }
diff --git a/universal-recommender_amd/csrc/cco_expand.hip b/universal-recommender_amd/csrc/cco_expand.hip
--- a/universal-recommender_amd/csrc/cco_expand.hip
+++ b/universal-recommender_amd/csrc/cco_expand.hip
@@ -134,17 +134,100 @@
   return hipGetLastError();
 }
 
+__global__ __launch_bounds__(SCAN_THREADS) void expand_downsweep_kernel(const int32_t* __restrict__ plen, int64_t n, const int64_t* __restrict__ tile_sums,
+                                                                        int64_t n_tiles, int64_t* __restrict__ out, const int64_t* __restrict__ n_live,
+                                                                        const int32_t* __restrict__ form, const unsigned* __restrict__ pstart32,
+                                                                        int64_t* __restrict__ pstart64) {
+  __shared__ long long s_wave[SCAN_THREADS / WAVE];
+  if ((int64_t)blockIdx.x * SCAN_TILE > *n_live) return;
+  const int f = *form;
+  const LoadI32 ld{plen};
+  const int64_t first = (int64_t)blockIdx.x * SCAN_TILE + (int64_t)threadIdx.x * SCAN_ITEMS;
+  static_assert(SCAN_ITEMS == 8, "load8");
+  long long x[SCAN_ITEMS];
+  long long v = 0;
+  const bool interior = first + SCAN_ITEMS <= n;
+  if (interior) {
+    ld.load8(first, x);
+  } else {
+#pragma unroll
+    for (int q = 0; q < SCAN_ITEMS; ++q) x[q] = first + q < n ? ld(first + q) : 0;
+  }
+#pragma unroll
+  for (int q = 0; q < SCAN_ITEMS; ++q) v += x[q];
+  long long tot;
+  long long run = block_exclusive_scan(v, s_wave, &tot) + tile_sums[blockIdx.x];
+  if (f == 0) {
+    unsigned* out32 = reinterpret_cast<unsigned*>(out);
+    unsigned r = (unsigned)run;
+    if (interior && (reinterpret_cast<uintptr_t>(out) & 15) == 0) {
+      unsigned e[SCAN_ITEMS];
+#pragma unroll
+      for (int q = 0; q < SCAN_ITEMS; ++q) {
+        e[q] = r;
+        r += (unsigned)x[q];
+      }
+      *reinterpret_cast<uint4*>(out32 + first) = make_uint4(e[0], e[1], e[2], e[3]);
+      *reinterpret_cast<uint4*>(out32 + first + 4) = make_uint4(e[4], e[5], e[6], e[7]);
+    } else {
+#pragma unroll
+      for (int q = 0; q < SCAN_ITEMS; ++q) {
+        if (first + q < n) out32[first + q] = r;
+        r += (unsigned)x[q];
+      }
+    }
+    if (blockIdx.x == 0 && threadIdx.x == 0) out32[n] = (unsigned)tile_sums[n_tiles];
+    return;
+  }
+  if (interior && (reinterpret_cast<uintptr_t>(out) & 15) == 0) {
+#pragma unroll
+    for (int q = 0; q < SCAN_ITEMS; q += 2) {
+      const long long e0 = run, e1 = run + x[q];
+      run = e1 + x[q + 1];
+      int4 w;
+      w.x = (int)(unsigned)e0; w.y = (int)(unsigned)((unsigned long long)e0 >> 32);
+      w.z = (int)(unsigned)e1; w.w = (int)(unsigned)((unsigned long long)e1 >> 32);
+      *reinterpret_cast<int4*>(out + first + q) = w;
+    }
+  } else {
+#pragma unroll
+    for (int q = 0; q < SCAN_ITEMS; ++q) {
+      const int64_t i = first + q;
+      if (i < n) out[i] = run;
+      run += x[q];
+    }
+  }
+  if (!(f & FORM_PS64) && pstart32 && pstart64) {
+#pragma unroll
+    for (int q = 0; q < SCAN_ITEMS; ++q)
+      if (first + q < n) pstart64[first + q] = (int64_t)pstart32[first + q];
+  }
+  if (blockIdx.x == 0 && threadIdx.x == 0) out[n] = tile_sums[n_tiles];
+}
+static hipError_t expand_scan(hipStream_t st, const int32_t* plen, int64_t cap, int64_t* wp, int64_t* tile_sums, const int64_t* n_live, bool tile_sums_ready,
+                              const unsigned* pstart32, int64_t* pstart64, ExpandForm form) {
+  const int64_t n_tiles = cap > 0 ? (cap + SCAN_TILE - 1) / SCAN_TILE : 1;
+  if (!tile_sums_ready || cap <= 0)
+    hipLaunchKernelGGL((scan_reduce_kernel<LoadI32>), dim3((unsigned)n_tiles), dim3(SCAN_THREADS), 0, st, LoadI32{plen}, cap, tile_sums, n_live);
+  hipLaunchKernelGGL(scan_tiles_kernel, dim3(1), dim3(ST_THREADS), 0, st, tile_sums, n_tiles, n_live, form);
+  hipLaunchKernelGGL(expand_downsweep_kernel, dim3((unsigned)n_tiles), dim3(SCAN_THREADS), 0, st, plen, cap, (const int64_t*)tile_sums, n_tiles, wp, n_live,
+                     (const int32_t*)form.word, pstart32, pstart64);
+  return hipGetLastError();
+}
+
 __global__ __launch_bounds__(256) void narrow_row_ptr_kernel(const int64_t* __restrict__ rp, int64_t n, unsigned* __restrict__ out) {
   for (int64_t i = (int64_t)blockIdx.x * 256 + threadIdx.x; i < n; i += (int64_t)gridDim.x * 256) out[i] = (unsigned)rp[i];
 }
 
 __global__ __launch_bounds__(256) void expand_prepare_kernel(const int64_t* __restrict__ a_cp, int32_t n_items_a, const int32_t* __restrict__ a_ri,
                                                              const int64_t* __restrict__ b_rp, const unsigned* __restrict__ b_rp32, int64_t n_rows_b,
-                                                             int64_t cap, int64_t* __restrict__ pstart, int32_t* __restrict__ plen) {
+                                                             int64_t cap, unsigned* __restrict__ pstart32, int64_t* __restrict__ pstart64,
+                                                             int32_t* __restrict__ plen, int32_t* __restrict__ form) {
   const int64_t nnz = a_cp[n_items_a];
   int64_t lim = (nnz / SCAN_TILE + 1) * SCAN_TILE;
   if (lim > cap) lim = cap;
   const bool narrow = b_rp32 != nullptr && b_rp[n_rows_b] < ((int64_t)1 << 32);
+  if (!narrow && pstart64 && blockIdx.x == 0 && threadIdx.x == 0) *form = FORM_PS64;
   const int64_t stride = (int64_t)gridDim.x * 256;
   for (int64_t p0 = (int64_t)blockIdx.x * 256 + threadIdx.x; p0 < lim; p0 += stride * 4) {
     int u[4];
@@ -171,7 +254,11 @@
     for (int q = 0; q < 4; ++q) {
       const int64_t p = p0 + q * stride;
       if (p < lim) {
-        pstart[p] = s[q];
+        if (narrow) {
+          if (pstart32) pstart32[p] = (unsigned)s[q];
+        } else if (pstart64) {
+          pstart64[p] = s[q];
+        }
         plen[p] = (int32_t)(e[q] - s[q]);
       }
     }
@@ -179,8 +266,10 @@
 }
 
 hipError_t launch_expand_prepare(hipStream_t st, int n_cu, const int64_t* a_col_ptr, int32_t n_items_a, const int32_t* a_row_idx,
-                                 const int64_t* b_row_ptr, unsigned* b_rp32_scratch, int64_t n_rows_b, int64_t cap, int64_t* pstart, int32_t* plen,
-                                 int64_t* wp, int64_t* tile_sums) {
+                                 const int64_t* b_row_ptr, unsigned* b_rp32_scratch, int64_t n_rows_b, int64_t cap, unsigned* pstart32, int64_t* pstart64,
+                                 int32_t* plen, int64_t* wp, int64_t* tile_sums, ExpandForm form) {
+  hipError_t e = hipMemsetAsync(form.word, 0, sizeof(int32_t), st);
+  if (e != hipSuccess) return e;
   if (cap > 0) {
     if (b_rp32_scratch) {
       int64_t nb = (n_rows_b + 1 + 255) / 256;
@@ -191,16 +280,16 @@
     const int64_t lim = (int64_t)n_cu * 16;
     if (blocks > lim) blocks = lim;
     hipLaunchKernelGGL(expand_prepare_kernel, dim3((unsigned)blocks), dim3(256), 0, st, a_col_ptr, n_items_a, a_row_idx, b_row_ptr,
-                       (const unsigned*)b_rp32_scratch, n_rows_b, cap, pstart, plen);
-  }
-  return launch_scan(st, LoadI32{plen}, cap, wp, tile_sums, a_col_ptr + n_items_a);
+                       (const unsigned*)b_rp32_scratch, n_rows_b, cap, pstart32, pstart64, plen, form.word);
+  }
+  return expand_scan(st, plen, cap, wp, tile_sums, a_col_ptr + n_items_a, false, pstart32, pstart64, form);
 }
 
 struct __attribute__((packed, aligned(4))) Words4 { unsigned a, b, c, d; };
 struct __attribute__((packed, aligned(4))) Words2 { unsigned a, b; };
 struct ExpandMultiArgs {
   const int64_t* b_rp[EXPAND_MULTI_MAX];
-  int64_t* pstart[EXPAND_MULTI_MAX];
+  unsigned* pstart[EXPAND_MULTI_MAX];
   int32_t* plen[EXPAND_MULTI_MAX];
   int64_t* tsum[EXPAND_MULTI_MAX];
   int n;
@@ -263,7 +352,7 @@
 #pragma unroll
           for (int d = 0; d < N; ++d) {
             const int32_t len = (int32_t)(v[q][N + d] - v[q][d]);
-            a.pstart[d][p] = (int64_t)v[q][d];
+            a.pstart[d][p] = v[q][d];
             a.plen[d][p] = len;
             sum[d] += (long long)len;
           }
@@ -288,7 +377,7 @@
   }
 }
 hipError_t launch_expand_prepare_multi(hipStream_t st, int n_cu, const int64_t* a_col_ptr, int32_t n_items_a, const int32_t* a_row_idx, int n,
-                                       const int64_t* const* b_row_ptr, int64_t n_rows_b, int64_t cap, int64_t* const* pstart, int32_t* const* plen, void* T,
+                                       const int64_t* const* b_row_ptr, int64_t n_rows_b, int64_t cap, unsigned* const* pstart, int32_t* const* plen, void* T,
                                        int64_t* const* tsum) {
   if (n < 1 || n > EXPAND_MULTI_MAX) return hipErrorInvalidValue;
   if (cap <= 0) return hipSuccess;
@@ -321,28 +410,38 @@
   return hipGetLastError();
 }
 hipError_t launch_expand_scan(hipStream_t st, const int64_t* a_col_ptr, int32_t n_items_a, const int32_t* plen, int64_t cap, int64_t* wp, int64_t* tile_sums,
-                              bool tile_sums_ready) {
-  return launch_scan(st, LoadI32{plen}, cap, wp, tile_sums, a_col_ptr + n_items_a, tile_sums_ready);
-}
-
+                              bool tile_sums_ready, const unsigned* pstart32, int64_t* pstart64, ExpandForm form) {
+  hipError_t e = hipMemsetAsync(form.word, 0, sizeof(int32_t), st);
+  if (e != hipSuccess) return e;
+  return expand_scan(st, plen, cap, wp, tile_sums, a_col_ptr + n_items_a, tile_sums_ready, pstart32, pstart64, form);
+}
+
+__device__ __forceinline__ int64_t work_prefix_at(const int64_t* __restrict__ wp, const int64_t* __restrict__ tile_sums, bool narrow, int64_t p) {
+  if (!narrow) return wp[p];
+  const int64_t base = tile_sums[p / SCAN_TILE];
+  return base + (int64_t)(unsigned)(reinterpret_cast<const unsigned*>(wp)[p] - (unsigned)base);
+}
 __global__ __launch_bounds__(256) void row_work_kernel(int32_t item_lo, int32_t item_hi, const int64_t* __restrict__ a_cp,
-                                                       const int64_t* __restrict__ wp, int64_t* __restrict__ work) {
+                                                       const int64_t* __restrict__ wp, const int64_t* __restrict__ tile_sums, const int32_t* __restrict__ form,
+                                                       int64_t* __restrict__ work) {
   const int64_t n = (int64_t)item_hi - item_lo;
+  const bool narrow = *form == 0;
   for (int64_t t = (int64_t)blockIdx.x * 256 + threadIdx.x; t < n; t += (int64_t)gridDim.x * 256) {
     const int64_t i = item_lo + t;
-    work[t] = wp[a_cp[i + 1]] - wp[a_cp[i]];
-  }
-}
-
-hipError_t launch_row_work(hipStream_t st, int n_cu, int32_t item_lo, int32_t item_hi, const int64_t* a_col_ptr, const int64_t* wp, int64_t* work) {
+    work[t] = work_prefix_at(wp, tile_sums, narrow, a_cp[i + 1]) - work_prefix_at(wp, tile_sums, narrow, a_cp[i]);
+  }
+}
+
+hipError_t launch_row_work(hipStream_t st, int n_cu, int32_t item_lo, int32_t item_hi, const int64_t* a_col_ptr, const int64_t* wp, const int64_t* tile_sums,
+                           const int32_t* form, int64_t* work) {
   const int64_t n = (int64_t)item_hi - item_lo;
   if (n <= 0) return hipSuccess;
   int64_t blocks = (n + 255) / 256;
   const int64_t cap = (int64_t)n_cu * 8;
   if (blocks > cap) blocks = cap;
-  hipLaunchKernelGGL(row_work_kernel, dim3((unsigned)blocks), dim3(256), 0, st, item_lo, item_hi, a_col_ptr, wp, work);
-  return hipGetLastError();
-}
-
-
-}
+  hipLaunchKernelGGL(row_work_kernel, dim3((unsigned)blocks), dim3(256), 0, st, item_lo, item_hi, a_col_ptr, wp, tile_sums, form, work);
+  return hipGetLastError();
+}
+
+
+}
diff --git a/universal-recommender_amd/csrc/cco_kernels.h b/universal-recommender_amd/csrc/cco_kernels.h
--- a/universal-recommender_amd/csrc/cco_kernels.h
+++ b/universal-recommender_amd/csrc/cco_kernels.h
@@ -30,15 +30,30 @@
 constexpr int32_t DBG_UNPACKED_COUNTS = 1048576;
 constexpr int32_t DBG_ROW_KERNELS = DBG_GATHER_ONLY | DBG_NO_LLR | DBG_NO_TOPK | DBG_NO_SELECT | DBG_NO_RANK | DBG_NO_COUNT_GATHER | DBG_SELECT_DELAY;
 
+constexpr int32_t FORM_WIDE = 1;
+constexpr int32_t FORM_PS64 = 2;
+constexpr int32_t FORM_TILE = 4;
+constexpr int32_t FORM_PACK = 8;
+constexpr int32_t FORM_HOST = 16;
+constexpr unsigned long long NARROW_LIMIT = 1ull << 32;
+struct ExpandForm {
+  int32_t* word;
+  const int32_t* pack_bad;
+  int32_t host_wide;
+  int32_t host_narrow;
+  unsigned long long limit;
+  long long seed;
+};
+
 struct CcoArgs {
   const int32_t* bin_rows;
   const int32_t* bin_off;
   const int64_t* a_col_ptr;
-  const int64_t* pstart;
+  const unsigned* pstart32;
   const int64_t* wp;
   const int32_t* b_col_idx;
   const int32_t* b_packed;
-  const int32_t* pack_bad;
+  const int32_t* form;
   int32_t pk_known;
   uint32_t b_col_mask;
   const int32_t* cnt_a;
@@ -71,6 +86,8 @@
   unsigned long long* g_cand_key;
   int32_t* g_cand_col;
   int32_t g_blocks;
+  const int64_t* pstart64;
+  const int64_t* work;
 };
 
 hipError_t launch_column_counts(hipStream_t st, int n_cu, const int32_t* col_idx, int64_t nnz, int32_t n_cols, int32_t* counts);
@@ -147,14 +164,15 @@
 
 hipError_t launch_expand_prepare(hipStream_t st, int n_cu, const int64_t* a_col_ptr, int32_t n_items_a, const int32_t* a_row_idx,
                                  const int64_t* b_row_ptr, unsigned* b_rp32_scratch , int64_t n_rows_b, int64_t cap,
-                                 int64_t* pstart, int32_t* plen, int64_t* wp, int64_t* tile_sums);
+                                 unsigned* pstart32, int64_t* pstart64, int32_t* plen, int64_t* wp, int64_t* tile_sums, ExpandForm form);
 constexpr int EXPAND_MULTI_MAX = 8;
 hipError_t launch_expand_prepare_multi(hipStream_t st, int n_cu, const int64_t* a_col_ptr, int32_t n_items_a, const int32_t* a_row_idx, int n,
-                                       const int64_t* const* b_row_ptr, int64_t n_rows_b, int64_t cap, int64_t* const* pstart, int32_t* const* plen, void* T,
+                                       const int64_t* const* b_row_ptr, int64_t n_rows_b, int64_t cap, unsigned* const* pstart, int32_t* const* plen, void* T,
                                        int64_t* const* tsum );
 hipError_t launch_expand_scan(hipStream_t st, const int64_t* a_col_ptr, int32_t n_items_a, const int32_t* plen, int64_t cap, int64_t* wp, int64_t* tile_sums,
-                              bool tile_sums_ready = false);
-hipError_t launch_row_work(hipStream_t st, int n_cu, int32_t item_lo, int32_t item_hi, const int64_t* a_col_ptr, const int64_t* wp, int64_t* work);
+                              bool tile_sums_ready, const unsigned* pstart32, int64_t* pstart64, ExpandForm form);
+hipError_t launch_row_work(hipStream_t st, int n_cu, int32_t item_lo, int32_t item_hi, const int64_t* a_col_ptr, const int64_t* wp, const int64_t* tile_sums,
+                           const int32_t* form, int64_t* work);
 
 hipError_t launch_binning(hipStream_t st, int32_t item_lo, int32_t n, const int64_t* work, const int32_t* cnt_a, int32_t n_cols_b,
                           int32_t count_bits, int32_t k, int64_t* tile_counts, int32_t* bin_off, int32_t* bin_rows, int64_t* stats);
diff --git a/universal-recommender_amd/csrc/cco_rows.hip b/universal-recommender_amd/csrc/cco_rows.hip
--- a/universal-recommender_amd/csrc/cco_rows.hip
+++ b/universal-recommender_amd/csrc/cco_rows.hip
@@ -465,9 +465,13 @@
 constexpr int URCCO_G_BLOCK = 2;
 constexpr int URCCO_SEL_M_BLOCK = 128;
 constexpr int URCCO_G_CU = 2;
+template <bool NARROW> struct PStart { typedef int64_t type; };
+template <> struct PStart<true> { typedef unsigned type; };
 template <int T, int E, int U, bool MP = false, bool DBG = false, bool PK = false>
 __global__ __launch_bounds__((T < 256 ? 256 : T), (T == 64 ? URCCO_OCC_WAVE : (T == 256 && E == 4096 ? URCCO_OCC_BS : (T == 512 ? 4 : 1)))) void cco_rows_kernel(CcoArgs a, int bin) {
-  if ((a.b_packed != nullptr && (a.pk_known != 0 || *a.pack_bad == 0)) != PK) return;
+  if ((a.b_packed != nullptr && (a.pk_known != 0 || *a.form == 0)) != PK) return;
+  using PS = typename PStart<PK>::type;
+  constexpr int WS = PK ? 1 : 2;
   const int dbg = DBG ? a.debug : 0;
   constexpr bool packed = PK;
   URCCO_OWN_GLOBAL_PTR(const int32_t, b_col_idx, PK ? a.b_packed : a.b_col_idx);
@@ -529,7 +533,7 @@
   unsigned* tab = s_tab + team * E;
   unsigned* cand = tab + SH;
   unsigned long long* share = s_share + (SHARE ? team * SHARE_WORDS : 0);
-  long long* ustart = SHARE ? reinterpret_cast<long long*>(share) : s_ustart + team * T;
+  PS* ustart = reinterpret_cast<PS*>(SHARE ? reinterpret_cast<long long*>(share) : s_ustart + team * T);
   unsigned* uoff = SHARE ? reinterpret_cast<unsigned*>(share + T) : s_uoff + team * (T + 1);
   unsigned* hist = SHARE ? reinterpret_cast<unsigned*>(share) : s_hist + team * NH * 128;
   unsigned* sel_res = s_selres + team * 4;
@@ -553,6 +557,9 @@
   const int S = total_teams;
   auto pos_of = [&](int l) { return list_start + (l < list_n ? l : list_n - 1); };
   const unsigned* wp32 = reinterpret_cast<const unsigned*>(a.wp);
+  const PS* pstart;
+  if constexpr (PK) pstart = a.pstart32;
+  else pstart = a.pstart64;
   const int lane3 = lane < 3 ? lane : 2;
   int idv = a.bin_rows[pos_of(li + lane3 * S)];
   int64_t cs_c, ce_c;
@@ -565,14 +572,14 @@
     bnd_b = a.a_col_ptr[id1 + (lane & 1)];
   }
   unsigned pf_w0, pf_w1, pf_wp;
-  int64_t pf_start;
+  PS pf_start;
   {
     const int64_t c1 = cs_c + T < ce_c ? cs_c + T : ce_c;
     const int64_t pl = cs_c + tl < c1 ? cs_c + tl : c1 - 1;
-    pf_w0 = wp32[2 * cs_c];
-    pf_w1 = wp32[2 * c1];
-    pf_wp = wp32[2 * pl];
-    pf_start = a.pstart[pl];
+    pf_w0 = wp32[WS * cs_c];
+    pf_w1 = wp32[WS * c1];
+    pf_wp = wp32[WS * pl];
+    pf_start = pstart[pl];
   }
   URCCO_SETTLE(idv); URCCO_SETTLE(bnd_b); URCCO_SETTLE(pf_w0); URCCO_SETTLE(pf_w1); URCCO_SETTLE(pf_wp); URCCO_SETTLE(pf_start);
   int64_t cs_n = 0, ce_n = 0, bnd_c = 0;
@@ -584,7 +591,7 @@
     ce_n = wave_read_lane64(bnd_b, 1);
     const unsigned row_w0 = uni(pf_w0), row_w1 = uni(pf_w1);
     const unsigned my_wp = pf_wp;
-    const int64_t my_start = pf_start;
+    const PS my_start = pf_start;
     int lz = lane;
     URCCO_OPAQUE(lz);
     idv = a.bin_rows[pos_of(li + (1 + (lz < 3 ? lz : 2)) * S)];
@@ -592,15 +599,15 @@
     if (!MP) {
       const int64_t c1 = cs_n + T < ce_n ? cs_n + T : ce_n;
       const int64_t pl = cs_n + tl < c1 ? cs_n + tl : c1 - 1;
-      pf_w0 = wp32[2 * cs_n];
-      pf_w1 = wp32[2 * c1];
-      pf_wp = wp32[2 * pl];
-      pf_start = a.pstart[pl];
+      pf_w0 = wp32[WS * cs_n];
+      pf_w1 = wp32[WS * c1];
+      pf_wp = wp32[WS * pl];
+      pf_start = pstart[pl];
     }
     int mp_s = 0;
     unsigned mp_q = 0u, n_run = 0u, run_cur = 0u;
     if (MP) {
-      const long long w_row = (long long)(uni(a.wp[ce]) - uni(a.wp[cs]));
+      const long long w_row = (long long)uni(a.work[i - a.item_lo]);
       const long long ca_row = a.cnt_a[i];
       const long long dd = w_row < (long long)a.n_cols_b ? w_row : (long long)a.n_cols_b;
       const long long cap = ((long long)E - 3ll * a.k - 2ll) / 3ll;
@@ -632,12 +639,12 @@
     for (int64_t c0 = cs; c0 < ce; c0 += T) {
       const int64_t c1 = c0 + T < ce ? c0 + T : ce;
       const bool pre = !MP && c0 == cs;
-      const unsigned w0 = pre ? row_w0 : uni(wp32[2 * c0]);
-      const unsigned total = (pre ? row_w1 : uni(wp32[2 * c1])) - w0;
+      const unsigned w0 = pre ? row_w0 : uni(wp32[WS * c0]);
+      const unsigned total = (pre ? row_w1 : uni(wp32[WS * c1])) - w0;
       const int64_t p = c0 + tl;
       if (p < c1) {
-        ustart[tl] = pre ? my_start : a.pstart[p];
-        uoff[tl] = (pre ? my_wp : wp32[2 * p]) - w0;
+        ustart[tl] = pre ? my_start : pstart[p];
+        uoff[tl] = (pre ? my_wp : wp32[WS * p]) - w0;
       } else {
         uoff[tl] = total;
       }
@@ -661,7 +668,7 @@
             lo = gt ? lo : mid + 1;
           }
           o = lo - 1;
-          pos = ustart[o] + (first - uoff[o]);
+          pos = (int64_t)ustart[o] + (first - uoff[o]);
           uend = uoff[o + 1];
         }
         for (unsigned x = 0; x < per; x += G) {
@@ -675,7 +682,7 @@
             if (on[q]) {
               if (t >= uend) {
                 do { ++o; } while (uoff[o + 1] <= t);
-                pos = ustart[o];
+                pos = (int64_t)ustart[o];
                 uend = uoff[o + 1];
               }
               jj[q] = (unsigned)b_col_idx[pos++];
@@ -1184,15 +1191,21 @@
   return best;
 }
 
+__device__ __forceinline__ unsigned gather_start(unsigned v, unsigned src) { return wave_gather(v, src); }
+__device__ __forceinline__ int64_t gather_start(int64_t v, unsigned src) { return wave_gather64(v, src); }
 template <int L, bool DBG, bool PK = false>
 __global__ __launch_bounds__(256, (L == WAVE ? URCCO_OCC_MICRO : URCCO_OCC_MICRO - 2)) void cco_rows_micro_kernel(CcoArgs a) {
-  if ((a.b_packed != nullptr && (a.pk_known != 0 || *a.pack_bad == 0)) != PK) return;
+  if ((a.b_packed != nullptr && (a.pk_known != 0 || *a.form == 0)) != PK) return;
+  using PS = typename PStart<PK>::type;
+  constexpr int WS = PK ? 1 : 2;
   using G = MicroGeom<L>;
   constexpr int S = G::S;
   const int dbg = DBG ? a.debug : 0;
   const int32_t* bin_rows = a.bin_rows;
   const int64_t* a_col_ptr = a.a_col_ptr;
-  const int64_t* pstart = a.pstart;
+  const PS* pstart;
+  if constexpr (PK) pstart = a.pstart32;
+  else pstart = a.pstart64;
   constexpr bool packed = PK;
   const int32_t* b_col_idx = PK ? a.b_packed : a.b_col_idx;
   const int cshift = 32 - a.count_bits;
@@ -1239,7 +1252,7 @@
   int i_n2 = row_at(li + 2 * stride);
   int64_t cs1 = a_col_ptr[i_n1], ce1 = a_col_ptr[i_n1 + 1];
   unsigned pf_w1, pf_wp;
-  int64_t pf_start;
+  PS pf_start;
   int pf_ca;
   double pf_ent;
   int n_cur;
@@ -1247,8 +1260,8 @@
     const int64_t cs0 = a_col_ptr[i_cur], ce0 = a_col_ptr[i_cur + 1];
     n_cur = (int)(ce0 - cs0);
     const int64_t pl = sl < n_cur ? cs0 + sl : ce0 - 1;
-    pf_w1 = wp32[2 * ce0];
-    pf_wp = wp32[2 * pl];
+    pf_w1 = wp32[WS * ce0];
+    pf_wp = wp32[WS * pl];
     pf_start = pstart[pl];
     pf_ca = cnt_a[i_cur];
     pf_ent = ent_a[i_cur];
@@ -1265,15 +1278,15 @@
     const bool owns_user = live && sl < n_cur;
     const long long ca = (long long)pf_ca;
     const double row_entropy = pf_ent;
-    const int64_t my_start = owns_user ? pf_start : 0;
+    const PS my_start = owns_user ? pf_start : (PS)0;
     const unsigned my_off = owns_user ? pf_wp - w0 : total;
     int i_n3 = row_at(li + 3 * stride);
     int64_t cs2 = a_col_ptr[i_n2], ce2 = a_col_ptr[i_n2 + 1];
     n_cur = (int)(ce1 - cs1);
     {
       const int64_t pl = sl < n_cur ? cs1 + sl : ce1 - 1;
-      pf_w1 = wp32[2 * ce1];
-      pf_wp = wp32[2 * pl];
+      pf_w1 = wp32[WS * ce1];
+      pf_wp = wp32[WS * pl];
       pf_start = pstart[pl];
       pf_ca = cnt_a[i_n1];
       pf_ent = ent_a[i_n1];
@@ -1283,11 +1296,11 @@
     if (owns_user) atomicMax(&marks[my_off], (unsigned)sl);
     wave_sync();
     const unsigned o = seg_inclusive_max<L>(marks[sl]);
-    const int64_t base_o = wave_gather64(my_start - (int64_t)my_off, (unsigned)(seg * L) + o);
+    const PS base_o = gather_start(my_start - (PS)my_off, (unsigned)(seg * L) + o);
     unsigned slot = 0xffffffffu;
     unsigned jj = 0u;
     if ((unsigned)sl < total) {
-      jj = (unsigned)b_col_idx[base_o + sl];
+      jj = (unsigned)b_col_idx[base_o + (PS)sl];
       if (!(dbg & DBG_GATHER_ONLY)) {
         bool ok;
         slot = tab_insert_claim(tab, (jj & colmask) + 1u, cb, (unsigned)(G::TW - 1), 32 - G::LOG2TW, ident, &ok);
@@ -1405,6 +1418,11 @@
 constexpr int GB_THREADS = 1024;
 constexpr int GSEL_K = 1024;
 
+__device__ __forceinline__ int64_t g_start(const unsigned* ps32, const int64_t* ps64, bool nar, int64_t p) { return nar ? (int64_t)ps32[p] : ps64[p]; }
+__device__ __forceinline__ int64_t g_len(const int64_t* wp, bool nar, int64_t p) {
+  const unsigned* w = reinterpret_cast<const unsigned*>(wp);
+  return nar ? (int64_t)(unsigned)(w[p + 1] - w[p]) : wp[p + 1] - wp[p];
+}
 __global__ __launch_bounds__(GB_THREADS) void cco_rows_global_kernel(CcoArgs a) {
   constexpr int NW = GB_THREADS / WAVE;
   __shared__ unsigned long long s_pkey[2][NW];
@@ -1425,19 +1443,20 @@
   const int G = 1 << a.g_log2;
   const int grp = threadIdx.x >> a.g_log2, gl = threadIdx.x & (G - 1), ngrp = GB_THREADS >> a.g_log2;
   const double xlx_n = *a.xlx_n;
+  const bool nar = *a.form == 0;
   for (int li = blockIdx.x; li < list_n; li += gridDim.x) {
     const int i = a.bin_rows[list_start + li];
     const int64_t cs = a.a_col_ptr[i], ce = a.a_col_ptr[i + 1];
     if (threadIdx.x == 0) s_ncand = 0;
     for (int64_t p = cs + grp; p < ce; p += ngrp) {
-      const int64_t s = a.pstart[p], e = s + (a.wp[p + 1] - a.wp[p]);
+      const int64_t s = g_start(a.pstart32, a.pstart64, nar, p), e = s + g_len(a.wp, nar, p);
       for (int64_t q = s + gl; q < e; q += G) atomicAdd(&cnt[(unsigned)a.b_col_idx[q] & a.b_col_mask], 1);
     }
     __syncthreads();
     const long long ca = a.cnt_a[i];
     const double row_entropy = a.ent_a[i];
     for (int64_t p = cs + grp; p < ce; p += ngrp) {
-      const int64_t s = a.pstart[p], e = s + (a.wp[p + 1] - a.wp[p]);
+      const int64_t s = g_start(a.pstart32, a.pstart64, nar, p), e = s + g_len(a.wp, nar, p);
       for (int64_t q = s + gl; q < e; q += G) {
         const int j = (int)((unsigned)a.b_col_idx[q] & a.b_col_mask);
         const long long k11 = atomicExch(&cnt[j], 0);
diff --git a/universal-recommender_amd/csrc/urcco_api.hip b/universal-recommender_amd/csrc/urcco_api.hip
--- a/universal-recommender_amd/csrc/urcco_api.hip
+++ b/universal-recommender_amd/csrc/urcco_api.hip
@@ -176,6 +176,7 @@
   if (s->arena) (void)hipFree(s->arena);
   if (s->xlx_tab) (void)hipFree(s->xlx_tab);
   if (s->xlx_hi) (void)hipFree(s->xlx_hi);
+  if (s->form_word) (void)hipFree(s->form_word);
   if (s->g_counts) { (void)hipFree(s->g_counts); (void)hipFree(s->g_cand_key); (void)hipFree(s->g_cand_col); }
   s->collect();
   for (hipEvent_t e : s->free_events) (void)hipEventDestroy(e);
@@ -192,6 +193,21 @@
 int urcco_session_set_debug(urcco_session* s, int32_t flags) {
   if (!s) return fail(URCCO_BAD_ARG, "session is NULL");
   s->debug = flags;
+  return URCCO_OK;
+}
+
+int urcco_session_set_expand_test(urcco_session* s, int64_t limit, int64_t prefix_seed) {
+  if (!s || limit < 0 || prefix_seed < 0) return fail(URCCO_BAD_ARG, "urcco_session_set_expand_test: bad argument");
+  s->narrow_limit = limit == 0 ? urcco::NARROW_LIMIT : (unsigned long long)limit;
+  s->prefix_seed = prefix_seed;
+  return URCCO_OK;
+}
+
+int urcco_session_expand_form(urcco_session* s, int32_t* form_host) {
+  if (!s || !form_host) return fail(URCCO_BAD_ARG, "urcco_session_expand_form: bad argument");
+  if (!s->form_word || !s->form_valid) return fail(URCCO_BAD_ARG, "urcco_session_expand_form: no rows were built on this session");
+  HIPC(hipMemcpyAsync(form_host, s->form_word, sizeof(int32_t), hipMemcpyDeviceToHost, s->stream));
+  HIPC(hipStreamSynchronize(s->stream));
   return URCCO_OK;
 }
 
@@ -318,15 +334,18 @@
     return fail(URCCO_BAD_ARG, "urcco_dev_row_work: bad argument");
   const int64_t cap = nnz_a_bound;
   const int64_t n_tiles = (cap + urcco::SCAN_TILE - 1) / urcco::SCAN_TILE;
-  URC(s->reserve(urcco_session::need((size_t)cap, 8) + urcco_session::need((size_t)cap, 4) + urcco_session::need((size_t)cap + 1, 8) +
-                 urcco_session::need((size_t)n_tiles + 2, 8)));
-  int64_t* pstart = s->take<int64_t>((size_t)cap);
+  URC(s->reserve(urcco_session::need((size_t)cap, 4) + urcco_session::need((size_t)cap + 1, 8) + urcco_session::need((size_t)n_tiles + 2, 8)));
+  if (!s->form_word) HIPC(hipMalloc((void**)&s->form_word, sizeof(int32_t)));
+  s->form_valid = false;
   int32_t* plen = s->take<int32_t>((size_t)cap);
   int64_t* wp = s->take<int64_t>((size_t)cap + 1);
   int64_t* tile_sums = s->take<int64_t>((size_t)n_tiles + 2);
+  int32_t* form = s->form_word;
   s->begin(URCCO_STAGE_ROW_WORK);
-  HIPC(urcco::launch_expand_prepare(s->stream, s->n_cu, a_col_ptr, n_items_a, a_row_idx, b_row_ptr, nullptr, 0, cap, pstart, plen, wp, tile_sums));
-  HIPC(urcco::launch_row_work(s->stream, s->n_cu, item_lo, item_hi, a_col_ptr, wp, work));
+  HIPC(urcco::launch_expand_prepare(s->stream, s->n_cu, a_col_ptr, n_items_a, a_row_idx, b_row_ptr, nullptr, 0, cap, nullptr, nullptr, plen, wp, tile_sums,
+                                    urcco::ExpandForm{form, nullptr, 0, 0, s->narrow_limit, s->prefix_seed}));
+  HIPC(urcco::launch_row_work(s->stream, s->n_cu, item_lo, item_hi, a_col_ptr, wp, tile_sums, form, work));
+  s->form_valid = true;
   s->end();
   return URCCO_OK;
 }
@@ -406,7 +425,7 @@
 int cco_rows_impl(urcco_session* s, int32_t item_lo, int32_t item_hi, int32_t n_items_a, const int64_t* a_col_ptr, const int32_t* a_row_idx, int64_t nnz_a_bound,
                   const int64_t* b_row_ptr, const int32_t* b_col_idx, int32_t n_cols_b, const int32_t* counts_a, const int32_t* counts_b, int64_t n_users,
                   int32_t exclude_self, int32_t k, int32_t has_min_llr, double min_llr, int32_t* out_count, int32_t* out_idx, double* out_llr, int64_t* stats_dev,
-                  const int64_t* pre_pstart, const int32_t* pre_plen, int64_t* pre_tile_sums, const int32_t* b_packed, const int32_t* pack_bad, bool pk_known) {
+                  const unsigned* pre_pstart, const int32_t* pre_plen, int64_t* pre_tile_sums, const int32_t* b_packed, const int32_t* pack_bad, bool pk_known, int64_t b_nnz_bound) {
   if (!s || item_lo < 0 || item_hi < item_lo || item_hi > n_items_a || n_cols_b < 0 || n_users < 0 || nnz_a_bound < 0 || !a_col_ptr || !b_row_ptr)
     return fail(URCCO_BAD_ARG, "urcco_dev_cco_rows: bad argument");
   if (k <= 0) return fail(URCCO_BAD_ARG, "maxInterestingElements must be positive, got %d", k);
@@ -439,16 +458,20 @@
   const int64_t n_tiles = ((int64_t)n + urcco::BIN_TILE - 1) / urcco::BIN_TILE;
   const int64_t cap = nnz_a_bound;
   const int64_t p_tiles = (cap + urcco::SCAN_TILE - 1) / urcco::SCAN_TILE;
-  URC(s->reserve(urcco_session::need((size_t)cap, 8) + urcco_session::need((size_t)cap, 4) + urcco_session::need((size_t)cap + 1, 8) +
+  if (!s->form_word) HIPC(hipMalloc((void**)&s->form_word, sizeof(int32_t)));
+  s->form_valid = false;
+  URC(s->reserve(urcco_session::need((size_t)cap, 8) + urcco_session::need((size_t)cap, 4) + (pre_pstart ? 0 : urcco_session::need((size_t)cap, 4)) + urcco_session::need((size_t)cap + 1, 8) +
                  urcco_session::need((size_t)p_tiles + 2, 8) +
                  urcco_session::need((size_t)n, 8) + urcco_session::need((size_t)(n_tiles + 1) * urcco::BIN_COLS_HOST, 8) +
                  urcco_session::need(urcco::BIN_OFF_LEN, 4) + urcco_session::need((size_t)n, 4) + urcco_session::need((size_t)n_items_a, 8) +
                  urcco_session::need((size_t)n_cols_b, 2) + urcco_session::need(1, 4) + urcco_session::need(urcco::CAND_SLOTS, 8) + urcco_session::need(1, 8) + urcco_session::need(URCCO_STATS_LEN, 8) +
                  urcco_session::need((size_t)n_users + 1, 4)));
-  int64_t* own_pstart = s->take<int64_t>((size_t)cap);
+  int64_t* pstart64 = s->take<int64_t>((size_t)cap);
+  unsigned* own_pstart = pre_pstart ? nullptr : s->take<unsigned>((size_t)cap);
   int32_t* own_plen = s->take<int32_t>((size_t)cap);
-  const int64_t* pstart = pre_pstart ? pre_pstart : own_pstart;
+  const unsigned* pstart32 = pre_pstart ? pre_pstart : own_pstart;
   int64_t* wp = s->take<int64_t>((size_t)cap + 1);
+  int32_t* form = s->form_word;
   int64_t* p_tile_sums = s->take<int64_t>((size_t)p_tiles + 2);
   int64_t* work = s->take<int64_t>((size_t)n);
   int64_t* tile_counts = s->take<int64_t>((size_t)(n_tiles + 1) * urcco::BIN_COLS_HOST);
@@ -462,12 +485,19 @@
   int64_t* stats = stats_dev ? stats_dev : s->take<int64_t>(URCCO_STATS_LEN);
   unsigned* b_rp32 = s->take<unsigned>((size_t)n_users + 1);
 
+  const int32_t* packed = pk_known ? b_col_idx : ((b_packed && pack_bad && !(s->debug & urcco::DBG_UNPACKED_COUNTS)) ? b_packed : nullptr);
+  const bool host_wide = packed == nullptr || (s->debug & urcco::DBG_ROW_KERNELS) != 0;
+  const bool narrow_known = pk_known && !host_wide && b_nnz_bound >= 0 && b_nnz_bound < ((int64_t)1 << 32) &&
+                            (unsigned long long)n_cols_b * (unsigned long long)urcco::SCAN_TILE < s->narrow_limit;
+  const urcco::ExpandForm ef{form, pk_known ? nullptr : pack_bad, host_wide ? 1 : 0, narrow_known ? 1 : 0, s->narrow_limit, s->prefix_seed};
+  int64_t* tile_sums = (pre_pstart && pre_plen && pre_tile_sums) ? pre_tile_sums : p_tile_sums;
   s->begin(URCCO_STAGE_ROW_WORK);
   if (pre_pstart && pre_plen)
-    HIPC(urcco::launch_expand_scan(s->stream, a_col_ptr, n_items_a, pre_plen, cap, wp, pre_tile_sums ? pre_tile_sums : p_tile_sums, pre_tile_sums != nullptr));
+    HIPC(urcco::launch_expand_scan(s->stream, a_col_ptr, n_items_a, pre_plen, cap, wp, tile_sums, pre_tile_sums != nullptr, pre_pstart, pstart64, ef));
   else
-    HIPC(urcco::launch_expand_prepare(s->stream, s->n_cu, a_col_ptr, n_items_a, a_row_idx, b_row_ptr, b_rp32, n_users, cap, own_pstart, own_plen, wp, p_tile_sums));
-  HIPC(urcco::launch_row_work(s->stream, s->n_cu, item_lo, item_hi, a_col_ptr, wp, work));
+    HIPC(urcco::launch_expand_prepare(s->stream, s->n_cu, a_col_ptr, n_items_a, a_row_idx, b_row_ptr, b_rp32, n_users, cap, own_pstart, pstart64, own_plen, wp, tile_sums, ef));
+  HIPC(urcco::launch_row_work(s->stream, s->n_cu, item_lo, item_hi, a_col_ptr, wp, tile_sums, form, work));
+  s->form_valid = true;
   s->end();
   s->begin(URCCO_STAGE_BINNING);
   HIPC(hipMemsetAsync(stats, 0, sizeof(int64_t) * URCCO_STATS_LEN, s->stream));
@@ -480,10 +510,8 @@
 
   urcco::CcoArgs a;
   a.bin_rows = bin_rows; a.bin_off = bin_off;
-  a.a_col_ptr = a_col_ptr; a.pstart = pstart; a.wp = wp; a.b_col_idx = b_col_idx;
-  a.b_packed = pk_known ? b_col_idx : ((b_packed && pack_bad && !(s->debug & urcco::DBG_UNPACKED_COUNTS)) ? b_packed : nullptr);
-  a.pack_bad = pack_bad;
-  a.pk_known = pk_known ? 1 : 0;
+  a.a_col_ptr = a_col_ptr; a.pstart32 = pstart32; a.pstart64 = pstart64; a.wp = wp; a.form = form; a.work = work; a.b_col_idx = b_col_idx;
+  a.b_packed = packed; a.pk_known = narrow_known ? 1 : 0;
   a.b_col_mask = pk_known ? (key_bits >= 32 ? 0xffffffffu : (1u << key_bits) - 1u) : 0xffffffffu;
   a.cnt_a = counts_a; a.cnt_b = counts_b; a.ent_a = ent_a; a.cnt_b16 = cnt_b16; a.cnt16_bad = cnt16_bad; a.xlx_n = xlx_n; a.xlx_tab = s->xlx_tab; a.xlx_hi = s->xlx_hi; a.col_ent = s->xlx_hi + urcco::XLX_TABLE_HOST; a.debug = s->debug;
   a.n_users = n_users; a.n_cols_b = n_cols_b; a.item_lo = item_lo; a.exclude_self = exclude_self ? 1 : 0; a.k = k;
@@ -524,7 +552,7 @@
 }
 
 int expand_multi(urcco_session* s, int n, const int64_t* a_col_ptr, int32_t n_items_a, const int32_t* a_row_idx, int64_t cap, const int64_t* const* b_row_ptr,
-                 int64_t n_users, int64_t* const* pstart, int32_t* const* plen, int64_t* const* tile_sums) {
+                 int64_t n_users, unsigned* const* pstart, int32_t* const* plen, int64_t* const* tile_sums) {
   if (!s || n < 1 || n > urcco::EXPAND_MULTI_MAX || !a_col_ptr || cap < 0) return fail(URCCO_BAD_ARG, "expand_multi: bad argument");
   URC(s->reserve(urcco_session::need(((size_t)n_users + 2) * (size_t)n, 4) + 256));
   void* T = s->take<unsigned>(((size_t)n_users + 2) * (size_t)n);
diff --git a/universal-recommender_amd/csrc/urcco_context.hip b/universal-recommender_amd/csrc/urcco_context.hip
--- a/universal-recommender_amd/csrc/urcco_context.hip
+++ b/universal-recommender_amd/csrc/urcco_context.hip
@@ -174,7 +174,7 @@
     HIPC(hipHostGetDevicePointer((void**)&h_verr_dev, h_verr, 0));
     return URCCO_OK;
   }
-  DBuf<int64_t> pre_pstart;
+  DBuf<unsigned> pre_pstart;
   DBuf<int32_t> pre_plen;
   DBuf<int64_t> pre_tsum;
   DBuf<int32_t> mlen, pack;
@@ -513,7 +513,7 @@
   URC(cco_rows_impl(E.s, D.item_lo, D.item_hi, (int32_t)pa.n_cols, D.a_cp[D.par].p, D.a_ri[D.par].p, a_nnz_bound, E.b_rp, E.b_ci, (int32_t)p.n_cols,
                     post_of(D, 0).p, post_of(D, d).p, n_users, d == 0 ? 1 : 0, p.k, p.has_min_llr, p.min_llr, E.o_count.p, E.o_idx.p, E.o_llr.p, E.stats.p,
                     pre_expanded ? E.pre_pstart.p : nullptr, pre_expanded ? E.pre_plen.p : nullptr, pre_expanded ? E.pre_tsum.p : nullptr,
-                    E.b_pk_known ? nullptr : E.b_pk.p, E.b_pk_known ? nullptr : E.pk_bad.p, E.b_pk_known));
+                    E.b_pk_known ? nullptr : E.b_pk.p, E.b_pk_known ? nullptr : E.pk_bad.p, E.b_pk_known, E.b_nnz_bound));
   URC(urcco_dev_compact_indicators(E.s, n, p.k, E.o_count.p, E.o_idx.p, E.o_llr.p, E.c_rp.p, E.c_idx.p, E.c_llr.p));
   HIPC(hipEventRecord(E.ev_done, E.s->stream));
   HIPC(hipEventRecord(E.ev_cons[D.par], E.s->stream));
@@ -575,7 +575,7 @@
     EvState& L = D.ev[1];
     if (L.s != A.s) HIPC(hipStreamWaitEvent(L.s->stream, D.a_ready, 0));
     std::vector<const int64_t*> rp((size_t)(n_ds - f0));
-    std::vector<int64_t*> ps((size_t)(n_ds - f0));
+    std::vector<unsigned*> ps((size_t)(n_ds - f0));
     std::vector<int32_t*> pl((size_t)(n_ds - f0));
     std::vector<int64_t*> ts((size_t)(n_ds - f0));
     for (int d = f0; d < n_ds; ++d) {
@@ -1121,7 +1121,7 @@
       EvState& L = D.ev[1];
       if (L.s != D.ev[0].s) HIPC(hipStreamWaitEvent(L.s->stream, D.a_ready, 0));
       std::vector<const int64_t*> rp((size_t)n_ds - 1);
-      std::vector<int64_t*> pst((size_t)n_ds - 1);
+      std::vector<unsigned*> pst((size_t)n_ds - 1);
       std::vector<int32_t*> pl((size_t)n_ds - 1);
       std::vector<int64_t*> ts((size_t)n_ds - 1);
       for (int d = 1; d < n_ds; ++d) {
diff --git a/universal-recommender_amd/csrc/urcco_internal.h b/universal-recommender_amd/csrc/urcco_internal.h
--- a/universal-recommender_amd/csrc/urcco_internal.h
+++ b/universal-recommender_amd/csrc/urcco_internal.h
@@ -79,14 +79,15 @@
 int cco_rows_impl(urcco_session* s, int32_t item_lo, int32_t item_hi, int32_t n_items_a, const int64_t* a_col_ptr, const int32_t* a_row_idx, int64_t nnz_a_bound,
                   const int64_t* b_row_ptr, const int32_t* b_col_idx, int32_t n_cols_b, const int32_t* counts_a, const int32_t* counts_b, int64_t n_users,
                   int32_t exclude_self, int32_t k, int32_t has_min_llr, double min_llr, int32_t* out_count, int32_t* out_idx, double* out_llr, int64_t* stats_dev,
-                  const int64_t* pre_pstart, const int32_t* pre_plen, int64_t* pre_tile_sums = nullptr ,
+                  const unsigned* pre_pstart, const int32_t* pre_plen, int64_t* pre_tile_sums = nullptr ,
                   const int32_t* b_packed = nullptr , const int32_t* pack_bad = nullptr ,
-                  bool pk_known = false );
+                  bool pk_known = false ,
+                  int64_t b_nnz_bound = -1 );
 int pack_counts(urcco_session* s, const int64_t* b_row_ptr, int64_t n_rows_b, const int32_t* b_col_idx, int64_t nnz_bound, const int32_t* counts_b, int32_t n_cols_b,
                 int32_t* out, int32_t* bad);
 int partition_dev(urcco_session* s, int32_t n_items, const int64_t* work, int32_t n_parts, int32_t* bounds_dev, int32_t** bounds_out);
 int expand_multi(urcco_session* s, int n, const int64_t* a_col_ptr, int32_t n_items_a, const int32_t* a_row_idx, int64_t cap, const int64_t* const* b_row_ptr,
-                 int64_t n_users, int64_t* const* pstart, int32_t* const* plen, int64_t* const* tile_sums = nullptr );
+                 int64_t n_users, unsigned* const* pstart, int32_t* const* plen, int64_t* const* tile_sums = nullptr );
 inline size_t expand_tile_words(int64_t cap) { return (size_t)((cap + urcco::SCAN_TILE - 1) / urcco::SCAN_TILE + 2); }
 }
 
@@ -108,6 +109,10 @@
   double* xlx_hi = nullptr;
   long long xlx_hi_n = -1;
   int debug = 0;
+  unsigned long long narrow_limit = urcco::NARROW_LIMIT;
+  long long prefix_seed = 0;
+  int32_t* form_word = nullptr;
+  bool form_valid = false;
   unsigned* marks = nullptr;
   unsigned mark_seq = 0;
   int unordered_rows = 0;
diff --git a/universal-recommender_amd/device.py b/universal-recommender_amd/device.py
--- a/universal-recommender_amd/device.py
+++ b/universal-recommender_amd/device.py
@@ -96,6 +96,14 @@
 
     def set_debug(self, flags: int):
         self._check(self.lib.urcco_session_set_debug(self.handle, int(flags)))
+
+    def expand_form(self) -> int:
+        f = C.c_int32(-1)
+        self._check(self.lib.urcco_session_expand_form(self.handle, C.byref(f)))
+        return int(f.value)
+
+    def set_expand_test(self, limit: int = 0, prefix_seed: int = 0):
+        self._check(self.lib.urcco_session_set_expand_test(self.handle, int(limit), int(prefix_seed)))
 
     def get_timings(self):
         ms = (C.c_double * _lib.N_STAGES)()
```

Measured after the change: 35.30 billion pairs/s, median of 6. 1.03x the previous value.
